# jzhoulab/orca

Hardware: AMD Instinct MI355X
Metric: Mb of sequence encoded+decoded per second (32Mb H1-ESC-shaped model, both strands, 6 levels) (higher is better)
Workload: dtype f16x2 | Encoder Conv1d stages 1-7: f16x2 = fp32 emulated as 2 x fp16 split operands, 3 MFMA products, fp32 accumulate (22 significant operand bits); Decoder / Decoder_1m Conv2d: f16x2 = fp32 emulated as 2 x fp16 split operands, 3 MFMA products, fp32 accumulate (22 significant operand bits); Encoder2; 1 GPU; H1-ESC 32Mb model forward, single random 32Mb sequence, fp32-class (f16x2 split operands on the 16-bit matrix cores, see dtype; parity vs the reference's fp32 in `parity` with --full), both strands (genomepredict-equivalent, 1 model): Encoder+Encoder2+6 Decoder+Decoder_1m per strand; sequence_bp=32000000, strands=2, levels=6, weights=synthetic seed 0, input=1 byte/base packed sequence in HBM, both strands read from it, parallelism=single GPU

## Files before the change

### include/orca_hip.h

```cpp
#ifndef ORCA_HIP_H
#define ORCA_HIP_H

#include <stddef.h>
#include <stdint.h>

#ifdef __cplusplus
extern "C" {
#endif

#define ORCA_OK 0
#define ORCA_EINVAL (-1)
#define ORCA_EHIP (-2)
#define ORCA_ENOMEM (-3)
#define ORCA_ENODEV (-4)

#define ORCA_ABI_VERSION 1

typedef struct orca_ctx orca_ctx;
typedef struct orca_net orca_net;

enum orca_net_kind {
  ORCA_NET_ENCODER = 1,
  ORCA_NET_ENCODER2 = 2,
  ORCA_NET_ENCODER3 = 3,
  ORCA_NET_DECODER = 4,
  ORCA_NET_DECODER_1M = 5,
  ORCA_NET_ENCODER2B = 6
};

#define ORCA_UPSAMPLE_NEAREST 0
#define ORCA_UPSAMPLE_BILINEAR 1

typedef struct orca_conv_desc {
  const float* weight_host;
  const float* bias_host;
  int32_t cout;
  int32_t cin;
  int32_t ksize;
  int32_t dilation;
} orca_conv_desc;


int orca_abi_version(void);
const char* orca_last_error(void);

int orca_device_count(void);

int orca_ctx_create(int device, void* hip_stream, orca_ctx** out);
int orca_ctx_destroy(orca_ctx* ctx);
int orca_ctx_set_stream(orca_ctx* ctx, void* hip_stream);
int orca_ctx_workspace_bytes(orca_ctx* ctx, size_t* out);
int orca_ctx_release_workspace(orca_ctx* ctx);

typedef struct orca_kernel_time {
  int32_t cout, cin, tile, batch;
  int64_t n;
  float ms;
  int32_t ksize;
} orca_kernel_time;
int orca_ctx_set_timing(orca_ctx* ctx, int enable);
int orca_ctx_get_timing(orca_ctx* ctx, orca_kernel_time* out, int max, int* n);

int orca_ctx_launch_counts(orca_ctx* ctx, int64_t* counts4);

int orca_net_create(orca_ctx* ctx, int kind, const orca_conv_desc* convs, int n_convs,
                    int upsample_mode, orca_net** out);
int orca_net_free(orca_net* net);

#define ORCA_PRECISION_F32 0
#define ORCA_PRECISION_BF16 1
#define ORCA_PRECISION_BF16X2 2
#define ORCA_PRECISION_BF16X3 3
#define ORCA_PRECISION_F16X2 4
#define ORCA_PRECISION_F16 5
int orca_net_set_precision(orca_net* net, int precision);
#define ORCA_ENCODER_FORM_DEFAULT 0
#define ORCA_ENCODER_FORM_STORED_RESIDUAL 1
#define ORCA_ENCODER_FORM_LCONV1_ONLY 2
#define ORCA_ENCODER_FORM_TWO_CONV 3
int orca_net_set_encoder_form(orca_net* net, int form);
int orca_net_set_decoder_block_runs(orca_net* net, int on);
int orca_net_set_encoder_two_strands(orca_net* net, int on);
int orca_net_get_encoder_two_strands(orca_net* net, int* on);
int orca_ctx_take_overflow(orca_ctx* ctx, int* flag);


int orca_encoder_forward(orca_ctx* ctx, orca_net* net, const float* x, int64_t sx_b, int64_t sx_c,
                         int64_t sx_l, int B, int64_t L, int64_t bin_lo, int64_t bin_hi, float* out,
                         int64_t so_b, int64_t so_c, int64_t chunk_bp);

int orca_pack_sequence(orca_ctx* ctx, const float* x, int64_t sx_c, int64_t sx_l, int64_t L, uint8_t* codes_out, int* packable);
int orca_encoder_forward_codes(orca_ctx* ctx, orca_net* net, const uint8_t* codes, int64_t sc_b, int reverse, int B, int64_t L,
                               int64_t bin_lo, int64_t bin_hi, float* out, int64_t so_b, int64_t so_c, int64_t chunk_bp);
int orca_encoder_forward_codes_window(orca_ctx* ctx, orca_net* net, const uint8_t* codes, int64_t sc_b, int64_t win_origin,
                                      int64_t win_len, int reverse, int B, int64_t L, int64_t bin_lo, int64_t bin_hi,
                                      float* out, int64_t so_b, int64_t so_c, int64_t chunk_bp);
int orca_encoder_forward_2bit(orca_ctx* ctx, orca_net* net, const uint8_t* two, const uint8_t* nmask, int64_t start, int reverse, int64_t L,
                              int64_t bin_lo, int64_t bin_hi, float* out, int64_t so_c, int64_t chunk_bp);
int orca_encoder_forward_two_strands(orca_ctx* ctx, orca_net* net, const uint8_t* codes, int64_t L, float* out_fwd, float* out_rev, int64_t so_c);

int64_t orca_p16_plane_units(int64_t n);
int orca_encoder_stage3_planes(orca_ctx* ctx, orca_net* net, const uint8_t* codes, int64_t L, int reverse, float* planes, int64_t plane_units);
int orca_p16_pool5_into(orca_ctx* ctx, const float* src, int64_t src_units, int64_t src_pos0, float* dst, int64_t dst_units, int64_t dst_pos0, int64_t count);
int orca_encoder_front_snippet(orca_ctx* ctx, orca_net* net, const uint8_t* codes, int64_t L, int reverse, int64_t base0, int64_t nbases, int64_t skip,
                               int64_t count, float* dst, int64_t dst_units, int64_t dst_pos0);
int orca_encoder_back(orca_ctx* ctx, orca_net* net, const float* s4, int64_t s4_units, int64_t n4, float* out, int64_t so_c);
int orca_encoder_stage4_rows(orca_ctx* ctx, orca_net* net, const float* s4, int64_t s4_units, int64_t n4, float* rows);
int orca_rows_pool5_into(orca_ctx* ctx, const float* src, int64_t src_rows, int64_t src_pos0, float* dst, int64_t dst_rows, int64_t dst_pos0, int64_t count);
int orca_encoder_front4_snippet(orca_ctx* ctx, orca_net* net, const uint8_t* codes, int64_t L, int reverse, int64_t base0, int64_t nbases, int64_t skip,
                                int64_t count, float* dst, int64_t dst_rows, int64_t dst_pos0);
int orca_encoder_front4_ranges(orca_ctx* ctx, orca_net* net, const uint8_t* codes, int64_t L, int reverse, int n_ranges, const int64_t* ranges_host,
                               float* dst, int64_t dst_rows);
int orca_encoder_back5(orca_ctx* ctx, orca_net* net, const float* rows, int64_t n5, float* out, int64_t so_c);

int orca_screen_edit_codes(orca_ctx* ctx, const uint8_t* window, int64_t L, const int64_t* table, int n_snippets, const uint8_t* payload, int64_t n_payload,
                           uint8_t* out, int64_t total);
int orca_screen_splice_rows(orca_ctx* ctx, const float* ref, int64_t n5, const float* fresh, int64_t n_fresh, const int64_t* table, int B, float* out);
int orca_encoder_back5_batch(orca_ctx* ctx, orca_net* net, const float* rows, int B, int64_t n5, float* out, int64_t so_b, int64_t so_c);
int orca_screen_scores(orca_ctx* ctx, const float* alt, int64_t map_bs, const float* ref, int B, int n, float* profile, float* mean, float* amax);

int orca_screen_edit_codes_multi(orca_ctx* ctx, const uint8_t* window, int64_t L, const int64_t* table, const int64_t* table_host, int n_snippets,
                                 const int64_t* spans, const int64_t* spans_host, int64_t n_spans, const uint8_t* payload, int64_t n_payload, uint8_t* out,
                                 int64_t total);
int orca_screen_splice_rows_multi(orca_ctx* ctx, const float* ref, int64_t n5, const float* fresh, int64_t n_fresh, const int64_t* segments,
                                  const int64_t* segments_host, int64_t n_segments, const int64_t* seg_off, const int64_t* seg_off_host, int B, float* out);
int orca_screen_region_scores(orca_ctx* ctx, const float* alt, int64_t map_bs, const float* ref, int B, int n, const int32_t* rects,
                              const int32_t* rects_host, int K, float* mean_signed, float* mean_abs);

int orca_screen_assemble_codes(orca_ctx* ctx, const uint8_t* context, int64_t C, const int64_t* table, const int64_t* table_host, int n_snippets,
                               const int64_t* pieces, const int64_t* pieces_host, int64_t n_pieces, const uint8_t* payload, int64_t n_payload, uint8_t* out,
                               int64_t total);
int orca_screen_gather_rows(orca_ctx* ctx, const float* ref, int64_t n5, const float* fresh, int64_t n_fresh, const float* const* entries,
                            const int64_t* entry_rows, const int64_t* entry_rows_host, int P, const int64_t* segments, const int64_t* segments_host,
                            int64_t n_segments, const int64_t* seg_off, const int64_t* seg_off_host, int B, float* out);

int orca_screen_aligned_scores(orca_ctx* ctx, const float* alt, int64_t map_bs, const float* ref, int B, int n, const int32_t* bin_map,
                               const int32_t* bin_map_host, float* profile, float* mean, float* amax);
int orca_screen_aligned_region_scores(orca_ctx* ctx, const float* alt, int64_t map_bs, const float* ref, int B, int n, const int32_t* bin_map,
                                      const int32_t* bin_map_host, const int32_t* rects, const int32_t* rects_host, int K, float* mean_signed,
                                      float* mean_abs);

int orca_screen_insulation(orca_ctx* ctx, const float* alt, int64_t map_bs, const float* ref, int B, int n, const int32_t* widths, const int32_t* widths_host,
                           int W, const int32_t* bin_map, const int32_t* bin_map_host, float* track, float* delta, float* aligned);
int orca_screen_viewpoints(orca_ctx* ctx, const float* alt, int64_t map_bs, const float* ref, int B, int n, const int32_t* views, const int32_t* views_host,
                           int V, const int32_t* bin_map, const int32_t* bin_map_host, float* delta, float* aligned);

int orca_screen_merge_strands(orca_ctx* ctx, const float* fwd, int64_t fwd_bs, const float* rev, int64_t rev_bs, const float* ref_fwd, const float* ref_rev,
                              int B, int n, float* out, int64_t out_bs, float* gap);

int orca_screen_epistasis_scores(orca_ctx* ctx, const float* alt, int64_t map_bs, const float* bank, int64_t bank_bs, int U, const float* ref, int B, int n,
                                 const int64_t* member_off, const int64_t* member_off_host, const int32_t* members, const int32_t* members_host, int64_t P,
                                 float* profile, float* mean, float* amax, float* add_mean);
int orca_screen_epistasis_region_scores(orca_ctx* ctx, const float* alt, int64_t map_bs, const float* bank, int64_t bank_bs, int U, const float* ref, int B,
                                        int n, const int64_t* member_off, const int64_t* member_off_host, const int32_t* members,
                                        const int32_t* members_host, int64_t P, const int32_t* rects, const int32_t* rects_host, int K, float* mean_signed,
                                        float* mean_abs);

int64_t orca_encoder_num_bins(int64_t L);

int orca_unet_forward(orca_ctx* ctx, orca_net* net, const float* x, int64_t sx_b, int64_t sx_c,
                      int64_t sx_l, int B, int n, float* const* outs_host, int n_outs);

int orca_decoder_forward(orca_ctx* ctx, orca_net* net, const float* x, int64_t sx_b, int64_t sx_c,
                         int64_t sx_l, const float* distenc, int64_t sd_b, int64_t sd_h, int64_t sd_w,
                         const float* y, int64_t sy_b, int64_t sy_h, int64_t sy_w, int B, int n,
                         float* out, int accumulate);

int orca_decoder_forward_mt(orca_ctx* ctx, orca_net* net, const float* x, int64_t sx_b, int64_t sx_c,
                            int64_t sx_l, const float* distenc, int64_t sd_b, int64_t sd_c, int64_t sd_h,
                            int64_t sd_w, const float* y, int64_t sy_b, int64_t sy_c, int64_t sy_h, int64_t sy_w,
                            int B, int n, float* out, int accumulate);

int orca_net_num_targets(orca_net* net, int* num_2d);

int orca_decoder_forward_rows(orca_ctx* ctx, orca_net* net, const float* const* x_rows, int64_t sx_c, int64_t sx_l,
                              const float* const* distenc_rows, int64_t sd_c, int64_t sd_h, int64_t sd_w,
                              const float* const* y_rows, int64_t sy_c, int64_t sy_h, int64_t sy_w, int B, int n,
                              float* out, int accumulate);
int orca_decoder1m_forward_rows(orca_ctx* ctx, orca_net* net, const float* const* x_rows, int64_t sx_c, int64_t sx_l,
                                int B, int n, float* out, int accumulate);

int orca_decoder1m_forward(orca_ctx* ctx, orca_net* net, const float* x, int64_t sx_b, int64_t sx_c,
                           int64_t sx_l, int B, int n, float* out, int accumulate);

int orca_decoder_probe(orca_ctx* ctx, orca_net* net, const float* x, int64_t sx_b, int64_t sx_c, int64_t sx_l,
                       const float* distenc, int64_t sd_b, int64_t sd_c, int64_t sd_h, int64_t sd_w, const float* y,
                       int64_t sy_b, int64_t sy_c, int64_t sy_h, int64_t sy_w, int B, int n, int stage, int channels,
                       float* map_out);

int orca_strand_merge(orca_ctx* ctx, const float* fwd, const float* rev, float* out, int n);

int orca_block_mean_f64(orca_ctx* ctx, const double* mat, int64_t ld, int64_t row0, int64_t col0, int nb, int npix,
                        double* mean_out, float* log_out, int flip);

int orca_adaptive_coarsegrain(orca_ctx* ctx, const float* ar, const float* countar, int64_t ld, int n, float cutoff,
                              int max_levels, int min_shape, float* out, int64_t ld_out);

int orca_genome_unpack_2bit(orca_ctx* ctx, const uint8_t* two_bit, const uint8_t* nmask, int64_t start, int64_t n, uint8_t* codes);

typedef struct orca_comm orca_comm;
#define ORCA_COMM_ID_BYTES 128
int orca_comm_unique_id(void* id128_host);
int orca_comm_init_rank(orca_ctx* ctx, int nranks, int rank, const void* id128_host, orca_comm** out);
int orca_comm_destroy(orca_comm* comm);
int orca_allgather(orca_ctx* ctx, orca_comm* comm, const float* send, float* recv, size_t count);

int orca_pointwise1d_forward(orca_ctx* ctx, const float* w_dev, const float* bias_dev, int cout, int cin, const float* x,
                             int64_t x_bs, int64_t ldx, float* y, int64_t y_bs, int64_t ldy, int B, int64_t n, int act);

int orca_conv1d_forward(orca_ctx* ctx, const orca_conv_desc* conv, const float* x, int64_t x_bs, int64_t ldx,
                        float* y, int64_t y_bs, int64_t ldy, const float* r1, const float* r2, int B, int64_t n,
                        int relu, int tile);
int orca_conv1d_nlc_forward(orca_ctx* ctx, const orca_conv_desc* conv, int precision, const float* x, float* y,
                            const float* r1, int B, int64_t n, int relu);
int orca_conv1d_p16_forward(orca_ctx* ctx, const orca_conv_desc* conv, const float* x, float* y, const float* r1,
                            int64_t n, int relu, int out_mode);
int orca_conv1d_b16_forward(orca_ctx* ctx, const orca_conv_desc* conv, const float* x, float* y, const float* r1,
                            int64_t n, int relu, int out_mode);
int orca_conv2d_forward(orca_ctx* ctx, const orca_conv_desc* conv, const float* x, float* y, const float* r,
                        int B, int n, int relu);
int orca_conv2d_m16_forward(orca_ctx* ctx, const orca_conv_desc* conv, int precision, const float* x, float* y,
                            const float* r, int B, int n, int relu);
int orca_conv2d_dblock_forward(orca_ctx* ctx, const orca_conv_desc* convs, int precision, const float* x, float* y, int B, int n);
int orca_conv2d_dblock_run_forward(orca_ctx* ctx, const orca_conv_desc* convs, int nblk, int precision, const float* x, float* y, int B, int n,
                                   int fused);
int orca_maxpool1d_forward(orca_ctx* ctx, const float* x, int64_t ldx, float* y, int64_t ldy, int64_t rows,
                           int64_t n_out, int k);

#ifdef __cplusplus
}
#endif
#endif
```

### orca_amd/_lib.py

```python
import ctypes
import os
from ctypes import POINTER, c_char_p, c_int, c_int32, c_int64, c_size_t, c_void_p

_HERE = os.path.dirname(os.path.abspath(__file__))
LIB_PATH = os.path.join(_HERE, "csrc", "liborca_hip.so")

ORCA_NET_ENCODER, ORCA_NET_ENCODER2, ORCA_NET_ENCODER3, ORCA_NET_DECODER, ORCA_NET_DECODER_1M, ORCA_NET_ENCODER2B = 1, 2, 3, 4, 5, 6
ORCA_UPSAMPLE_NEAREST, ORCA_UPSAMPLE_BILINEAR = 0, 1
PRECISIONS = {"f32": 0, "bf16": 1, "bf16x2": 2, "bf16x3": 3, "f16x2": 4, "f16": 5}
ENCODER_FORMS = {"default": 0, "stored_residual": 1, "lconv1_only": 2, "two_conv": 3}


class OrcaHipError(RuntimeError):
    pass


class ConvDesc(ctypes.Structure):
    _fields_ = [("weight_host", c_void_p), ("bias_host", c_void_p), ("cout", c_int32), ("cin", c_int32),
                ("ksize", c_int32), ("dilation", c_int32)]


class KernelTime(ctypes.Structure):
    _fields_ = [("cout", c_int32), ("cin", c_int32), ("tile", c_int32), ("batch", c_int32), ("n", c_int64),
                ("ms", ctypes.c_float), ("ksize", c_int32)]


SIGNATURES = {
    "orca_abi_version": (c_int, []),
    "orca_last_error": (c_char_p, []),
    "orca_device_count": (c_int, []),
    "orca_ctx_create": (c_int, [c_int, c_void_p, POINTER(c_void_p)]),
    "orca_ctx_destroy": (c_int, [c_void_p]),
    "orca_ctx_set_stream": (c_int, [c_void_p, c_void_p]),
    "orca_ctx_workspace_bytes": (c_int, [c_void_p, POINTER(c_size_t)]),
    "orca_ctx_release_workspace": (c_int, [c_void_p]),
    "orca_ctx_take_overflow": (c_int, [c_void_p, POINTER(c_int)]),
    "orca_ctx_set_timing": (c_int, [c_void_p, c_int]),
    "orca_ctx_get_timing": (c_int, [c_void_p, POINTER(KernelTime), c_int, POINTER(c_int)]),
    "orca_ctx_launch_counts": (c_int, [c_void_p, POINTER(ctypes.c_int64)]),
    "orca_net_create": (c_int, [c_void_p, c_int, POINTER(ConvDesc), c_int, c_int, POINTER(c_void_p)]),
    "orca_net_free": (c_int, [c_void_p]),
    "orca_net_set_precision": (c_int, [c_void_p, c_int]),
    "orca_net_set_encoder_form": (c_int, [c_void_p, c_int]),
    "orca_net_set_decoder_block_runs": (c_int, [c_void_p, c_int]),
    "orca_net_set_encoder_two_strands": (c_int, [c_void_p, c_int]),
    "orca_net_get_encoder_two_strands": (c_int, [c_void_p, POINTER(c_int)]),
    "orca_encoder_forward_two_strands": (c_int, [c_void_p, c_void_p, c_void_p, c_int64, c_void_p, c_void_p, c_int64]),
    "orca_encoder_forward": (c_int, [c_void_p, c_void_p, c_void_p, c_int64, c_int64, c_int64, c_int, c_int64, c_int64,
                                     c_int64, c_void_p, c_int64, c_int64, c_int64]),
    "orca_p16_plane_units": (c_int64, [c_int64]),
    "orca_encoder_stage3_planes": (c_int, [c_void_p, c_void_p, c_void_p, c_int64, c_int, c_void_p, c_int64]),
    "orca_p16_pool5_into": (c_int, [c_void_p, c_void_p, c_int64, c_int64, c_void_p, c_int64, c_int64, c_int64]),
    "orca_encoder_front_snippet": (c_int, [c_void_p, c_void_p, c_void_p, c_int64, c_int, c_int64, c_int64, c_int64, c_int64, c_void_p, c_int64, c_int64]),
    "orca_encoder_back": (c_int, [c_void_p, c_void_p, c_void_p, c_int64, c_int64, c_void_p, c_int64]),
    "orca_encoder_stage4_rows": (c_int, [c_void_p, c_void_p, c_void_p, c_int64, c_int64, c_void_p]),
    "orca_rows_pool5_into": (c_int, [c_void_p, c_void_p, c_int64, c_int64, c_void_p, c_int64, c_int64, c_int64]),
    "orca_encoder_front4_snippet": (c_int, [c_void_p, c_void_p, c_void_p, c_int64, c_int, c_int64, c_int64, c_int64, c_int64, c_void_p, c_int64, c_int64]),
    "orca_encoder_front4_ranges": (c_int, [c_void_p, c_void_p, c_void_p, c_int64, c_int, c_int, POINTER(ctypes.c_int64), c_void_p, c_int64]),
    "orca_encoder_back5": (c_int, [c_void_p, c_void_p, c_void_p, c_int64, c_void_p, c_int64]),
    "orca_screen_edit_codes": (c_int, [c_void_p, c_void_p, c_int64, c_void_p, c_int, c_void_p, c_int64, c_void_p, c_int64]),
    "orca_screen_splice_rows": (c_int, [c_void_p, c_void_p, c_int64, c_void_p, c_int64, c_void_p, c_int, c_void_p]),
    "orca_encoder_back5_batch": (c_int, [c_void_p, c_void_p, c_void_p, c_int, c_int64, c_void_p, c_int64, c_int64]),
    "orca_screen_scores": (c_int, [c_void_p, c_void_p, c_int64, c_void_p, c_int, c_int, c_void_p, c_void_p, c_void_p]),
    "orca_screen_edit_codes_multi": (c_int, [c_void_p, c_void_p, c_int64, c_void_p, c_void_p, c_int, c_void_p, c_void_p, c_int64, c_void_p, c_int64, c_void_p,
                                             c_int64]),
    "orca_screen_splice_rows_multi": (c_int, [c_void_p, c_void_p, c_int64, c_void_p, c_int64, c_void_p, c_void_p, c_int64, c_void_p, c_void_p, c_int, c_void_p]),
    "orca_screen_region_scores": (c_int, [c_void_p, c_void_p, c_int64, c_void_p, c_int, c_int, c_void_p, c_void_p, c_int, c_void_p, c_void_p]),
    "orca_screen_assemble_codes": (c_int, [c_void_p, c_void_p, c_int64, c_void_p, c_void_p, c_int, c_void_p, c_void_p, c_int64, c_void_p, c_int64, c_void_p,
                                           c_int64]),
    "orca_screen_gather_rows": (c_int, [c_void_p, c_void_p, c_int64, c_void_p, c_int64, c_void_p, c_void_p, c_void_p, c_int, c_void_p, c_void_p, c_int64, c_void_p,
                                        c_void_p, c_int, c_void_p]),
    "orca_screen_aligned_scores": (c_int, [c_void_p, c_void_p, c_int64, c_void_p, c_int, c_int, c_void_p, c_void_p, c_void_p, c_void_p, c_void_p]),
    "orca_screen_aligned_region_scores": (c_int, [c_void_p, c_void_p, c_int64, c_void_p, c_int, c_int, c_void_p, c_void_p, c_void_p, c_void_p, c_int, c_void_p,
                                                  c_void_p]),
    "orca_screen_insulation": (c_int, [c_void_p, c_void_p, c_int64, c_void_p, c_int, c_int, c_void_p, c_void_p, c_int, c_void_p, c_void_p, c_void_p, c_void_p,
                                       c_void_p]),
    "orca_screen_viewpoints": (c_int, [c_void_p, c_void_p, c_int64, c_void_p, c_int, c_int, c_void_p, c_void_p, c_int, c_void_p, c_void_p, c_void_p, c_void_p]),
    "orca_screen_merge_strands":(c_int, [c_void_p, c_void_p, c_int64, c_void_p, c_int64, c_void_p, c_void_p, c_int, c_int, c_void_p, c_int64, c_void_p]),
    "orca_screen_epistasis_scores": (c_int, [c_void_p, c_void_p, c_int64, c_void_p, c_int64, c_int, c_void_p, c_int, c_int, c_void_p, c_void_p, c_void_p, c_void_p,
                                             c_int64, c_void_p, c_void_p, c_void_p, c_void_p]),
    "orca_screen_epistasis_region_scores": (c_int, [c_void_p, c_void_p, c_int64, c_void_p, c_int64, c_int, c_void_p, c_int, c_int, c_void_p, c_void_p, c_void_p,
                                                    c_void_p, c_int64, c_void_p, c_void_p, c_int, c_void_p, c_void_p]),
    "orca_encoder_forward_2bit": (c_int, [c_void_p, c_void_p, c_void_p, c_void_p, c_int64, c_int, c_int64, c_int64, c_int64, c_void_p, c_int64, c_int64]),
    "orca_pack_sequence": (c_int, [c_void_p, c_void_p, c_int64, c_int64, c_int64, c_void_p, POINTER(c_int)]),
    "orca_encoder_forward_codes": (c_int, [c_void_p, c_void_p, c_void_p, c_int64, c_int, c_int, c_int64, c_int64, c_int64,
                                           c_void_p, c_int64, c_int64, c_int64]),
    "orca_encoder_forward_codes_window": (c_int, [c_void_p, c_void_p, c_void_p, c_int64, c_int64, c_int64, c_int, c_int, c_int64, c_int64, c_int64,
                                                  c_void_p, c_int64, c_int64, c_int64]),
    "orca_encoder_num_bins": (c_int64, [c_int64]),
    "orca_unet_forward": (c_int, [c_void_p, c_void_p, c_void_p, c_int64, c_int64, c_int64, c_int, c_int,
                                  POINTER(c_void_p), c_int]),
    "orca_decoder_forward": (c_int, [c_void_p, c_void_p, c_void_p, c_int64, c_int64, c_int64, c_void_p, c_int64,
                                     c_int64, c_int64, c_void_p, c_int64, c_int64, c_int64, c_int, c_int, c_void_p, c_int]),
    "orca_decoder_forward_mt": (c_int, [c_void_p, c_void_p, c_void_p, c_int64, c_int64, c_int64, c_void_p, c_int64, c_int64,
                                        c_int64, c_int64, c_void_p, c_int64, c_int64, c_int64, c_int64, c_int, c_int, c_void_p, c_int]),
    "orca_decoder_forward_rows": (c_int, [c_void_p, c_void_p, POINTER(c_void_p), c_int64, c_int64, POINTER(c_void_p), c_int64, c_int64, c_int64,
                                          POINTER(c_void_p), c_int64, c_int64, c_int64, c_int, c_int, c_void_p, c_int]),
    "orca_decoder1m_forward_rows": (c_int, [c_void_p, c_void_p, POINTER(c_void_p), c_int64, c_int64, c_int, c_int, c_void_p, c_int]),
    "orca_net_num_targets": (c_int, [c_void_p, POINTER(c_int)]),
    "orca_decoder1m_forward": (c_int, [c_void_p, c_void_p, c_void_p, c_int64, c_int64, c_int64, c_int, c_int, c_void_p, c_int]),
    "orca_decoder_probe": (c_int, [c_void_p, c_void_p, c_void_p, c_int64, c_int64, c_int64, c_void_p, c_int64, c_int64, c_int64, c_int64, c_void_p,
                                   c_int64, c_int64, c_int64, c_int64, c_int, c_int, c_int, c_int, c_void_p]),
    "orca_strand_merge": (c_int, [c_void_p, c_void_p, c_void_p, c_void_p, c_int]),
    "orca_block_mean_f64": (c_int, [c_void_p, c_void_p, c_int64, c_int64, c_int64, c_int, c_int, c_void_p, c_void_p, c_int]),
    "orca_adaptive_coarsegrain": (c_int, [c_void_p, c_void_p, c_void_p, c_int64, c_int, ctypes.c_float, c_int, c_int, c_void_p, c_int64]),
    "orca_genome_unpack_2bit": (c_int, [c_void_p, c_void_p, c_void_p, c_int64, c_int64, c_void_p]),
    "orca_comm_unique_id": (c_int, [c_void_p]),
    "orca_comm_init_rank": (c_int, [c_void_p, c_int, c_int, c_void_p, POINTER(c_void_p)]),
    "orca_comm_destroy": (c_int, [c_void_p]),
    "orca_allgather": (c_int, [c_void_p, c_void_p, c_void_p, c_void_p, c_size_t]),
    "orca_conv1d_forward": (c_int, [c_void_p, POINTER(ConvDesc), c_void_p, c_int64, c_int64, c_void_p, c_int64, c_int64,
                                    c_void_p, c_void_p, c_int, c_int64, c_int, c_int]),
    "orca_conv1d_nlc_forward": (c_int, [c_void_p, POINTER(ConvDesc), c_int, c_void_p, c_void_p, c_void_p, c_int, c_int64, c_int]),
    "orca_conv1d_p16_forward": (c_int, [c_void_p, POINTER(ConvDesc), c_void_p, c_void_p, c_void_p, c_int64, c_int, c_int]),
    "orca_conv1d_b16_forward": (c_int, [c_void_p, POINTER(ConvDesc), c_void_p, c_void_p, c_void_p, c_int64, c_int, c_int]),
    "orca_conv2d_forward": (c_int, [c_void_p, POINTER(ConvDesc), c_void_p, c_void_p, c_void_p, c_int, c_int, c_int]),
    "orca_conv2d_m16_forward": (c_int, [c_void_p, POINTER(ConvDesc), c_int, c_void_p, c_void_p, c_void_p, c_int, c_int, c_int]),
    "orca_conv2d_dblock_forward": (c_int, [c_void_p, POINTER(ConvDesc), c_int, c_void_p, c_void_p, c_int, c_int]),
    "orca_conv2d_dblock_run_forward": (c_int, [c_void_p, POINTER(ConvDesc), c_int, c_int, c_void_p, c_void_p, c_int, c_int, c_int]),
    "orca_maxpool1d_forward": (c_int, [c_void_p, c_void_p, c_int64, c_void_p, c_int64, c_int64, c_int64, c_int]),
    "orca_pointwise1d_forward": (c_int, [c_void_p, c_void_p, c_void_p, c_int, c_int, c_void_p, c_int64, c_int64, c_void_p, c_int64,
                                          c_int64, c_int, c_int64, c_int]),
}

_lib = None


def load():
    global _lib
    if _lib is not None:
        return _lib
    if not os.path.exists(LIB_PATH):
        raise OrcaHipError(
            f"{LIB_PATH} not found: the HIP extension is not built. Run `make -C orca_amd/csrc` "
            "(or `python -c 'import __graft_entry__ as g; g.build()'`). There is no CPU fallback.")
    import torch
    lib = ctypes.CDLL(LIB_PATH)
    for name, (res, args) in SIGNATURES.items():
        fn = getattr(lib, name)
        fn.restype = res
        fn.argtypes = args
    if lib.orca_abi_version() != 1:
        raise OrcaHipError("liborca_hip ABI version mismatch")
    _lib = lib
    return lib


def check(rc, what=""):
    if rc != 0:
        msg = load().orca_last_error()
        raise OrcaHipError(f"{what} failed (code {rc}): {msg.decode('utf8', 'replace') if msg else ''}")
```

### orca_amd/csrc/conv2d_dblock.h

```cpp
#pragma once
#include "conv2d_m16.h"

struct DBlockArgs {
  f32x4* cur;
  const void* w[12];
  const float* bias[12];
  long bs;
  int H, W, dil, nblk;
  unsigned* flag;
};

#ifndef DBLOCK_STORE_WT
#define DBLOCK_STORE_WT 0
#endif
__device__ __forceinline__ void db_store_unit(u32x4_t* p, const u32x4_t& v) {
#if DBLOCK_STORE_WT
  m16_store_unit(p, v);
#else
  *p = v;
#endif
}

template <int N>
__device__ __forceinline__ void db_vmwait() { asm volatile("s_waitcnt vmcnt(%0)" ::"n"(N) : "memory"); }

template <int NS, int DT, int MAXBLK, int ABL>
__device__ __forceinline__ void dblock_body(const DBlockArgs& a) {
  static_assert(MAXBLK == 1 || (NS == 2 && DT == 1), "block runs: f16x2 only");
  constexpr int WNS = DT == 1 ? 2 : 1;
  constexpr int NT = 512, PXW = 256 + 16;
  constexpr int AU = NS * 8 * PXW, BU = NS * 4 * PXW;
  constexpr int WP = NS * 9 * 2 * 32;
  constexpr int WIT = (WP + NT - 1) / NT;
  static_assert(NS * 8 * 256 / NT == 4 * NS, "gather: NS DMA instructions per thread and K-chunk of the first layer (the same for every wave)");
  constexpr int EXTRA = (WP - (WIT - 1) * NT + 63) / 64;
  __shared__ f32x4 smem[AU + BU + 3 * WP + 48 * MAXBLK];
  f32x4* const As = smem;
  f32x4* const Bs = smem + AU;
  f32x4* const Ws = smem + AU + BU;
  float* const bias_s = reinterpret_cast<float*>(smem + AU + BU + 3 * WP);

  const int tid = threadIdx.x, lane = tid & 63;
  const int wave = __builtin_amdgcn_readfirstlane(tid >> 6);
  const int l31 = lane & 31, g = lane >> 5;
  const int d = a.dil, H = a.H, W = a.W;
  const int nblk = MAXBLK == 1 ? 1 : a.nblk;
  const int ld = 31 - __builtin_clz(d);
  const int lS = 8 - ld, S = 1 << lS;
  const int lG = 2 * ld - 8, G = 1 << lG;
  f32x4* const cur = a.cur + (long)blockIdx.y * a.bs;

  int bx = (int)blockIdx.x;
  if (!(ABL & 64)) {
    const int xcd = bx & 7, t = bx >> 3;
    if (G == 1) { const int run = xcd * 4 + (t >> 3); bx = (run >> 1) * 16 + (run & 1) * 8 + (t & 7); }
    else if (G == 4) { const int pair = xcd * 16 + (t >> 1); bx = pair * 2 + (t & 1); }
  }
  auto pix = [&](int p, int& row, int& col, int& r, int& c) {
    const int sid = (bx << lG) + (p >> (2 * lS)), q = p & ((1 << (2 * lS)) - 1);
    r = q >> lS; c = q & (S - 1);
    row = (sid >> ld) + (r << ld);
    col = (sid & (d - 1)) + (c << ld);
  };
  {
    const int sid0 = bx << lG;
    if ((sid0 >> ld) >= H || (sid0 & (d - 1)) >= W) return;
  }

  if (tid < NS * 8 * 16) As[(tid >> 4) * PXW + 256 + (tid & 15)] = (f32x4)(0.f);
  if (tid >= 256 && tid < 256 + NS * 4 * 16) Bs[((tid - 256) >> 4) * PXW + 256 + (tid & 15)] = (f32x4)(0.f);
  __syncthreads();
  if (wave == 0 && lane < 48) {
#pragma unroll
    for (int b = 0; b < MAXBLK; ++b)
      if (b < nblk) {
        const float *b0 = a.bias[4 * b], *b1 = a.bias[4 * b + 1], *b2 = a.bias[4 * b + 2], *b3 = a.bias[4 * b + 3];
        const float* src = lane < 8 ? b0 + 4 * lane : (lane < 24 ? b1 + 4 * (lane - 8) : (lane < 32 ? b2 + 4 * (lane - 24) : b3 + 4 * (lane - 32)));
        p16_glds16(reinterpret_cast<const f32x4*>(src), smem + AU + BU + 3 * WP + 48 * b);
      }
  }

  auto issue_piece = [&](const void* wl, int i, int slot) {
    const int L = i >> 2, j = i & 3;
    const bool wide = L & 1;
    const int k = wide ? (j & 1) : j, h = wide ? (j >> 1) : 0, cout = wide ? 64 : 32;
    f32x4* dst = Ws + slot;
#pragma unroll
    for (int it = 0; it < WIT; ++it) {
      const int u = tid + it * NT;
      const int grp = u >> 5, co = u & 31;
      if (u < WP) p16_glds16(reinterpret_cast<const f32x4*>(wl) + ((long)k * (WNS * 9 * 2) + grp) * cout + h * 32 + co, dst + it * NT + wave * 64);
    }
  };
  int ro0 = 0, ro1 = WP, ro2 = 2 * WP;
  {
    int row, col, r_, c_;
    pix(tid & 255, row, col, r_, c_);
    const bool ok = row < H && col < W;
    const long off = ok ? (long)row * M16_PX + col : 255;
#pragma unroll
    for (int k = 0; k < 4; ++k) {
#pragma unroll
      for (int s_ = 0; s_ < NS; ++s_) {
        const int plane = s_ * 8 + 2 * k + (wave >> 2);
        if (!(ABL & 4)) p16_glds16(cur + m16_plane(plane & 7, s_, NS, H) + off, As + plane * PXW + (wave & 3) * 64);
      }
      if (k < 3) issue_piece(a.w[0], k, k * WP);
    }
  }

  const int p = wave * 32 + l31;
  int prow, pcol, pr, pc;
  pix(p, prow, pcol, pr, pc);
  const bool pvalid = prow < H && pcol < W;
  const long poff = (long)prow * M16_PX + pcol;

  f32x16 acc[2];
  const unsigned as_lds = p16_lds_addr(As), bs_lds = p16_lds_addr(Bs), ws_lds = p16_lds_addr(Ws + g * 32 + l31);
  bool overflow = false;
  auto put = [&](f32x4* Xs, int XG, int oct, f32x4 v) {
    if (!pvalid) v = (f32x4)(0.f);
    u32x2 sp[NS];
    split4<NS, DT>(v, sp, overflow);
#pragma unroll
    for (int s = 0; s < NS; ++s) *reinterpret_cast<u32x2*>(reinterpret_cast<char*>(Xs + (s * XG + oct) * PXW + p) + 8 * g) = sp[s];
  };
  auto get_A = [&](int oct) -> f32x4 {
    float f[4] = {0.f, 0.f, 0.f, 0.f};
#pragma unroll
    for (int s = 0; s < NS; ++s) {
      const u32x2 u = *reinterpret_cast<const u32x2*>(reinterpret_cast<const char*>(As + (s * 8 + oct) * PXW + p) + 8 * g);
      float a0, a1, a2, a3;
      m16_pair<DT>(u.x, a0, a1);
      m16_pair<DT>(u.y, a2, a3);
      f[0] += a0; f[1] += a1; f[2] += a2; f[3] += a3;
    }
    f32x4 r;
    r.x = f[0]; r.y = f[1]; r.z = f[2]; r.w = f[3];
    return r;
  };
  auto acc4 = [&](int h, int q, const float* bl, bool relu) -> f32x4 {
    const f32x4 b = *reinterpret_cast<const f32x4*>(bl + 8 * q + 4 * g);
    f32x4 v;
    v.x = acc[h][4 * q + 0] + b.x; v.y = acc[h][4 * q + 1] + b.y; v.z = acc[h][4 * q + 2] + b.z; v.w = acc[h][4 * q + 3] + b.w;
    if (relu) { v.x = p16_vmax(v.x, 0.f); v.y = p16_vmax(v.y, 0.f); v.z = p16_vmax(v.z, 0.f); v.w = p16_vmax(v.w, 0.f); }
    return v;
  };
  auto zero_acc = [&]() {
#pragma unroll
    for (int h = 0; h < 2; ++h)
#pragma unroll
      for (int r = 0; r < 16; ++r) acc[h][r] = 0.f;
  };
#define DB_READ(buf_, t_)                                                                                         \
  _Pragma("unroll") for (int s = 0; s < NS; ++s) {                                                                \
    xv[buf_][s] = p16_lds_read16(xrow + nb16[t_], s * XG * PXW * 16);                                             \
    wv[buf_][s] = p16_lds_read16(wrow, ((s * 9 + (t_)) * 2) * 32 * 16);                                           \
  }
#define DB_WAIT(NG, NW)                            \
  if (wave < EXTRA) db_vmwait<(NG) * NS + (NW) * WIT>(); else db_vmwait<(NG) * NS + (NW) * (WIT - 1)>()
#define DB_LAYER(LY, XLDS, XG_, WIDE)                                                                             \
  {                                                                                                               \
    constexpr int XG = XG_;                                                                                       \
    _Pragma("unroll") for (int j = 0; j < 4; ++j) {                                                               \
      constexpr bool wide_ = WIDE;                                                                                \
      const int piece = 4 * (LY) + j;                                                                             \
      const int k = wide_ ? (j & 1) : j;                                                                          \
      const int h = wide_ ? (j >> 1) : 0;                                                                         \
      if (piece <= 2 && first) {                                                                                  \
        if (piece == 0) { DB_WAIT(3, 2); } else if (piece == 1) { DB_WAIT(2, 1); } else { DB_WAIT(1, 1); }        \
      } else if (piece == 15 && last) db_vmwait<0>();                                                             \
      else { DB_WAIT(0, 1); }                                                                                     \
      if (!(ABL & 16) || j == 0) asm volatile("s_waitcnt lgkmcnt(0)\n\ts_barrier" ::: "memory");                  \
      if (!(ABL & 2)) {                                                                                           \
        const int slot2 = (piece + 2) % 3 == 0 ? ro0 : ((piece + 2) % 3 == 1 ? ro1 : ro2);                        \
        if (piece == 0) { if (!first) issue_piece(wb[0], 2, slot2); }                                             \
        else if (piece >= 14) { if (!last) issue_piece(wb[4], piece - 14, slot2); }                               \
        else issue_piece(wb[(piece + 2) >> 2], piece + 2, slot2);                                                 \
      }                                                                                                           \
      const unsigned wrow = ws_lds + (unsigned)((piece % 3 == 0 ? ro0 : (piece % 3 == 1 ? ro1 : ro2)) * 16);     \
      const unsigned xrow = (XLDS) + (unsigned)((2 * k + g) * PXW * 16);                                          \
      f16x8 xv[2][NS], wv[2][NS];                                                                                 \
      DB_READ(0, 0);                                                                                              \
      _Pragma("unroll") for (int t = 0; t < 9; ++t) {                                                             \
        const int fb = t & 1;                                                                                     \
        if (t + 1 < 9) { if (!(ABL & 8)) { DB_READ(fb ^ 1, t + 1); m16_wait<2 * NS, NS>(xv[fb], wv[fb]); } }      \
        else m16_wait<0, NS>(xv[fb], wv[fb]);                                                                     \
        typedef typename Op16<DT>::vec V_;                                                                        \
        if constexpr ((ABL & 1) != 0) { asm volatile("" ::"v"(xv[fb][0]), "v"(wv[fb][0])); } else                \
        if constexpr (NS == 2) {                                                                                  \
          acc[h] = Op16<DT>::mfma(__builtin_bit_cast(V_, wv[fb][0]), __builtin_bit_cast(V_, xv[fb][NS - 1]), acc[h]); \
          acc[h] = Op16<DT>::mfma(__builtin_bit_cast(V_, wv[fb][NS - 1]), __builtin_bit_cast(V_, xv[fb][0]), acc[h]); \
        }                                                                                                         \
        if constexpr ((ABL & 1) == 0) acc[h] = Op16<DT>::mfma(__builtin_bit_cast(V_, wv[fb][0]), __builtin_bit_cast(V_, xv[fb][0]), acc[h]); \
        __builtin_amdgcn_sched_barrier(0);                                                                        \
      }                                                                                                           \
    }                                                                                                             \
  }

  float vmax = 0.f;
#pragma unroll 1
  for (int bi = 0; bi < nblk; ++bi) {
    const int b = MAXBLK == 1 ? 0 : bi;
    const bool first = b == 0, last = MAXBLK == 1 || b + 1 == nblk;
    const void* wb[5];
#pragma unroll
    for (int q = 0; q < 5; ++q) wb[q] = a.w[4 * b + (q < 4 || !last ? q : 0)];
    const float* const bl = bias_s + 192 * b;
    unsigned nb16[9];
#pragma unroll
    for (int t = 0; t < 9; ++t) {
      const int dy = (t / 3 - 1) * (1 << b), dx = (t % 3 - 1) * (1 << b);
      const bool in = (unsigned)(pr + dy) < (unsigned)S && (unsigned)(pc + dx) < (unsigned)S;
      nb16[t] = (in ? (unsigned)(p + dy * S + dx) : 256u + ((unsigned)(p + dy * S + dx) & 15u)) * 16u;
    }
    zero_acc();
    DB_LAYER(0, as_lds, 8, false);
#pragma unroll
    for (int q = 0; q < 4; ++q) put(Bs, 4, q, acc4(0, q, bl, false));
    zero_acc();
    DB_LAYER(1, bs_lds, 4, true);
#pragma unroll
    for (int h = 0; h < 2; ++h)
#pragma unroll
      for (int q = 0; q < 4; ++q) put(As, 8, h * 4 + q, acc4(h, q, bl + 32 + h * 32, false) + get_A(h * 4 + q));
    zero_acc();
    DB_LAYER(2, as_lds, 8, false);
#pragma unroll
    for (int q = 0; q < 4; ++q) put(Bs, 4, q, acc4(0, q, bl + 96, true));
    zero_acc();
    DB_LAYER(3, bs_lds, 4, true);
    if constexpr (NS == 2) {
#pragma unroll
      for (int h = 0; h < 2; ++h)
#pragma unroll
        for (int q = 0; q < 4; ++q) {
          f32x4 v = acc4(h, q, bl + 128 + h * 32, true) + get_A(h * 4 + q);
          vmax = p16_vmax3_abs(p16_vmax3_abs(vmax, v.x, v.y), v.z, v.w);
          if (!last && !pvalid) v = (f32x4)(0.f);
          unsigned h0_, h1_, l0_, l1_;
          p16_split_hl(v, h0_, h1_, l0_, l1_);
          if (last) {
            p16_swap32(h0_, l0_);
            p16_swap32(h1_, l1_);
            u32x4_t unit_;
            unit_.x = h0_; unit_.y = h1_; unit_.z = l0_; unit_.w = l1_;
            if (pvalid) db_store_unit(reinterpret_cast<u32x4_t*>(cur) + m16_plane(h * 4 + q, g, NS, H) + poff, unit_);
          } else {
            u32x2 hi_, lo_;
            hi_.x = h0_; hi_.y = h1_; lo_.x = l0_; lo_.y = l1_;
            *reinterpret_cast<u32x2*>(reinterpret_cast<char*>(As + (h * 4 + q) * PXW + p) + 8 * g) = hi_;
            *reinterpret_cast<u32x2*>(reinterpret_cast<char*>(As + (8 + h * 4 + q) * PXW + p) + 8 * g) = lo_;
          }
        }
    } else {
#pragma unroll
      for (int h = 0; h < 2; ++h)
#pragma unroll
        for (int qp = 0; qp < 2; ++qp) {
          const f32x4 v0 = acc4(h, 2 * qp, bl + 128 + h * 32, true) + get_A(h * 4 + 2 * qp);
          const f32x4 v1 = acc4(h, 2 * qp + 1, bl + 128 + h * 32, true) + get_A(h * 4 + 2 * qp + 1);
          if (DT == 1) vmax = p16_vmax3_abs(p16_vmax3_abs(p16_vmax3_abs(p16_vmax3_abs(vmax, v0.x, v0.y), v0.z, v0.w), v1.x, v1.y), v1.z, v1.w);
          unsigned a0_ = m16_pk2<DT>(v0.x, v0.y), a1_ = m16_pk2<DT>(v0.z, v0.w), b0_ = m16_pk2<DT>(v1.x, v1.y), b1_ = m16_pk2<DT>(v1.z, v1.w);
          p16_swap32(a0_, b0_);
          p16_swap32(a1_, b1_);
          u32x4_t unit_;
          unit_.x = a0_; unit_.y = a1_; unit_.z = b0_; unit_.w = b1_;
          if (pvalid) db_store_unit(reinterpret_cast<u32x4_t*>(cur) + m16_plane(h * 4 + 2 * qp + g, 0, NS, H) + poff, unit_);
        }
    }
    if constexpr (MAXBLK > 1) { const int t_ = ro0; ro0 = ro1; ro1 = ro2; ro2 = t_; }
  }
#undef DB_LAYER
#undef DB_WAIT
#undef DB_READ
  if (DT == 1 && pvalid && vmax > 65504.f) overflow = true;
  if (DT == 1 && overflow && a.flag) *a.flag = 1u;
}

template <int NS, int DT, int ABL = 0>
__global__ __launch_bounds__(512, NS == 1 ? 4 : 2) void conv2d_dblock_kernel(DBlockArgs a) {
  dblock_body<NS, DT, 1, ABL>(a);
}

template <int NS, int DT, int ABL = 0>
__global__ __launch_bounds__(512, 2) void conv2d_dblock_run_kernel(DBlockArgs a) {
  dblock_body<NS, DT, 3, ABL>(a);
}
```

### orca_amd/csrc/conv2d_m16q.h

```cpp
#pragma once
#include <type_traits>
#include "conv2d_m16.h"

struct ConvM16QArgs {
  ConvM16Args c;
  const f32x4* zero;
  int ngroups;
  int nb;
};

__device__ __forceinline__ float m16_hl_lo(unsigned h, unsigned l) {
  float r;
  asm("v_fma_mix_f32 %0, %1, 1.0, %2 op_sel_hi:[1,0,1]" : "=v"(r) : "v"(h), "v"(l));
  return r;
}
__device__ __forceinline__ float m16_hl_hi(unsigned h, unsigned l) {
  float r;
  asm("v_fma_mix_f32 %0, %1, 1.0, %2 op_sel:[1,0,1] op_sel_hi:[1,0,1]" : "=v"(r) : "v"(h), "v"(l));
  return r;
}


template <int COUT, int NS, int DT, int HB = 0, int NH = COUT / 32>
__device__ __forceinline__ void m16_tile_epilogue(const ConvM16Args& a, f32x16 (&acc)[NH], int b, int yr, int px, int g,
                                                  const u32x4_t* ru, bool res, float& vmax) {
  const int H = a.H, W = a.W;
  const bool pxok = px < W;
  const long rowoff = (long)yr * M16_PX + px;
  f32x4* const yb = a.y + (long)b * a.y_bs;
  const f32x4* const rb = res ? a.r + (long)b * a.r_bs : nullptr;
  const float* tabr = nullptr;
  const float* tabc = nullptr;
  if (a.tab && pxok) {
    const float* tb = a.tab + (long)b * a.tab_bs;
    const int xc = px == 0 ? 0 : (px == W - 1 ? 2 : 1), yc = yr == 0 ? 0 : (yr == H - 1 ? 2 : 1);
    tabr = tb + ((long)xc * H + yr) * 64;
    tabc = tb + ((long)(3 + yc) * H + px) * 64;
  }
  if constexpr (NS == 2) {
#pragma unroll
    for (int h = 0; h < NH; ++h)
#pragma unroll
      for (int q = 0; q < 4; ++q) {
        const int o = (HB + h) * 4 + q;
        f32x4 v;
        v.x = acc[h][4 * q + 0]; v.y = acc[h][4 * q + 1]; v.z = acc[h][4 * q + 2]; v.w = acc[h][4 * q + 3];
        if (tabr) {
          const f32x4 tr = *reinterpret_cast<const f32x4*>(tabr + (HB + h) * 32 + 8 * q + 4 * g), tc = *reinterpret_cast<const f32x4*>(tabc + (HB + h) * 32 + 8 * q + 4 * g);
          v.x += tr.x + tc.x; v.y += tr.y + tc.y; v.z += tr.z + tc.z; v.w += tr.w + tc.w;
        }
        if (a.relu) { v.x = p16_vmax(v.x, 0.f); v.y = p16_vmax(v.y, 0.f); v.z = p16_vmax(v.z, 0.f); v.w = p16_vmax(v.w, 0.f); }
        if (rb) {
          const u32x4_t u_ = ru[h * 4 + q];
          unsigned ux_ = u_.x, uy_ = u_.y, uz_ = u_.z, uw_ = u_.w;
          p16_swap32(ux_, uz_);
          p16_swap32(uy_, uw_);
          v.x += m16_hl_lo(ux_, uz_); v.y += m16_hl_hi(ux_, uz_);
          v.z += m16_hl_lo(uy_, uw_); v.w += m16_hl_hi(uy_, uw_);
        }
        if (!pxok) v = (f32x4)(0.f);
        vmax = p16_vmax3_abs(p16_vmax3_abs(vmax, v.x, v.y), v.z, v.w);
        unsigned h0_, h1_, l0_, l1_;
        p16_split_hl(v, h0_, h1_, l0_, l1_);
        p16_swap32(h0_, l0_);
        p16_swap32(h1_, l1_);
        u32x4_t unit_;
        unit_.x = h0_; unit_.y = h1_; unit_.z = l0_; unit_.w = l1_;
        m16_store_unit(reinterpret_cast<u32x4_t*>(yb) + m16_plane(o, g, NS, H) + rowoff, unit_);
      }
  } else {
#pragma unroll
    for (int h = 0; h < NH; ++h)
#pragma unroll
      for (int qp = 0; qp < 2; ++qp) {
        const int o = (HB + h) * 4 + 2 * qp;
        f32x4 v0, v1;
        v0.x = acc[h][8 * qp + 0]; v0.y = acc[h][8 * qp + 1]; v0.z = acc[h][8 * qp + 2]; v0.w = acc[h][8 * qp + 3];
        v1.x = acc[h][8 * qp + 4]; v1.y = acc[h][8 * qp + 5]; v1.z = acc[h][8 * qp + 6]; v1.w = acc[h][8 * qp + 7];
        if (tabr) {
          const int co_ = (HB + h) * 32 + 16 * qp + 4 * g;
          const f32x4 r0 = *reinterpret_cast<const f32x4*>(tabr + co_), c0 = *reinterpret_cast<const f32x4*>(tabc + co_);
          const f32x4 r1 = *reinterpret_cast<const f32x4*>(tabr + co_ + 8), c1 = *reinterpret_cast<const f32x4*>(tabc + co_ + 8);
          v0.x += r0.x + c0.x; v0.y += r0.y + c0.y; v0.z += r0.z + c0.z; v0.w += r0.w + c0.w;
          v1.x += r1.x + c1.x; v1.y += r1.y + c1.y; v1.z += r1.z + c1.z; v1.w += r1.w + c1.w;
        }
        if (a.relu) {
          v0.x = p16_vmax(v0.x, 0.f); v0.y = p16_vmax(v0.y, 0.f); v0.z = p16_vmax(v0.z, 0.f); v0.w = p16_vmax(v0.w, 0.f);
          v1.x = p16_vmax(v1.x, 0.f); v1.y = p16_vmax(v1.y, 0.f); v1.z = p16_vmax(v1.z, 0.f); v1.w = p16_vmax(v1.w, 0.f);
        }
        if (rb) {
          const u32x4_t u_ = reinterpret_cast<const u32x4_t*>(rb)[m16_plane(o + g, 0, NS, H) + rowoff];
// ... 14 lines not shown
        u32x4_t unit_;
        unit_.x = a0_; unit_.y = a1_; unit_.z = b0_; unit_.w = b1_;
        m16_store_unit(reinterpret_cast<u32x4_t*>(yb) + m16_plane(o + g, 0, NS, H) + rowoff, unit_);
      }
  }
}

template <int N, int NS>
__device__ __forceinline__ void m16q_wait_w(f16x8 (&w)[NS]) {
  if constexpr (NS == 2) asm volatile("s_waitcnt lgkmcnt(%2)" : "+v"(w[0]), "+v"(w[1]) : "n"(N));
  else asm volatile("s_waitcnt lgkmcnt(%1)" : "+v"(w[0]) : "n"(N));
}
template <int N, int NS>
__device__ __forceinline__ void m16q_wait_xw(f16x8 (&x)[4][NS], f16x8 (&w)[NS]) {
  if constexpr (NS == 2)
    asm volatile("s_waitcnt lgkmcnt(%10)"
                 : "+v"(x[0][0]), "+v"(x[0][1]), "+v"(x[1][0]), "+v"(x[1][1]), "+v"(x[2][0]), "+v"(x[2][1]), "+v"(x[3][0]), "+v"(x[3][1]), "+v"(w[0]), "+v"(w[1])
                 : "n"(N));
  else asm volatile("s_waitcnt lgkmcnt(%5)" : "+v"(x[0][0]), "+v"(x[1][0]), "+v"(x[2][0]), "+v"(x[3][0]), "+v"(w[0]) : "n"(N));
}
template <int N>
__device__ __forceinline__ void m16q_vmwait() { asm volatile("s_waitcnt vmcnt(%0)" ::"n"(N) : "memory"); }

#ifndef M16Q_SPREAD
#define M16Q_SPREAD 1
#endif
#ifndef M16Q_ABL
#define M16Q_ABL 0
#endif
#ifdef M16Q_STAMPS
__device__ unsigned long long m16q_stamp_buf[8 * 16];
#define M16Q_STAMP(n_) { if (blockIdx.x == M16Q_STAMPS && blockIdx.y == 0 && lane == 0) { m16q_stamp_buf[wave * 16 + (n_)] = __builtin_readcyclecounter(); if ((n_) == 0 || (n_) == 11) m16q_stamp_buf[wave * 16 + 12 + ((n_) != 0)] = __builtin_amdgcn_s_memrealtime(); } }
#else
#define M16Q_STAMP(n_)
#endif
template <int COUT, int NS, int DT>
__global__ __launch_bounds__(512, 1) void conv2d_3x3_m16q_kernel(ConvM16QArgs aq) {
  static_assert(NS == 1 || DT == 1, "f16x2, plain fp16 or plain bf16");
  const ConvM16Args& a = aq.c;
  constexpr int WNS = DT == 1 ? 2 : 1;
  constexpr int NT = 512, NH = COUT / 32, TW = 128, ROWP = 8 + TW + 8, SR = 6;
  constexpr int XROWS = NS * 2 * SR;
  constexpr int XB = XROWS * ROWP;
  constexpr int WP = NS * 9 * 2 * 32;
  constexpr int XIT = (XB + NT - 1) / NT;
  constexpr int XFULL = (XB - (XIT - 1) * NT) / 64;
  constexpr int WIT = (WP + NT - 1) / NT;
  constexpr int WFULL = (WP - (WIT - 1) * NT) / 64;
  static_assert(XB % 64 == 0 && WP % 64 == 0, "whole-wave DMA rounds");
  __shared__ f32x4 smem[2 * XB + 2 * WP];
  f32x4* const Xs = smem;
  f32x4* const Ws = smem + 2 * XB;

  const int tid = threadIdx.x, lane = tid & 63;
  const int wave = __builtin_amdgcn_readfirstlane(tid >> 6);
  const int l31 = lane & 31, g = lane >> 5;
  const int H = a.H, d = a.dil;
  int b = blockIdx.y;
  const int nb = aq.nb, bstep = gridDim.y;
  const int per_xcd = (int)gridDim.x >> 3, tix = ((int)blockIdx.x & 7) * per_xcd + ((int)blockIdx.x >> 3);
  if (tix >= aq.ngroups * 2) return;
  const int nq = aq.ngroups / d, cls = (tix >> 1) / nq, q4 = (tix >> 1) - cls * nq, px0 = (tix & 1) * TW;
  const int y0 = q4 * 4 * d + cls;
  if (y0 >= H) return;
  const int r0 = (wave >> 2) * 2;
  const int wpx = (wave & 3) * 32;
  M16Q_STAMP(0);

  int xoff[XIT];
#pragma unroll
  for (int it = 0; it < XIT; ++it) {
    const int u = it * NT + tid;
    const int uu = u < XB ? u : 0;
    const int row = uu / ROWP, col = uu - row * ROWP;
    const int s = row / (2 * SR), gg = (row / SR) & 1, rr = row % SR;
    const int ys = y0 + (rr - 1) * d, px = px0 - 8 + col;
    const bool ok = ys >= 0 && ys < H && px >= 0 && px < M16_PX;
    xoff[it] = ok ? (int)(m16_plane(gg, s, NS, H) + (long)ys * M16_PX + px) : -1;
  }
  const f32x4* xb = a.x + (long)b * a.x_bs;
  auto issue_x1 = [&](const f32x4* xm, int k, int buf, int it) {
    if (it + 1 < XIT || wave < XFULL) p16_glds16(xoff[it] >= 0 ? xm + m16_plane(2 * k, 0, NS, H) + xoff[it] : aq.zero, Xs + buf * XB + it * NT + wave * 64);
  };
  auto issue_w1 = [&](int i, int slot, int it) {
    const int k = i / NH, h = i - k * NH;
    const int u = tid + it * NT;
    if (it + 1 < WIT || wave < WFULL)
      p16_glds16(reinterpret_cast<const f32x4*>(a.w) + ((long)k * (WNS * 9 * 2) + (u >> 5)) * COUT + h * 32 + (u & 31), Ws + slot * WP + it * NT + wave * 64);
  };
  auto issue_x = [&](const f32x4* xm, int k, int buf) {
#pragma unroll
    for (int it = 0; it < XIT; ++it) issue_x1(xm, k, buf, it);
  };
  auto issue_w = [&](int i, int slot) {
#pragma unroll
    for (int it = 0; it < WIT; ++it) issue_w1(i, slot, it);
  };

  issue_w(0, 0);
  issue_x(xb, 0, 0);
  M16Q_STAMP(1);
  const unsigned ws_lds = p16_lds_addr(Ws + g * 32 + l31);
  const unsigned xs_lds = p16_lds_addr(Xs + (g * SR + r0) * ROWP + 8 + wpx + l31);
  const int px = px0 + wpx + l31;
  const int yr0 = y0 + r0 * d, yr1 = yr0 + d;
  float vmax = 0.f;

  while (true) {
  const bool has_next = b + bstep < nb;
  const f32x4* const xb_next = xb + (long)bstep * a.x_bs;

  f32x16 acc[2][NH];
  int gb_ = g;
  asm volatile("" : "+v"(gb_));
#pragma unroll
  for (int h = 0; h < NH; ++h)
#pragma unroll
    for (int q = 0; q < 4; ++q) {
      const f32x4 b4 = *reinterpret_cast<const f32x4*>(a.bias + h * 32 + 8 * q + 4 * gb_);
#pragma unroll
      for (int j = 0; j < 2; ++j) { acc[j][h][4 * q + 0] = b4.x; acc[j][h][4 * q + 1] = b4.y; acc[j][h][4 * q + 2] = b4.z; acc[j][h][4 * q + 3] = b4.w; }
    }

  constexpr int NRU = NS == 2 ? NH * 4 : 1;
  u32x4_t ru[NRU], ru1[NRU];
  const f32x4* const rb = a.r ? a.r + (long)b * a.r_bs : nullptr;
  const bool res_late = rb != nullptr;

#define M16Q_READ_X(dst_, kx_)                                            \
  if constexpr (!(M16Q_ABL & 2)) _Pragma("unroll") for (int j_ = 0; j_ < 4; ++j_)                         \
      _Pragma("unroll") for (int s_ = 0; s_ < NS; ++s_) dst_[j_][s_] = p16_lds_read16(xcol[kx_], ((s_ * 2 * SR) + j_) * ROWP * 16);
#define M16Q_READ_W(dst_, t_) if constexpr (!(M16Q_ABL & 2)) _Pragma("unroll") for (int s_ = 0; s_ < NS; ++s_) dst_[s_] = p16_lds_read16(wrow, ((s_ * 9 + (t_)) * 2) * 32 * 16);
#define M16Q_MFMA(w_, x_, j_, h_)                                                                                       \
  if constexpr (!(M16Q_ABL & 1)) {                                                                                      \
    typedef typename Op16<DT>::vec V_;                                                                                  \
    if constexpr (NS == 2) {                                                                                            \
      acc[j_][h_] = Op16<DT>::mfma(__builtin_bit_cast(V_, w_[0]), __builtin_bit_cast(V_, x_[NS - 1]), acc[j_][h_]);     \
      acc[j_][h_] = Op16<DT>::mfma(__builtin_bit_cast(V_, w_[NS - 1]), __builtin_bit_cast(V_, x_[0]), acc[j_][h_]);     \
    }                                                                                                                   \
    acc[j_][h_] = Op16<DT>::mfma(__builtin_bit_cast(V_, w_[0]), __builtin_bit_cast(V_, x_[0]), acc[j_][h_]);           \
  }

  auto piece = [&](const int k, auto hc, auto lastc) __attribute__((always_inline)) {
    constexpr int h = decltype(hc)::value;
    constexpr bool LASTP = decltype(lastc)::value;
    const int i = k * NH + h;
    if (!LASTP && NH == 2 && h == 1) {
      if (wave < XFULL) m16q_vmwait<XIT>();
      else m16q_vmwait<XIT - 1>();
    } else m16q_vmwait<0>();
    M16Q_STAMP(2 + 2 * (i < 4 ? i : 3));
    M16_BARRIER();
    M16Q_STAMP(3 + 2 * (i < 4 ? i : 3));
    if constexpr (NS == 2 && LASTP) {
      if (res_late && yr0 < H) {
        int px_ = px, g_ = g;
        asm volatile("" : "+v"(px_), "+v"(g_));
#pragma unroll
        for (int j = 0; j < NRU; ++j) ru[j] = reinterpret_cast<const u32x4_t*>(rb)[m16_plane(j, g_, NS, H) + (long)yr0 * M16_PX + px_];
      } else {
#pragma unroll
        for (int j = 0; j < NRU; ++j) ru[j] = (u32x4_t)(0u);
      }
    }
    const bool lastk = k + 1 == a.nchunks;
    const bool dow = (LASTP ? has_next : true) && !(M16Q_ABL & 16);
    const bool dox = (LASTP ? (NH == 1 && has_next) : (h == 0 && (lastk ? (NH == 2 && has_next) : true))) && !(M16Q_ABL & 8);
    const int i_nx = LASTP ? 0 : i + 1, k_nx = (LASTP || lastk) ? 0 : k + 1;
    const f32x4* const x_nx = (LASTP || lastk) ? xb_next : xb;
    static_assert(WIT + XIT <= 10, "transfer slots of a piece");
#define M16Q_DMA_SLOT(n_)                                                                              \
  {                                                                                                    \
    const int first_ = (n_) == 0 ? 0 : (n_) + 1, cnt_ = (n_) == 0 ? 2 : 1;                              \
    _Pragma("unroll") for (int q_ = first_; q_ < first_ + cnt_; ++q_) {                                 \
      if (q_ < WIT) { if (dow) issue_w1(i_nx, (i + 1) & 1, q_); }                                       \
      else if (q_ - WIT < XIT) { if (dox) issue_x1(x_nx, k_nx, (k + 1) & 1, q_ - WIT); }                \
    }                                                                                                  \
  }
    if (!M16Q_SPREAD) {
      if (dow) issue_w(i_nx, (i + 1) & 1);
      if (dox) issue_x(x_nx, k_nx, (k + 1) & 1);
    }
    const unsigned wrow = ws_lds + (unsigned)((i & 1) * WP * 16);
    unsigned xcol[3];
#pragma unroll
    for (int kx = 0; kx < 3; ++kx) xcol[kx] = xs_lds + (unsigned)(((k & 1) * XB + (kx - 1) * d) * 16);
    f16x8 xr[2][4][NS], wv[2][NS];
    if constexpr (M16Q_ABL & 2) { _Pragma("unroll") for (int q_ = 0; q_ < 2; ++q_) _Pragma("unroll") for (int s_ = 0; s_ < NS; ++s_) { wv[q_][s_] = (f16x8)(0); _Pragma("unroll") for (int j_ = 0; j_ < 4; ++j_) xr[q_][j_][s_] = (f16x8)(0); } }
    M16Q_READ_X(xr[0], 0);
    M16Q_READ_W(wv[0], 0);
#pragma unroll
    for (int kx = 0; kx < 3; ++kx) {
#pragma unroll
      for (int ky = 0; ky < 3; ++ky) {
        const int n = kx * 3 + ky, fb = n & 1, xq = kx & 1;
        if (M16Q_SPREAD) M16Q_DMA_SLOT(n);
        if constexpr (NS == 2 && LASTP) {
          if (kx == 2 && ky == 0 && res_late && yr1 < H) {
            int px_ = px, g_ = g;
            asm volatile("" : "+v"(px_), "+v"(g_));
#pragma unroll
            for (int j = 0; j < NRU; ++j) ru1[j] = reinterpret_cast<const u32x4_t*>(rb)[m16_plane(j, g_, NS, H) + (long)yr1 * M16_PX + px_];
          } else if (kx == 2 && ky == 0) {
#pragma unroll
            for (int j = 0; j < NRU; ++j) ru1[j] = (u32x4_t)(0u);
          }
        }
        if (n < 8) { const int n1 = n + 1, t1 = (n1 % 3) * 3 + n1 / 3; M16Q_READ_W(wv[fb ^ 1], t1); }
        if (ky == 0 && kx < 2) M16Q_READ_X(xr[xq ^ 1], kx + 1);
        if (ky == 0) {
          if (kx == 0 && (M16Q_ABL & 32)) m16q_wait_xw<15, NS>(xr[xq], wv[fb]);
          else if (kx < 2) m16q_wait_xw<5 * NS, NS>(xr[xq], wv[fb]);
          else m16q_wait_xw<NS, NS>(xr[xq], wv[fb]);
        } else {
          if (n < 8) m16q_wait_w<NS, NS>(wv[fb]);
          else m16q_wait_w<0, NS>(wv[fb]);
        }
        M16Q_MFMA(wv[fb], xr[xq][ky], 0, h);
        M16Q_MFMA(wv[fb], xr[xq][ky + 1], 1, h);
        __builtin_amdgcn_sched_barrier(0);
      }
    }
  };
  typedef std::integral_constant<int, 0> H0_;
  typedef std::integral_constant<int, 1> H1_;
  for (int k = 0; k + 1 < a.nchunks; ++k) {
    piece(k, H0_(), std::false_type());
    if constexpr (NH == 2) piece(k, H1_(), std::false_type());
  }
  if constexpr (NH == 2) {
    piece(a.nchunks - 1, H0_(), std::false_type());
    piece(a.nchunks - 1, H1_(), std::true_type());
  } else piece(a.nchunks - 1, H0_(), std::true_type());

  M16Q_STAMP(10);
  if constexpr (M16Q_ABL & 4) { if (acc[0][0][0] != 0.12345f) return; }
  {
    int px_ = px, g_ = g;
    asm volatile("" : "+v"(px_), "+v"(g_));
    if (yr0 < H) m16_tile_epilogue<COUT, NS, DT>(a, acc[0], b, yr0, px_, g_, ru, res_late, vmax);
    if (yr1 < H) m16_tile_epilogue<COUT, NS, DT>(a, acc[1], b, yr1, px_, g_, ru1, res_late, vmax);
  }
  M16Q_STAMP(11);
  if (!has_next) break;
  b += bstep;
  xb = xb_next;
  }
#undef M16Q_READ_X
#undef M16Q_READ_W
#undef M16Q_MFMA
#undef M16Q_DMA_SLOT
  if (DT == 1 && vmax > 65504.f && a.flag) *a.flag = 1u;
}
```

### orca_amd/csrc/orca_core.hip

```cpp
#include "orca_internal.h"

static thread_local std::string g_err;

int fail(int code, const char* fmt, ...) {
  char buf[1024];
  va_list ap;
  va_start(ap, fmt);
  vsnprintf(buf, sizeof buf, fmt, ap);
  va_end(ap);
  g_err = buf;
  return code;
}

int ws_ensure(orca_ctx* ctx, size_t bytes) {
  ctx->ws_off = 0;
  if (ctx->ws_used && ctx->ws_stream != ctx->stream) HIPCHECK(hipStreamSynchronize(ctx->ws_stream));
  ctx->ws_stream = ctx->stream;
  ctx->ws_used = true;
  if (bytes <= ctx->ws_bytes) return ORCA_OK;
  const size_t step = bytes >= (size_t(1) << 30) ? (size_t(1) << 30) : (size_t(64) << 20);
  bytes = (bytes + step - 1) / step * step;
  if (ctx->ws) {
    HIPCHECK(hipStreamSynchronize(ctx->stream));
    HIPCHECK(hipFree(ctx->ws));
// ... 257 lines not shown
  HIPCHECK(hipSetDevice(device));
  hipDeviceProp_t prop;
  HIPCHECK(hipGetDeviceProperties(&prop, device));
  if (strncmp(prop.gcnArchName, "gfx950", 6) != 0)
    return fail(ORCA_ENODEV, "device %d is %s; liborca_hip is built for gfx950 only", device, prop.gcnArchName);
  orca_ctx* c = new orca_ctx();
  c->device = device;
  c->stream = static_cast<hipStream_t>(hip_stream);
  if (hipMalloc(reinterpret_cast<void**>(&c->d_flag), 4 * sizeof(unsigned)) != hipSuccess || hipMemset(c->d_flag, 0, 4 * sizeof(unsigned)) != hipSuccess ||
      hipMalloc(reinterpret_cast<void**>(&c->d_edge), 4 * 40 * 128 * sizeof(float)) != hipSuccess ||
      hipMalloc(reinterpret_cast<void**>(&c->d_zero), 256) != hipSuccess || hipMemset(c->d_zero, 0, 256) != hipSuccess) {
    delete c;
    return fail(ORCA_ENOMEM, "could not allocate the context flag word");
  }
  *out = c;
  return ORCA_OK;
}

extern "C" int orca_ctx_destroy(orca_ctx* ctx) {
  if (!ctx) return ORCA_OK;
  (void)hipSetDevice(ctx->device);
  if (ctx->ws) {
    if (ctx->ws_used && ctx->ws_stream != ctx->stream) (void)hipStreamSynchronize(ctx->ws_stream);
    (void)hipStreamSynchronize(ctx->stream);
    (void)hipFree(ctx->ws);
  }
  if (ctx->d_flag) (void)hipFree(ctx->d_flag);
  if (ctx->d_edge) (void)hipFree(ctx->d_edge);
  if (ctx->d_zero) (void)hipFree(ctx->d_zero);
  delete ctx;
  return ORCA_OK;
}

extern "C" int orca_ctx_set_stream(orca_ctx* ctx, void* hip_stream) {
  if (!ctx) return fail(ORCA_EINVAL, "ctx is NULL");
  ctx->stream = static_cast<hipStream_t>(hip_stream);
  return ORCA_OK;
}

extern "C" int orca_ctx_set_timing(orca_ctx* ctx, int enable) {
  if (!ctx) return fail(ORCA_EINVAL, "ctx is NULL");
  ctx->timing = enable != 0;
  return ORCA_OK;
}

extern "C" int orca_ctx_launch_counts(orca_ctx* ctx, int64_t* counts4) {
  if (!ctx || !counts4) return fail(ORCA_EINVAL, "NULL argument");
  for (int i = 0; i < 4; ++i) counts4[i] = ctx->counts[i];
  return ORCA_OK;
}

extern "C" int orca_ctx_get_timing(orca_ctx* ctx, orca_kernel_time* out, int max, int* n) {
  if (!ctx || !n) return fail(ORCA_EINVAL, "NULL argument");
  HIPCHECK(hipSetDevice(ctx->device));
  HIPCHECK(hipStreamSynchronize(ctx->stream));
  *n = (int)ctx->timed.size();
  for (size_t i = 0; i < ctx->timed.size(); ++i) {
    TimedLaunch& t = ctx->timed[i];
    float ms = 0.f;
    (void)hipEventElapsedTime(&ms, t.e0, t.e1);
    t.rec.ms = ms;
    if (out && (int)i < max) out[i] = t.rec;
    (void)hipEventDestroy(t.e0);
    (void)hipEventDestroy(t.e1);
  }
  ctx->timed.clear();
  return ORCA_OK;
}

extern "C" int orca_ctx_take_overflow(orca_ctx* ctx, int* flag) {
  if (!ctx || !flag) return fail(ORCA_EINVAL, "NULL argument");
  HIPCHECK(hipSetDevice(ctx->device));
  unsigned h = 0;
  HIPCHECK(hipMemcpyAsync(&h, ctx->d_flag, sizeof h, hipMemcpyDeviceToHost, ctx->stream));
  HIPCHECK(hipMemsetAsync(ctx->d_flag, 0, sizeof h, ctx->stream));
  HIPCHECK(hipStreamSynchronize(ctx->stream));
  *flag = (int)h;
  return ORCA_OK;
}

extern "C" int orca_ctx_workspace_bytes(orca_ctx* ctx, size_t* out) {
  if (!ctx || !out) return fail(ORCA_EINVAL, "NULL argument");
  *out = ctx->ws_bytes;
  return ORCA_OK;
}

extern "C" int orca_ctx_release_workspace(orca_ctx* ctx) {
  if (!ctx) return fail(ORCA_EINVAL, "ctx is NULL");
  HIPCHECK(hipSetDevice(ctx->device));
  if (ctx->ws) {
    if (ctx->ws_used && ctx->ws_stream != ctx->stream) HIPCHECK(hipStreamSynchronize(ctx->ws_stream));
    HIPCHECK(hipStreamSynchronize(ctx->stream));
    HIPCHECK(hipFree(ctx->ws));
  }
  ctx->ws = nullptr; ctx->ws_bytes = 0; ctx->ws_off = 0; ctx->ws_used = false;
  return ORCA_OK;
}

struct Shape { int cout, cin, k; };

static void expected_shapes(int kind, std::vector<Shape>* s, int T = 1) {
  const int F = T > 5 ? T : 5;
  s->clear();
  auto c1 = [&](int co, int ci) { s->push_back({co, ci, 9}); };
  auto c2 = [&](int co, int ci) { s->push_back({co, ci, 3}); };
  if (kind == ORCA_NET_ENCODER) {
    const int ch[7] = {64, 96, 128, 128, 128, 128, 128};
    int prev = 4;
    for (int i = 0; i < 7; ++i) { c1(ch[i], prev); c1(ch[i], ch[i]); c1(ch[i], ch[i]); c1(ch[i], ch[i]); prev = ch[i]; }
  } else if (kind == ORCA_NET_ENCODER2 || kind == ORCA_NET_ENCODER3) {
    const int nlev = kind == ORCA_NET_ENCODER2 ? 5 : 3;
    for (int i = 0; i < 8 * nlev; ++i) c1(128, 128);
  } else if (kind == ORCA_NET_ENCODER2B) {
    for (int i = 0; i < 4 * 5; ++i) c1(128, 128);
  } else if (kind == ORCA_NET_DECODER) {
    c2(64, 128 + T); c2(64, 64); c2(64, 64); c2(64, 64);
    c2(64, 64 + T); c2(64, 64); c2(64, 64); c2(64, 64);
    for (int i = 0; i < 28; ++i) { c2(32, 64); c2(64, 32); c2(32, 64); c2(64, 32); }
    s->push_back({F, 64, 1}); s->push_back({T, F, 1});
  } else if (kind == ORCA_NET_DECODER_1M) {
    for (int i = 0; i < 19; ++i) { c2(32, i == 0 ? 128 : 64); c2(64, 32); c2(32, 64); c2(64, 32); }
    s->push_back({F, 64, 1}); s->push_back({T, F, 1});
  }
}

extern "C" int orca_net_create(orca_ctx* ctx, int kind, const orca_conv_desc* convs, int n_convs, int upsample_mode, orca_net** out) {
  if (!ctx || !convs || !out) return fail(ORCA_EINVAL, "orca_net_create: NULL argument");
  HIPCHECK(hipSetDevice(ctx->device));
  std::vector<Shape> exp;
  int T = 1;
  if ((kind == ORCA_NET_DECODER || kind == ORCA_NET_DECODER_1M) && n_convs > 0) {
    T = convs[n_convs - 1].cout;
    if (T < 1 || T > ORCA_MAX_TARGETS) return fail(ORCA_EINVAL, "decoder with %d target maps (supported: 1..%d)", T, ORCA_MAX_TARGETS);
  }
  expected_shapes(kind, &exp, T);
  if (exp.empty()) return fail(ORCA_EINVAL, "unknown net kind %d", kind);
  if ((int)exp.size() != n_convs) return fail(ORCA_EINVAL, "net kind %d expects %zu convs, got %d", kind, exp.size(), n_convs);
  for (int i = 0; i < n_convs; ++i)
    if (convs[i].cout != exp[i].cout || convs[i].cin != exp[i].cin || convs[i].ksize != exp[i].k)
      return fail(ORCA_EINVAL, "net kind %d conv %d: expected cout=%d cin=%d k=%d, got cout=%d cin=%d k=%d", kind, i,
                  exp[i].cout, exp[i].cin, exp[i].k, convs[i].cout, convs[i].cin, convs[i].ksize);
  orca_net* net = new orca_net();
  net->ctx = ctx; net->kind = kind; net->upsample_mode = upsample_mode; net->num_2d = T;
  net->convs.resize(n_convs);
  for (int i = 0; i < n_convs; ++i) {
    int rc = make_layer(convs[i], &net->convs[i]);
    if (rc != ORCA_OK) { orca_net_free(net); return rc; }
  }
  if (kind == ORCA_NET_DECODER) {
    const orca_conv_desc& d0 = convs[0];
    std::vector<float> ws((size_t)2 * 3 * 3 * 128 * 64);
    for (int which = 0; which < 2; ++which)
      for (int cls = 0; cls < 3; ++cls)
        for (int k = 0; k < 3; ++k)
          for (int c = 0; c < 128; ++c)
            for (int co = 0; co < 64; ++co) {
              double acc = 0.0;
              for (int o = (cls == 0 ? 1 : 0); o <= (cls == 2 ? 1 : 2); ++o) {
                const int ky = which == 0 ? k : o, kx = which == 0 ? o : k;
                acc += d0.weight_host[(((size_t)co * d0.cin + c) * 3 + ky) * 3 + kx];
              }
              ws[((((size_t)which * 3 + cls) * 3 + k) * 128 + c) * 64 + co] = (float)acc;
            }
    int rc = upload(ws, &net->d_sep);
    if (rc != ORCA_OK) { orca_net_free(net); return rc; }
  }
// ... 40 lines not shown
      auto pack_first = [&](const std::vector<double>& w, const std::vector<double>& b, int ntap, void** d_w, float** d_b) -> int {
        const int KS = (4 * ntap + 15) / 16;
        std::vector<uint16_t> pk((size_t)2 * KS * 2 * 64 * 8, 0);
        for (int co = 0; co < 64; ++co)
          for (int k = 0; k < 4 * ntap; ++k) {
            float v = (float)w[((size_t)co * 4 + (k & 3)) * ntap + (k >> 2)];
            const int kk = k / 16, gg = (k % 16) / 8, e = k % 8;
            for (int sp = 0; sp < 2; ++sp) {
              const _Float16 hh = (_Float16)v;
              v -= (float)hh;
              uint16_t bits;
              memcpy(&bits, &hh, 2);
              pk[((((size_t)sp * KS + kk) * 2 + gg) * 64 + co) * 8 + e] = bits;
            }
          }
        std::vector<float> bf(64);
        for (int i = 0; i < 64; ++i) bf[i] = (float)b[i];
        if (hipMalloc(d_w, pk.size() * 2) != hipSuccess || hipMemcpy(*d_w, pk.data(), pk.size() * 2, hipMemcpyHostToDevice) != hipSuccess) return ORCA_EHIP;
        return upload(bf, d_b);
      };
      auto in_f16 = [](const std::vector<double>& w) {
        for (double v : w) if (!(v > -65504.0 && v < 65504.0)) return false;
        return true;
      };
      {
        auto tab32 = [&](const std::vector<double>& w, const std::vector<double>& b, int ntap, float** d_w, float** d_b) -> int {
          std::vector<float> t((size_t)ntap * 4 * 64), bf(64);
          for (int co = 0; co < 64; ++co) {
            bf[co] = (float)b[co];
            for (int ci = 0; ci < 4; ++ci)
              for (int tt = 0; tt < ntap; ++tt) t[((size_t)tt * 4 + ci) * 64 + co] = (float)w[((size_t)co * 4 + ci) * ntap + tt];
          }
          return upload(t, d_w) != ORCA_OK ? ORCA_EHIP : upload(bf, d_b);
        };
        if (tab32(w17, b17, 17, &net->d_l1_f32, &net->d_l1_bias32) != ORCA_OK || tab32(w25, b25, 25, &net->d_c1a_f32, &net->d_c1a_bias32) != ORCA_OK) {
          orca_net_free(net);
          return fail(ORCA_EHIP, "composed first-layer upload failed");
        }
      }
      if (in_f16(w17) && in_f16(b17)) {
        if (pack_first(w17, b17, 17, &net->d_l1_w16, &net->d_l1_bias) != ORCA_OK) { orca_net_free(net); return fail(ORCA_EHIP, "composed first-layer upload failed"); }
        if (in_f16(w25) && in_f16(b25) && pack_first(w25, b25, 25, &net->d_c1a_w16, &net->d_c1a_bias) != ORCA_OK) {
          orca_net_free(net);
          return fail(ORCA_EHIP, "composed first-layer upload failed");
        }
      }
      for (int st = 1; st <= 2; ++st) {
        compose_pair(convs[4 * st], convs[4 * st + 1], &w17, &b17);
        if (!in_f16(w17)) continue;
        rc = make_layer17(convs[4 * st].cin, convs[4 * st + 1].cout, w17, b17, &net->comp[st]);
        if (rc != ORCA_OK) { orca_net_free(net); return rc; }
      }
    }
  }
  *out = net;
  return ORCA_OK;
}

extern "C" int orca_net_set_precision(orca_net* net, int precision) {
  if (!net) return fail(ORCA_EINVAL, "net is NULL");
  if (precision < ORCA_PRECISION_F32 || precision > ORCA_PRECISION_F16) return fail(ORCA_EINVAL, "unknown precision %d", precision);
  const bool dec = net->kind == ORCA_NET_DECODER || net->kind == ORCA_NET_DECODER_1M;
  const bool unet = net->kind == ORCA_NET_ENCODER2 || net->kind == ORCA_NET_ENCODER3 || net->kind == ORCA_NET_ENCODER2B;
  if (precision != ORCA_PRECISION_F32 && !(((net->kind == ORCA_NET_ENCODER || unet) && precision != ORCA_PRECISION_F16) ||
                                           (dec && (precision == ORCA_PRECISION_F16X2 || precision == ORCA_PRECISION_BF16 || precision == ORCA_PRECISION_F16))))
    return fail(ORCA_EINVAL, "precision %d is not implemented for net kind %d", precision, net->kind);
  net->precision = precision;
  return ORCA_OK;
}

extern "C" int orca_net_set_encoder_form(orca_net* net, int form) {
  if (!net || net->kind != ORCA_NET_ENCODER) return fail(ORCA_EINVAL, "orca_net_set_encoder_form: not an Encoder net");
  if (form < ORCA_ENCODER_FORM_DEFAULT || form > ORCA_ENCODER_FORM_TWO_CONV) return fail(ORCA_EINVAL, "orca_net_set_encoder_form: form %d unknown", form);
  net->enc_form = form;
  return ORCA_OK;
}

extern "C" int orca_net_set_decoder_block_runs(orca_net* net, int on) {
  if (!net || (net->kind != ORCA_NET_DECODER && net->kind != ORCA_NET_DECODER_1M)) return fail(ORCA_EINVAL, "orca_net_set_decoder_block_runs: not a Decoder net");
  net->dec_block_runs = on ? 1 : 0;
  return ORCA_OK;
}

extern "C" int orca_net_free(orca_net* net) {
  if (!net) return ORCA_OK;
  if (net->ctx) (void)hipSetDevice(net->ctx->device);
  for (auto& L : net->convs) free_layer(L);
  if (net->d_first_w) (void)hipFree(net->d_first_w);
  if (net->d_first_w16) (void)hipFree(net->d_first_w16);
  if (net->d_first_tab) (void)hipFree(net->d_first_tab);
  if (net->d_sep) (void)hipFree(net->d_sep);
  if (net->d_l1_w16) (void)hipFree(net->d_l1_w16);
  if (net->d_l1_bias) (void)hipFree(net->d_l1_bias);
  if (net->d_c1a_w16) (void)hipFree(net->d_c1a_w16);
  if (net->d_c1a_bias) (void)hipFree(net->d_c1a_bias);
  if (net->d_l1_f32) (void)hipFree(net->d_l1_f32);
  if (net->d_c1a_f32) (void)hipFree(net->d_c1a_f32);
  if (net->d_l1_bias32) (void)hipFree(net->d_l1_bias32);
  if (net->d_c1a_bias32) (void)hipFree(net->d_c1a_bias32);
  for (auto& L : net->comp) free_layer(L);
  delete net;
  return ORCA_OK;
}


extern "C" int orca_net_num_targets(orca_net* net, int* num_2d) {
  if (!net || !num_2d) return fail(ORCA_EINVAL, "orca_net_num_targets: NULL argument");
  *num_2d = net->num_2d;
  return ORCA_OK;
}
```

### orca_amd/csrc/orca_decoder.hip

```cpp
#include "orca_internal.h"

#include <type_traits>

#include "conv2d_m16.h"
#include "conv2d_m16q.h"
#include "conv2d_dblock.h"
#include "misc_kernels.h"
#include "coarsegrain.h"

int launch_conv2d(orca_ctx* ctx, const ConvLayer& L, const float* x, long x_bs, float* y, long y_bs,
                         const float* r, long r_bs, int B, int n, int relu) {
  if (L.ksize != 3) return fail(ORCA_EINVAL, "launch_conv2d on a non-3x3 layer");
  Conv2dArgs a;
  a.x = x; a.w = L.d_w; a.bias = L.d_bias; a.y = y; a.r = r;
  a.x_bs = x_bs; a.y_bs = y_bs; a.r_bs = r_bs; a.H = n; a.W = n; a.dil = L.dil; a.nchunks = L.nchunks; a.relu = relu;
  dim3 grid((unsigned)n, (unsigned)B);
  if (L.cout == 64) hipLaunchKernelGGL((conv2d_3x3_kernel<64>), grid, dim3(512), 0, ctx->stream, a);
  else hipLaunchKernelGGL((conv2d_3x3_kernel<32>), grid, dim3(512), 0, ctx->stream, a);
  LAUNCHCHECK("conv2d_3x3_kernel");
  return ORCA_OK;
}

template <class F>
static void m16_variant(int mode, int cout, F f) {
  auto by_cout = [&](auto ns, auto dt) {
    if (cout == 64) f(std::integral_constant<int, 64>(), ns, dt);
    else f(std::integral_constant<int, 32>(), ns, dt);
  };
  if (mode == 1) by_cout(std::integral_constant<int, 1>(), std::integral_constant<int, 0>());
  else if (mode == 2) by_cout(std::integral_constant<int, 1>(), std::integral_constant<int, 1>());
  else by_cout(std::integral_constant<int, 2>(), std::integral_constant<int, 1>());
}

int launch_conv2d_m16(orca_ctx* ctx, const ConvLayer& L, const f32x4* x, long x_bs, int x_oct, f32x4* y, long y_bs, int y_oct,
                             const f32x4* r, long r_bs, int B, int n, int relu, int mode, int chunk0, int nchunks_,
                             const float* tab, long tab_bs) {
  const bool bf16 = mode == 1;
  if (L.ksize != 3 || !L.d_wf16 || !L.d_wb16p) return fail(ORCA_EINVAL, "launch_conv2d_m16 on a layer without a 16-bit pack");
  if (!bf16 && !L.f16_ok) return fail(ORCA_EINVAL, "layer weights exceed the fp16 range");
  if (L.dil > 8) return fail(ORCA_EINVAL, "conv2d_3x3_m16_kernel handles dilations 1-8 (got %d); larger ones run as fused blocks", L.dil);
  ConvM16Args a;
  a.x = x; a.w = bf16 ? L.d_wb16p : L.d_wf16; a.bias = L.d_bias; a.y = y; a.r = r; a.x_bs = x_bs; a.y_bs = y_bs; a.r_bs = r_bs;
  a.H = n; a.W = n; a.dil = L.dil; a.nchunks = nchunks_ > 0 ? nchunks_ : (L.cin + 15) / 16; a.relu = relu; a.flag = ctx->d_flag;
  a.tab = tab; a.tab_bs = tab_bs;
  if (chunk0 > 0) a.w = static_cast<const char*>(a.w) + (size_t)chunk0 * (bf16 ? 1 : 2) * 9 * 2 * L.cout * 8 * 2;
  if (a.nchunks * 2 > x_oct) return fail(ORCA_EINVAL, "conv2d_m16: input map has %d channel octets, layer needs %d", x_oct, a.nchunks * 2);
  if (L.cout / 8 > y_oct) return fail(ORCA_EINVAL, "conv2d_m16: output map narrower than the layer");
  if (B >= 2) {
    ConvM16QArgs aq;
    aq.c = a; aq.c.banded = 0; aq.zero = reinterpret_cast<const f32x4*>(ctx->d_zero);
    aq.ngroups = ((n + 4 * L.dil - 1) / (4 * L.dil)) * L.dil;
    aq.nb = B;
    const int ncu = device_cus();
    const int gx = (aq.ngroups * 2 + 7) / 8 * 8;
    int gy = B;
    const int res = (mode != 0 && L.cout == 32) ? 2 * ncu : ncu;
    if (a.nchunks % 2 == 0 && gx * B > res) gy = res / gx > 1 ? res / gx : 1;
    if (gy > B) gy = B;
    dim3 gridq((unsigned)gx, (unsigned)gy);
    m16_variant(mode, L.cout, [&](auto co, auto ns, auto dt) {
      hipLaunchKernelGGL((conv2d_3x3_m16q_kernel<decltype(co)::value, decltype(ns)::value, decltype(dt)::value>), gridq, dim3(512), 0, ctx->stream, aq);
    });
    LAUNCHCHECK("conv2d_3x3_m16q_kernel");
    return ORCA_OK;
  }
  a.banded = n >= 64 ? 1 : 0;
  dim3 grid((unsigned)(a.banded ? 8 * ((n + 7) / 8) : n), (unsigned)B);
  m16_variant(mode, L.cout, [&](auto co, auto ns, auto dt) {
    hipLaunchKernelGGL((conv2d_3x3_m16_kernel<decltype(co)::value, decltype(ns)::value, decltype(dt)::value>), grid, dim3(512), 0, ctx->stream, a);
  });
  LAUNCHCHECK("conv2d_3x3_m16_kernel");
  return ORCA_OK;
}

template <int NS, int DT>
int launch_dblocks(orca_ctx* ctx, f32x4* cur, long bs, int B, int n, const ConvLayer* p, int nblk) {
  if (nblk < 1 || nblk > (NS == 2 && DT == 1 ? 3 : 1)) return fail(ORCA_EINVAL, "launch_dblocks: %d blocks in one launch", nblk);
  DBlockArgs a{};
  a.cur = cur; a.bs = bs; a.H = n; a.W = n; a.dil = p[0].dil; a.nblk = nblk; a.flag = ctx->d_flag;
  for (int k = 0; k < 4 * nblk; ++k) {
    const int dil = a.dil << (k >> 2);
    if (!(dil == 16 || dil == 32 || dil == 64) || p[k].dil != dil) return fail(ORCA_EINVAL, "decoder block: dilation %d unsupported", p[k].dil);
    if (DT == 1 && !p[k].f16_ok) return fail(ORCA_EINVAL, "layer weights exceed the fp16 range");
    a.w[k] = DT == 0 ? p[k].d_wb16p : p[k].d_wf16;
    a.bias[k] = p[k].d_bias;
  }
  if (nblk == 1) {
    hipLaunchKernelGGL((conv2d_dblock_kernel<NS, DT>), dim3(256, (unsigned)B), dim3(512), 0, ctx->stream, a);
    LAUNCHCHECK("conv2d_dblock_kernel");
  } else if constexpr (NS == 2 && DT == 1) {
    hipLaunchKernelGGL((conv2d_dblock_run_kernel<2, 1>), dim3(256, (unsigned)B), dim3(512), 0, ctx->stream, a);
    LAUNCHCHECK("conv2d_dblock_run_kernel");
  }
  return ORCA_OK;
}
template int launch_dblocks<2, 1>(orca_ctx*, f32x4*, long, int, int, const ConvLayer*, int);
template int launch_dblocks<1, 0>(orca_ctx*, f32x4*, long, int, int, const ConvLayer*, int);
template int launch_dblocks<1, 1>(orca_ctx*, f32x4*, long, int, int, const ConvLayer*, int);

struct RowSrc {
  const float* base = nullptr;
  long bs = 0;
  const float* const* rows = nullptr;
  const float* at(int b) const { return rows ? rows[b] : (base ? base + (long)b * bs : nullptr); }
  explicit operator bool() const { return rows || base; }
};

static FinalArgs final_args(const orca_net* net, const float* cur, long cur_bs, float* out, int n, int accumulate) {
  const ConvLayer& fa = net->convs[net->convs.size() - 2];
  const ConvLayer& fb = net->convs[net->convs.size() - 1];
  FinalArgs a;
  a.cur = cur; a.w1 = fa.d_w; a.b1 = fa.d_bias; a.w2 = fb.d_w; a.b2 = fb.d_bias; a.out = out;
  a.cur_bs = cur_bs; a.out_bs = (long)net->num_2d * n * n; a.n = n; a.accumulate = accumulate;
  a.T = net->num_2d; a.F = fa.cout;
  return a;
}

struct DecoderProbe {
  int stage, channels;
  float* out;
};

template <class P>
struct DecMaps {
  P* p;
  long bs;
  int oct;
};
constexpr int DEC_STOP = 1;

template <class M, class Conv>
static int residual_block(Conv& conv, const ConvLayer* p, const M& cur, const M& oth, const M& T) {
  ORCA_TRY(conv(p[0], cur, T, nullptr, 0));
  ORCA_TRY(conv(p[1], T, oth, &cur, 0));
  ORCA_TRY(conv(p[2], oth, T, nullptr, 1));
  return conv(p[3], T, cur, &oth, 1);
}

template <class M, class Conv, class Block>
static int decoder_chain(const orca_net* net, bool with_y, const M& IN, const M& A, const M& Bf, const M& Cf, const M& Df, const M& T, Conv conv,
                         Block block, M* last) {
  const bool is1m = net->kind == ORCA_NET_DECODER_1M;
  const ConvLayer* L = net->convs.data();
  const ConvLayer* pairs = is1m ? L : L + 8;
  const int npairs = is1m ? 19 : 28;
  if (!is1m) {
    ORCA_TRY(conv(L[0], IN, Bf, nullptr, 0));
    ORCA_TRY(conv(L[1], Bf, Cf, nullptr, 0));
    ORCA_TRY(conv(L[2], Cf, Bf, nullptr, 1));
    ORCA_TRY(conv(L[3], Bf, A, &Cf, 1));
  }
  if (!is1m && with_y) {
    ORCA_TRY(conv(L[4], A, Bf, nullptr, 0));
    ORCA_TRY(conv(L[5], Bf, Cf, nullptr, 0));
    ORCA_TRY(conv(L[6], Cf, Bf, nullptr, 1));
    ORCA_TRY(conv(L[7], Bf, Df, &Cf, 1));
  } else {
    ORCA_TRY(conv(pairs[0], is1m ? IN : A, T, nullptr, 0));
    ORCA_TRY(conv(pairs[1], T, Cf, nullptr, 0));
    ORCA_TRY(conv(pairs[2], Cf, T, nullptr, 1));
    ORCA_TRY(conv(pairs[3], T, Df, &Cf, 1));
  }
  for (int i = 1; i < npairs; ++i) ORCA_TRY(block(i, Df, Cf));
  *last = Df;
  return ORCA_OK;
}

template <int NS, int DT>
static int decoder_m16(orca_ctx* ctx, orca_net* net, const RowSrc& x, long sx_c, long sx_l, const RowSrc& de,
                       long sd_c, long sd_h, long sd_w, const RowSrc& y, long sy_c, long sy_h, long sy_w, int B, int n,
                       float* out, int accumulate, const DecoderProbe* probe = nullptr) {
  typedef DecMaps<f32x4> M;
  const int nt2 = net->num_2d;
  const bool is1m = net->kind == ORCA_NET_DECODER_1M;
  const int mode = DT == 0 ? 1 : (NS == 1 ? 2 : 0);
  const int oIN = is1m ? 16 : 2, oA = 10;
  const size_t tabsz = (size_t)2 * 3 * n * 64;
  const size_t upo = (size_t)NS * n * ORCA_LDW;
  const size_t szIN = upo * oIN, szA = upo * oA, sz64 = upo * 8, sz32 = upo * 4;
  const size_t need = ru256(B * szIN * 16) + ru256(B * szA * 16) + 3 * ru256(B * sz64 * 16) + ru256(B * sz32 * 16) + ru256(B * tabsz * 4);
  ORCA_TRY(ws_ensure(ctx, need));
  auto take = [&](size_t units, int oct) { return M{reinterpret_cast<f32x4*>(ws_take(ctx, B * units * 4)), (long)units, oct}; };
  float* const TAB = is1m ? nullptr : ws_take(ctx, B * tabsz);
  const M IN = take(szIN, oIN), A = take(szA, oA), Bf = take(sz64, 8), Cf = take(sz64, 8), Df = take(sz64, 8), T = take(sz32, 4);
  hipStream_t s = ctx->stream;
  auto emit = [&](const M& m) -> int {
    for (int b = 0; b < B; ++b)
      hipLaunchKernelGGL((m16_to_nchw_kernel<NS, DT>), dim3((unsigned)n), dim3(ORCA_LDW), 0, s, m.p + b * m.bs, probe->channels, n,
                         probe->out + (size_t)b * probe->channels * n * n);
    LAUNCHCHECK("m16_to_nchw_kernel");
    return DEC_STOP;
  };
#define PROBE(k, m) \
  if (probe && probe->stage == (k)) return emit(m)
  for (int c0 = 0; c0 < B; c0 += 8) {
    const int nc = B - c0 < 8 ? B - c0 : 8;
    M16HeadArgs ha{};
    for (int b = 0; b < nc; ++b) { ha.x[b] = x.at(c0 + b); ha.de[b] = de.at(c0 + b); ha.y[b] = (!is1m && y) ? y.at(c0 + b) : nullptr; }
    ha.sx_c = sx_c; ha.sx_l = sx_l; ha.sd_c = sd_c; ha.sd_h = sd_h; ha.sd_w = sd_w; ha.sy_c = sy_c; ha.sy_h = sy_h; ha.sy_w = sy_w;
    ha.in = IN.p + c0 * szIN; ha.in_bs = (long)szIN;
    ha.tab = is1m ? nullptr : TAB + c0 * tabsz; ha.tab_bs = (long)tabsz;
    ha.a = A.p + c0 * szA; ha.a_bs = (long)szA;
    ha.wsep = net->d_sep; ha.nt = nt2; ha.n = n; ha.o0 = is1m ? 0 : 16; ha.noct = oIN; ha.nsep = is1m ? 0 : 6;
    ha.bilinear = net->upsample_mode == ORCA_UPSAMPLE_BILINEAR ? 1 : 0; ha.flag = ctx->d_flag;
    const unsigned roles = (unsigned)(oIN + ha.nsep + ((!is1m && y) ? 1 : 0));
    hipLaunchKernelGGL((decoder_head_m16_kernel<NS, DT>), dim3((unsigned)n, roles, (unsigned)nc), dim3(256), 0, s, ha);
    LAUNCHCHECK("decoder_head_m16_kernel");
  }
  const auto stop = [](int rc) { return rc == DEC_STOP ? ORCA_OK : rc; };
  if (probe && probe->stage == 0) return stop(emit(IN));
  const ConvLayer* L = net->convs.data();
  const ConvLayer* pairs = is1m ? L : L + 8;
  const int npairs = is1m ? 19 : 28;
  auto conv = [&](const ConvLayer& l, const M& src, const M& dst, const M* res, int relu) -> int {
    const bool sep = !is1m && &l == L;
    ORCA_TRY(launch_conv2d_m16(ctx, l, src.p, src.bs, src.oct, dst.p, dst.bs, dst.oct, res ? res->p : nullptr, res ? res->bs : 0, B, n, relu, mode,
                               sep ? 8 : 0, sep ? 1 : 0, sep ? TAB : nullptr, sep ? (long)tabsz : 0));
    if (sep) PROBE(1, dst);
    if (!is1m && &l == L + 3) PROBE(2, dst);
    return ORCA_OK;
  };
  int run_end = 0;
  auto block = [&](int i, const M& cur, const M& oth) -> int {
    if (i < run_end) return ORCA_OK;
    PROBE(3 + i - 1, cur);
    const ConvLayer* p = pairs + 4 * i;
    if (p[0].dil < 16) return residual_block(conv, p, cur, oth, T);
    int nblk = 1;
    if constexpr (NS == 2 && DT == 1) {
      bool is_run = net->dec_block_runs && p[0].dil == 16 && i + 2 < npairs && !(probe && (probe->stage == 3 + i || probe->stage == 3 + i + 1));
      for (int k = 0; is_run && k < 12; ++k) is_run = p[k].dil == 16 << (k >> 2);
      if (is_run) nblk = 3;
    }
    run_end = i + nblk;
    return launch_dblocks<NS, DT>(ctx, cur.p, cur.bs, B, n, p, nblk);
  };
  M cur;
  int rc = decoder_chain(net, (bool)y, IN, A, Bf, Cf, Df, T, conv, block, &cur);
  if (rc == ORCA_OK && probe && probe->stage == 3 + npairs - 1) rc = emit(cur);
#undef PROBE
  if (rc != ORCA_OK) return stop(rc);
  const FinalArgs fa = final_args(net, reinterpret_cast<const float*>(cur.p), cur.bs, out, n, accumulate);
  hipLaunchKernelGGL((final_sym_m16_kernel<NS, DT>), dim3(136u, (unsigned)B), dim3(256), 0, s, fa);
  LAUNCHCHECK("final_sym_m16_kernel");
  return ORCA_OK;
}

static int decoder_common(orca_ctx* ctx, orca_net* net, const RowSrc& x, long sx_c, long sx_l, const RowSrc& de,
                          long sd_c, long sd_h, long sd_w, const RowSrc& y, long sy_c, long sy_h, long sy_w,
                          int B, int n, float* out, int accumulate, const DecoderProbe* probe = nullptr) {
  const int nt2 = net->num_2d;
  if (n <= 0 || n > ORCA_LDW || (n & 1)) return fail(ORCA_EINVAL, "map size %d unsupported (even, <=256)", n);
  if (B <= 0) return ORCA_OK;
  HIPCHECK(hipSetDevice(ctx->device));
  if (net->precision == ORCA_PRECISION_F16X2)
    return decoder_m16<2, 1>(ctx, net, x, sx_c, sx_l, de, sd_c, sd_h, sd_w, y, sy_c, sy_h, sy_w, B, n, out, accumulate, probe);
  if (net->precision == ORCA_PRECISION_BF16)
    return decoder_m16<1, 0>(ctx, net, x, sx_c, sx_l, de, sd_c, sd_h, sd_w, y, sy_c, sy_h, sy_w, B, n, out, accumulate, probe);
  if (net->precision == ORCA_PRECISION_F16)
    return decoder_m16<1, 1>(ctx, net, x, sx_c, sx_l, de, sd_c, sd_h, sd_w, y, sy_c, sy_h, sy_w, B, n, out, accumulate, probe);
  if (probe) return fail(ORCA_EINVAL, "orca_decoder_probe: an f32 net has no M16 stages (its convs are conv2d_3x3_kernel)");
  typedef DecMaps<float> M;
  const bool is1m = net->kind == ORCA_NET_DECODER_1M;
  const size_t plane = (size_t)n * ORCA_LDW;
  const int cin0 = is1m ? 128 : 136;
  const size_t szIN = plane * cin0, szA = plane * 72, sz64 = plane * 64, sz32 = plane * 32;
  const size_t need = ru256(B * szIN * 4) + ru256(B * szA * 4) + 3 * ru256(B * sz64 * 4) + ru256(B * sz32 * 4);
  ORCA_TRY(ws_ensure(ctx, need));
  auto take = [&](size_t floats) { return M{ws_take(ctx, B * floats), (long)floats, 0}; };
  const M IN = take(szIN), A = take(szA), Bf = take(sz64), Cf = take(sz64), Df = take(sz64), T = take(sz32);
  hipStream_t s = ctx->stream;
  for (int b = 0; b < B; ++b) {
    hipLaunchKernelGGL(outer_sum_kernel, dim3((unsigned)n, (unsigned)cin0), dim3(64), 0, s, x.at(b), sx_c, sx_l,
                       de.at(b), sd_c, sd_h, sd_w, nt2, IN.p + b * szIN, n, cin0);
    LAUNCHCHECK("outer_sum_kernel");
  }
  const ConvLayer* L = net->convs.data();
  auto conv = [&](const ConvLayer& l, const M& src, const M& dst, const M* res, int relu) -> int {
    ORCA_TRY(launch_conv2d(ctx, l, src.p, src.bs, dst.p, dst.bs, res ? res->p : nullptr, res ? res->bs : 0, B, n, relu));
    if (is1m || !y || &l != L + 3) return ORCA_OK;
    for (int b = 0; b < B; ++b) {
      hipLaunchKernelGGL(upsample2d_x2_kernel, dim3((unsigned)n, 8), dim3(ORCA_LDW), 0, s, y.at(b), sy_c, sy_h, sy_w, nt2,
                         A.p + b * szA + 64 * plane, n, net->upsample_mode == ORCA_UPSAMPLE_BILINEAR ? 1 : 0, 8);
      LAUNCHCHECK("upsample2d_x2_kernel");
    }
    return ORCA_OK;
  };
  const ConvLayer* pairs = is1m ? L : L + 8;
  auto block = [&](int i, const M& cur, const M& oth) -> int { return residual_block(conv, pairs + 4 * i, cur, oth, T); };
  M cur;
  ORCA_TRY(decoder_chain(net, (bool)y, IN, A, Bf, Cf, Df, T, conv, block, &cur));
  const FinalArgs fa = final_args(net, cur.p, cur.bs, out, n, accumulate);
  hipLaunchKernelGGL(final_sym_kernel, dim3((unsigned)n, (unsigned)B), dim3(256), 0, s, fa);
  LAUNCHCHECK("final_sym_kernel");
  return ORCA_OK;
}

extern "C" int orca_decoder_forward(orca_ctx* ctx, orca_net* net, const float* x, int64_t sx_b, int64_t sx_c, int64_t sx_l,
                                    const float* distenc, int64_t sd_b, int64_t sd_h, int64_t sd_w, const float* y,
                                    int64_t sy_b, int64_t sy_h, int64_t sy_w, int B, int n, float* out, int accumulate) {
  if (!ctx || !net || !x || !distenc || !out) return fail(ORCA_EINVAL, "orca_decoder_forward: NULL argument");
  if (net->kind != ORCA_NET_DECODER) return fail(ORCA_EINVAL, "orca_decoder_forward: net is not a Decoder");
  if (net->num_2d != 1) return fail(ORCA_EINVAL, "orca_decoder_forward: net predicts %d maps, use orca_decoder_forward_mt", net->num_2d);
  RowSrc xs, ds, ys;
  xs.base = x; xs.bs = sx_b; ds.base = distenc; ds.bs = sd_b; ys.base = y; ys.bs = sy_b;
  return decoder_common(ctx, net, xs, sx_c, sx_l, ds, 0, sd_h, sd_w, ys, 0, sy_h, sy_w, B, n, out, accumulate);
}

extern "C" int orca_decoder_forward_mt(orca_ctx* ctx, orca_net* net, const float* x, int64_t sx_b, int64_t sx_c, int64_t sx_l,
                                       const float* distenc, int64_t sd_b, int64_t sd_c, int64_t sd_h, int64_t sd_w, const float* y,
                                       int64_t sy_b, int64_t sy_c, int64_t sy_h, int64_t sy_w, int B, int n, float* out,
                                       int accumulate) {
  if (!ctx || !net || !x || !distenc || !out) return fail(ORCA_EINVAL, "orca_decoder_forward_mt: NULL argument");
  if (net->kind != ORCA_NET_DECODER) return fail(ORCA_EINVAL, "orca_decoder_forward_mt: net is not a Decoder");
  RowSrc xs, ds, ys;
  xs.base = x; xs.bs = sx_b; ds.base = distenc; ds.bs = sd_b; ys.base = y; ys.bs = sy_b;
  return decoder_common(ctx, net, xs, sx_c, sx_l, ds, sd_c, sd_h, sd_w, ys, sy_c, sy_h, sy_w, B, n, out, accumulate);
}

extern "C" int orca_decoder_forward_rows(orca_ctx* ctx, orca_net* net, const float* const* x_rows, int64_t sx_c, int64_t sx_l,
                                         const float* const* distenc_rows, int64_t sd_c, int64_t sd_h, int64_t sd_w,
                                         const float* const* y_rows, int64_t sy_c, int64_t sy_h, int64_t sy_w, int B, int n, float* out,
                                         int accumulate) {
  if (!ctx || !net || !x_rows || !distenc_rows || !out) return fail(ORCA_EINVAL, "orca_decoder_forward_rows: NULL argument");
  if (net->kind != ORCA_NET_DECODER) return fail(ORCA_EINVAL, "orca_decoder_forward_rows: net is not a Decoder");
  for (int b = 0; b < B; ++b)
    if (!x_rows[b] || !distenc_rows[b] || (y_rows && !y_rows[b])) return fail(ORCA_EINVAL, "orca_decoder_forward_rows: NULL row pointer %d", b);
  RowSrc xs, ds, ys;
  xs.rows = x_rows; ds.rows = distenc_rows; ys.rows = y_rows;
  return decoder_common(ctx, net, xs, sx_c, sx_l, ds, sd_c, sd_h, sd_w, ys, sy_c, sy_h, sy_w, B, n, out, accumulate);
}

extern "C" int orca_decoder1m_forward_rows(orca_ctx* ctx, orca_net* net, const float* const* x_rows, int64_t sx_c, int64_t sx_l, int B, int n,
                                           float* out, int accumulate) {
  if (!ctx || !net || !x_rows || !out) return fail(ORCA_EINVAL, "orca_decoder1m_forward_rows: NULL argument");
  if (net->kind != ORCA_NET_DECODER_1M) return fail(ORCA_EINVAL, "orca_decoder1m_forward_rows: net is not a Decoder_1m");
  for (int b = 0; b < B; ++b)
    if (!x_rows[b]) return fail(ORCA_EINVAL, "orca_decoder1m_forward_rows: NULL row pointer %d", b);
  RowSrc xs, none;
  xs.rows = x_rows;
  return decoder_common(ctx, net, xs, sx_c, sx_l, none, 0, 0, 0, none, 0, 0, 0, B, n, out, accumulate);
}

extern "C" int orca_decoder1m_forward(orca_ctx* ctx, orca_net* net, const float* x, int64_t sx_b, int64_t sx_c, int64_t sx_l,
                                      int B, int n, float* out, int accumulate) {
  if (!ctx || !net || !x || !out) return fail(ORCA_EINVAL, "orca_decoder1m_forward: NULL argument");
  if (net->kind != ORCA_NET_DECODER_1M) return fail(ORCA_EINVAL, "orca_decoder1m_forward: net is not a Decoder_1m");
  RowSrc xs, none;
  xs.base = x; xs.bs = sx_b;
  return decoder_common(ctx, net, xs, sx_c, sx_l, none, 0, 0, 0, none, 0, 0, 0, B, n, out, accumulate);
}

extern "C" int orca_decoder_probe(orca_ctx* ctx, orca_net* net, const float* x, int64_t sx_b, int64_t sx_c, int64_t sx_l, const float* distenc,
                                  int64_t sd_b, int64_t sd_c, int64_t sd_h, int64_t sd_w, const float* y, int64_t sy_b, int64_t sy_c, int64_t sy_h,
                                  int64_t sy_w, int B, int n, int stage, int channels, float* map_out) {
  if (!ctx || !net || !x || !map_out) return fail(ORCA_EINVAL, "orca_decoder_probe: NULL argument");
  const bool is1m = net->kind == ORCA_NET_DECODER_1M;
  if (!is1m && net->kind != ORCA_NET_DECODER) return fail(ORCA_EINVAL, "orca_decoder_probe: net is neither a Decoder nor a Decoder_1m");
  if (is1m ? (distenc || y) : !distenc) return fail(ORCA_EINVAL, "orca_decoder_probe: a Decoder needs distenc, a Decoder_1m takes neither distenc nor y");
  const int last = 3 + (is1m ? 19 : 28) - 1;
  if (stage < 0 || stage > last || (is1m && (stage == 1 || stage == 2)))
    return fail(ORCA_EINVAL, "orca_decoder_probe: this net has no stage %d", stage);
  const int want = stage == 0 ? (is1m ? 128 : 16) : (stage == 2 && y ? 80 : 64);
  if (channels != want) return fail(ORCA_EINVAL, "orca_decoder_probe: stage %d has %d channels, got %d", stage, want, channels);
  const DecoderProbe probe{stage, channels, map_out};
  RowSrc xs, ds, ys;
  xs.base = x; xs.bs = sx_b; ds.base = distenc; ds.bs = sd_b; ys.base = y; ys.bs = sy_b;
  return decoder_common(ctx, net, xs, sx_c, sx_l, ds, sd_c, sd_h, sd_w, ys, sy_c, sy_h, sy_w, B, n, nullptr, 0, &probe);
}

extern "C" int orca_strand_merge(orca_ctx* ctx, const float* fwd, const float* rev, float* out, int n) {
  if (!ctx || !fwd || !rev || !out || n <= 0) return fail(ORCA_EINVAL, "orca_strand_merge: bad argument");
  HIPCHECK(hipSetDevice(ctx->device));
  hipLaunchKernelGGL(strand_merge_kernel, dim3((unsigned)((n * n + 255) / 256)), dim3(256), 0, ctx->stream, fwd, rev, out, n);
  LAUNCHCHECK("strand_merge_kernel");
  return ORCA_OK;
}

extern "C" int orca_block_mean_f64(orca_ctx* ctx, const double* mat, int64_t ld, int64_t row0, int64_t col0, int nb, int npix, double* mean_out,
                                   float* log_out, int flip) {
// ... 51 lines not shown
```

### orca_amd/csrc/orca_internal.h

```cpp
#pragma once
#include <hip/hip_runtime.h>

#include <cstdarg>
#include <cstdint>
#include <cstdio>
#include <cstdlib>
#include <cstring>
#include <string>
#include <vector>

#include "conv_kernels.h"
#include "orca_hip.h"

int fail(int code, const char* fmt, ...) __attribute__((format(printf, 2, 3)));

#define HIPCHECK(expr)                                                                          \
  do {                                                                                          \
    hipError_t _e = (expr);                                                                     \
    if (_e != hipSuccess) return fail(ORCA_EHIP, "%s failed: %s (%s:%d)", #expr, hipGetErrorString(_e), __FILE__, __LINE__); \
  } while (0)

#define LAUNCHCHECK(name)                                                                        \
  do {                                                                                          \
    hipError_t _e = hipGetLastError();                                                          \
    if (_e != hipSuccess) return fail(ORCA_EHIP, "launch of %s failed: %s", name, hipGetErrorString(_e)); \
  } while (0)

#define ORCA_TRY(expr)        \
  do {                        \
    int _rc = (expr);         \
    if (_rc != ORCA_OK) return _rc; \
  } while (0)

static inline long ru4(long v) { return (v + 3) & ~3L; }
static inline size_t ru256(size_t v) { return (v + 255) & ~size_t(255); }

struct TimedLaunch {
  orca_kernel_time rec;
  hipEvent_t e0, e1;
};

struct orca_ctx {
  int device = 0;
  hipStream_t stream = nullptr;
  char* ws = nullptr;
  size_t ws_bytes = 0;
  size_t ws_off = 0;
  hipStream_t ws_stream = nullptr;
  bool ws_used = false;
  bool timing = false;
  std::vector<TimedLaunch> timed;
  long long counts[4] = {0, 0, 0, 0};
  unsigned* d_flag = nullptr;
  float* d_edge = nullptr;
  float* d_zero = nullptr;
};

int ws_ensure(orca_ctx* ctx, size_t bytes);
float* ws_take(orca_ctx* ctx, size_t nfloats);
static inline int ws_three(orca_ctx* ctx, size_t nfloats, float* buf[3]) {
  const int rc = ws_ensure(ctx, 3 * ru256(nfloats * sizeof(float)));
  for (int i = 0; rc == ORCA_OK && i < 3; ++i) buf[i] = ws_take(ctx, nfloats);
  return rc;
}

#ifndef ORCA_MAX_TARGETS
#define ORCA_MAX_TARGETS 8
#endif
#define ORCA_EDGE_SLAB (40 * 128)

struct ConvLayer {
  int cin = 0, cout = 0, ksize = 0, dil = 1;
  int kc = 8, nchunks = 0;
  float* d_w = nullptr;
  float* d_bias = nullptr;
  void* d_wb16 = nullptr;
  void* d_wf16 = nullptr;
  void* d_wb16p = nullptr;
  bool f16_ok = true;
};

struct orca_net {
  orca_ctx* ctx = nullptr;
  int kind = 0;
  int precision = ORCA_PRECISION_F32;
  int dec_block_runs = 1;
  int enc_two_strands = 1;
  int enc_form = ORCA_ENCODER_FORM_DEFAULT;
  float* d_first_w = nullptr;
  void* d_first_w16 = nullptr;
  float* d_first_tab = nullptr;
  int upsample_mode = ORCA_UPSAMPLE_BILINEAR;
  int num_2d = 1;
  float* d_sep = nullptr;
  void* d_l1_w16 = nullptr;
  float* d_l1_bias = nullptr;
  void* d_c1a_w16 = nullptr;
  float* d_c1a_bias = nullptr;
  float* d_l1_f32 = nullptr;
  float* d_c1a_f32 = nullptr;
  float* d_l1_bias32 = nullptr;
  float* d_c1a_bias32 = nullptr;
  ConvLayer comp[3];
  std::vector<ConvLayer> convs;
};

int make_layer(const orca_conv_desc& d, ConvLayer* out);
int make_layer17(int cin, int cout, const std::vector<double>& w17, const std::vector<double>& b17, ConvLayer* out);
void compose_pair(const orca_conv_desc& c1, const orca_conv_desc& c2, std::vector<double>* w17, std::vector<double>* b17);
void free_layer(ConvLayer& L);

static inline int device_cus() {
  static int ncu = [] { int dev = 0, v = 256; (void)hipGetDevice(&dev); (void)hipDeviceGetAttribute(&v, hipDeviceAttributeMultiprocessorCount, dev); return v; }();
  return ncu;
}
template <auto KERNEL, int THREADS>
static int resident_workgroups() {
  static int resident = [] {
    int per_cu = 1;
    if (hipOccupancyMaxActiveBlocksPerMultiprocessor(&per_cu, KERNEL, THREADS, 0) != hipSuccess || per_cu < 1) { (void)hipGetLastError(); per_cu = 1; }
    return device_cus() * per_cu;
  }();
  return resident;
}
struct LaunchTimer {
  orca_ctx* ctx;
  bool on;
  TimedLaunch tl;
  LaunchTimer(orca_ctx* c, long n, bool wanted = true) : ctx(c), on(c->timing && n >= 65536 && wanted) {}
  int open() {
    if (!on) return ORCA_OK;
    HIPCHECK(hipEventCreate(&tl.e0));
    HIPCHECK(hipEventCreate(&tl.e1));
    HIPCHECK(hipEventRecord(tl.e0, ctx->stream));
    return ORCA_OK;
  }
  int close(int cout, int cin, int tile, int batch, long n, int ksize) {
    if (!on) return ORCA_OK;
    HIPCHECK(hipEventRecord(tl.e1, ctx->stream));
    tl.rec.cout = cout; tl.rec.cin = cin; tl.rec.tile = tile; tl.rec.batch = batch; tl.rec.n = n; tl.rec.ms = 0.f; tl.rec.ksize = ksize;
    ctx->timed.push_back(tl);
    return ORCA_OK;
  }
};

static inline bool al16(const void* p) { return (reinterpret_cast<uintptr_t>(p) & 15) == 0; }
static inline long p16_plen(long n) { return ((n + 512) / 512) * 512 + 32; }
struct FusedFirst;
struct P16Layout { long x_plen = 0, y_plen = 0, y_off = 0, n_valid = 0; };
int launch_conv1d(orca_ctx* ctx, const ConvLayer& L, const float* x, long x_bs, long ldx, float* y, long y_bs, long ldy, const float* r1, const float* r2,
                  int B, long n, int relu, int tile, int y_nlc = 0);
int launch_conv1d_b16(orca_ctx* ctx, const ConvLayer& L, int precision, const float* x, long x_bs, float* y, long y_bs, const float* r1, int B, long n, int relu,
                      int pool4 = 0, const float* r2 = nullptr, int fixed_tile = 0);
int launch_conv1d_p16(orca_ctx* ctx, const ConvLayer& L, const float* x, void* y, const float* r1, long n, int relu, int out_mode, const FusedFirst* f1 = nullptr,
                      int fmt = 0, const P16Layout* lay = nullptr);
int launch_p16_zero_pads(orca_ctx* ctx, float* base, int C, long n_valid, int fmt = 0, long plen = 0, long gap0 = 0, long gap1 = 0);
int launch_pool(orca_ctx* ctx, const float* x, long ldx, float* y, long ldy, long rows, long n_out, int k);
int launch_conv2d(orca_ctx* ctx, const ConvLayer& L, const float* x, long x_bs, float* y, long y_bs, const float* r, long r_bs, int B, int n, int relu);
int launch_conv2d_m16(orca_ctx* ctx, const ConvLayer& L, const f32x4* x, long x_bs, int x_oct, f32x4* y, long y_bs, int y_oct, const f32x4* r, long r_bs, int B,
                      int n, int relu, int mode, int chunk0 = 0, int nchunks_ = 0, const float* tab = nullptr, long tab_bs = 0);
template <int NS, int DT>
int launch_dblocks(orca_ctx* ctx, f32x4* cur, long bs, int B, int n, const ConvLayer* p, int nblk);
```

### orca_amd/engine.py

```python
import ctypes
import threading
import weakref

import numpy as np
import torch

from . import _lib
from ._lib import ConvDesc, OrcaHipError, check

BN_EPS = 1e-5


_tls = threading.local()


class Context:
    def __init__(self, device_index):
        lib = _lib.load()
        self.device_index = device_index
        self.handle = ctypes.c_void_p()
        stream = torch.cuda.current_stream(device_index).cuda_stream
        check(lib.orca_ctx_create(device_index, ctypes.c_void_p(stream), ctypes.byref(self.handle)), "orca_ctx_create")
        self._finalizer = weakref.finalize(self, lib.orca_ctx_destroy, self.handle)

    def sync_stream(self):
        stream = torch.cuda.current_stream(self.device_index).cuda_stream
        check(_lib.load().orca_ctx_set_stream(self.handle, ctypes.c_void_p(stream)), "orca_ctx_set_stream")

    def workspace_bytes(self):
        n = ctypes.c_size_t()
        check(_lib.load().orca_ctx_workspace_bytes(self.handle, ctypes.byref(n)))
        return n.value

    def take_overflow(self):
        f = ctypes.c_int()
        check(_lib.load().orca_ctx_take_overflow(self.handle, ctypes.byref(f)), "orca_ctx_take_overflow")
        return bool(f.value)

    def set_timing(self, enable):
        check(_lib.load().orca_ctx_set_timing(self.handle, 1 if enable else 0))

    def get_timing(self, max_records=4096):
        buf = (_lib.KernelTime * max_records)()
        n = ctypes.c_int()
        check(_lib.load().orca_ctx_get_timing(self.handle, buf, max_records, ctypes.byref(n)))
        return [(r.cout, r.cin, r.tile, r.batch, r.n, r.ms, r.ksize) for r in buf[: min(n.value, max_records)]]

    def launch_counts(self):
        c = (ctypes.c_int64 * 4)()
        check(_lib.load().orca_ctx_launch_counts(self.handle, c), "orca_ctx_launch_counts")
        return dict(zip(("conv_small", "conv_bf16s", "planar", "decoder_pairs"), [int(x) for x in c]))

    def release_workspace(self):
        check(_lib.load().orca_ctx_release_workspace(self.handle))


def get_context(device):
    if isinstance(device, torch.device):
        if device.type != "cuda":
            raise OrcaHipError(f"orca_amd runs on MI355X only; got a tensor on '{device}'. There is no CPU path.")
        idx = device.index if device.index is not None else torch.cuda.current_device()
    else:
        idx = int(device)
    ctx = getattr(_tls, "override", None)
    if ctx is None or ctx.device_index != idx:
        ctxs = getattr(_tls, "ctxs", None)
        if ctxs is None:
            ctxs = _tls.ctxs = {}
        if idx not in ctxs:
            ctxs[idx] = Context(idx)
        ctx = ctxs[idx]
    ctx.sync_stream()
    return ctx


import contextlib


class _GuardState(threading.local):
    defer = False
    force_safe = False

    def __getitem__(self, key):
        return getattr(self, key)

    def __setitem__(self, key, value):
        setattr(self, key, value)


_guard = _GuardState()


@contextlib.contextmanager
def _guard_scope(key, value):
    old = _guard[key]
    _guard[key] = value
    try:
        yield
    finally:
        _guard[key] = old


def defer_overflow_guard():
    return _guard_scope("defer", True)


def immediate_overflow_guard():
    return _guard_scope("defer", False)


def force_safe_precision():
    return _guard_scope("force_safe", True)


class ContextPool:

    def __init__(self, device, k):
        self.index = device.index if isinstance(device, torch.device) and device.index is not None else torch.cuda.current_device()
        self.streams = [torch.cuda.Stream(device=self.index) for _ in range(k)]
        self.ctxs = []
        for s in self.streams:
            with torch.cuda.stream(s):
                self.ctxs.append(Context(self.index))
        self._fork = torch.cuda.Event()
        self._join = [torch.cuda.Event() for _ in range(k)]
        self.side = torch.cuda.Stream(device=self.index)
        self._dirty = set()

    def __len__(self):
        return len(self.ctxs)

    def fork(self, stream=None):
        self._fork.record(stream or torch.cuda.current_stream(self.index))
        for s in self.streams:
            s.wait_event(self._fork)

    def run(self, i, fn):
# ... 63 lines not shown
    if lst is not None and _guard.defer and not _guard.force_safe:
        lst.append(undo)


def run_with_overflow_retry(fn, device, pool=None):
    if not (isinstance(device, torch.device) and device.type == "cuda"):
        return fn()
    ctx = get_context(device)
    outer, _tls.tentative = getattr(_tls, "tentative", None), []
    try:
        with defer_overflow_guard():
            out = fn()
        over = ctx.take_overflow()
        for p in ([pool] if pool is not None else []) + [q for q in _thread_pools().values() if q is not pool and q.index == ctx.device_index]:
            over = p.take_overflow() or over
        if over:
            import warnings
            warnings.warn("orca_amd: an activation left the fp16 range; recomputing with range-safe arithmetic (bf16x3 / f32)")
            for undo in _tls.tentative:
                undo()
            _tls.tentative = []
            with force_safe_precision():
                out = fn()
    finally:
        _tls.tentative = outer
    return out


def _np64(v):
    if isinstance(v, torch.Tensor):
        return v.detach().cpu().double().numpy()
    return np.asarray(v, dtype=np.float64)


def fold_conv(sd, conv, bn=None, dilation=1):
    w = _np64(sd[conv + ".weight"])
    b = _np64(sd[conv + ".bias"])
    if bn is not None:
        s = _np64(sd[bn + ".weight"]) / np.sqrt(_np64(sd[bn + ".running_var"]) + BN_EPS)
        w = w * s.reshape((-1,) + (1,) * (w.ndim - 1))
        b = (b - _np64(sd[bn + ".running_mean"])) * s + _np64(sd[bn + ".bias"])
    return {"w": np.ascontiguousarray(w, dtype=np.float32), "b": np.ascontiguousarray(b, dtype=np.float32),
            "cout": w.shape[0], "cin": w.shape[1], "k": w.shape[2], "dil": int(dilation)}


def make_descs(convs):
    arr = (ConvDesc * len(convs))()
    for i, c in enumerate(convs):
        arr[i].weight_host = c["w"].ctypes.data
        arr[i].bias_host = c["b"].ctypes.data
        arr[i].cout, arr[i].cin, arr[i].ksize, arr[i].dilation = c["cout"], c["cin"], c["k"], c["dil"]
    return arr


class Net:

    def __init__(self, ctx, kind, convs, upsample_mode=_lib.ORCA_UPSAMPLE_BILINEAR):
        lib = _lib.load()
        self.ctx, self.kind = ctx, kind
        self.handle = ctypes.c_void_p()
        descs = make_descs(convs)
        check(lib.orca_net_create(ctx.handle, kind, descs, len(convs), upsample_mode, ctypes.byref(self.handle)), "orca_net_create")
        self._finalizer = weakref.finalize(self, lib.orca_net_free, self.handle)

    def num_targets(self):
        if getattr(self, "_num_targets", None) is None:
            t = ctypes.c_int(0)
            check(_lib.load().orca_net_num_targets(self.handle, ctypes.byref(t)), "orca_net_num_targets")
            self._num_targets = int(t.value)
        return self._num_targets

    def set_precision(self, name):
        if name not in _lib.PRECISIONS:
            raise ValueError(f"precision must be one of {sorted(_lib.PRECISIONS)}, got {name!r}")
        check(_lib.load().orca_net_set_precision(self.handle, _lib.PRECISIONS[name]), "orca_net_set_precision")

    def set_encoder_form(self, name):
        if name not in _lib.ENCODER_FORMS:
            raise ValueError(f"form must be one of {sorted(_lib.ENCODER_FORMS)}, got {name!r}")
        check(_lib.load().orca_net_set_encoder_form(self.handle, _lib.ENCODER_FORMS[name]), "orca_net_set_encoder_form")

    def set_decoder_block_runs(self, on):
        check(_lib.load().orca_net_set_decoder_block_runs(self.handle, 1 if on else 0), "orca_net_set_decoder_block_runs")

    def set_encoder_two_strands(self, on):
        check(_lib.load().orca_net_set_encoder_two_strands(self.handle, 1 if on else 0), "orca_net_set_encoder_two_strands")

    def encoder_two_strands(self):
        on = ctypes.c_int(0)
        check(_lib.load().orca_net_get_encoder_two_strands(self.handle, ctypes.byref(on)), "orca_net_get_encoder_two_strands")
        return bool(on.value)


def _f32_cuda(t, name):
    if not isinstance(t, torch.Tensor):
        raise TypeError(f"{name} must be a torch.Tensor")
    if not t.is_cuda:
        raise OrcaHipError(f"{name} is on '{t.device}': orca_amd has no CPU path (move it to the MI355X with .cuda())")
    if t.dtype != torch.float32:
        t = t.float()
    return t


def _p(t):
    return ctypes.c_void_p(t.data_ptr())


def encoder_num_bins(L):
    return int(_lib.load().orca_encoder_num_bins(int(L)))


def encoder_forward(net, x, bin_lo=0, bin_hi=0, chunk_bp=0, out=None):
    x = _f32_cuda(x, "x")
    if x.dim() != 3 or x.shape[1] != 4:
        raise ValueError(f"Encoder input must be [B,4,L], got {tuple(x.shape)}")
    B, _, L = x.shape
    total = encoder_num_bins(L)
    hi = total if bin_hi <= 0 else bin_hi
    if out is None:
        out = torch.empty((B, 128, hi - bin_lo), dtype=torch.float32, device=x.device)
    net.ctx.sync_stream()
    check(_lib.load().orca_encoder_forward(net.ctx.handle, net.handle, _p(x), x.stride(0), x.stride(1), x.stride(2), B, L,
                                           bin_lo, hi, _p(out), out.stride(0), out.stride(1), chunk_bp), "orca_encoder_forward")
    return out


def pack_sequence(x):
    x = _f32_cuda(x, "x")
    B, C, L = x.shape
    if C != 4:
        raise ValueError(f"sequence must be [B,4,L], got {tuple(x.shape)}")
    codes = torch.empty((B, L), dtype=torch.uint8, device=x.device)
    ctx = get_context(x.device)
    ok = True
    for b in range(B):
        flag = ctypes.c_int()
        check(_lib.load().orca_pack_sequence(ctx.handle, ctypes.c_void_p(x[b].data_ptr()), x.stride(1), x.stride(2), L,
                                             ctypes.c_void_p(codes[b].data_ptr()), ctypes.byref(flag)), "orca_pack_sequence")
        ok = ok and bool(flag.value)
    return codes, ok


class CodeWindow:

    def __init__(self, codes, origin, L):
        self.codes, self.origin, self.L = codes, int(origin), int(L)

    @property
    def shape(self):
        return (self.codes.shape[0], self.L)

    device = property(lambda self: self.codes.device)
    dtype = property(lambda self: self.codes.dtype)


def code_window_range(L, bin_lo, bin_hi, reverse=False, halo=112000, binsize=4000):
    total = encoder_num_bins(L)
    lo = max(0, bin_lo * binsize - halo)
    hi = L if bin_hi >= total else min(L, bin_hi * binsize + halo)
    return (L - hi, L - lo) if reverse else (lo, hi)


def encoder_forward_codes(net, codes, reverse=False, bin_lo=0, bin_hi=0, chunk_bp=0, out=None):
    win = codes if isinstance(codes, CodeWindow) else None
    if win is not None:
        codes = win.codes
# ... 485 lines not shown
def unet_forward(net, x, nlev):
    x = _f32_cuda(x, "x")
    if x.dim() != 3 or x.shape[1] != 128:
        raise ValueError(f"Encoder2/3 input must be [B,128,n], got {tuple(x.shape)}")
    B, _, n = x.shape
    outs = [torch.empty((B, 128, n >> i), dtype=torch.float32, device=x.device) for i in range(nlev + 1)]
    ptrs = (ctypes.c_void_p * (nlev + 1))(*[o.data_ptr() for o in outs])
    net.ctx.sync_stream()
    check(_lib.load().orca_unet_forward(net.ctx.handle, net.handle, _p(x), x.stride(0), x.stride(1), x.stride(2), B, n, ptrs,
                                        nlev + 1), "orca_unet_forward")
    return outs


def decoder_forward(net, x, distenc, y=None, out=None, accumulate=False):
    x = _f32_cuda(x, "x")
    distenc = _f32_cuda(distenc, "distenc")
    B, C, n = x.shape
    T = net.num_targets()
    if C != 128:
        raise ValueError(f"Decoder input must be [B,128,n], got {tuple(x.shape)}")
    if distenc.dim() != 4 or distenc.shape[1] != T or distenc.shape[2] != n or distenc.shape[3] != n:
        raise ValueError(f"distenc must be [B,{T},{n},{n}], got {tuple(distenc.shape)}")
    if distenc.shape[0] not in (1, B):
        raise ValueError("distenc batch mismatch")
    sd_b = distenc.stride(0) if distenc.shape[0] == B else 0
    yp, sy = ctypes.c_void_p(0), (0, 0, 0, 0)
    if y is not None:
        y = _f32_cuda(y, "y")
        if tuple(y.shape) != (B, T, n // 2, n // 2):
            raise ValueError(f"coarse prediction must be [{B},{T},{n // 2},{n // 2}], got {tuple(y.shape)}")
        yp, sy = _p(y), (y.stride(0), y.stride(1), y.stride(2), y.stride(3))
    if out is None:
        out = torch.empty((B, T, n, n), dtype=torch.float32, device=x.device)
        accumulate = False
    elif tuple(out.shape) != (B, T, n, n) or not out.is_contiguous():
        raise ValueError(f"out must be a contiguous [{B},{T},{n},{n}] tensor")
    net.ctx.sync_stream()
    if T == 1:
        check(_lib.load().orca_decoder_forward(net.ctx.handle, net.handle, _p(x), x.stride(0), x.stride(1), x.stride(2), _p(distenc),
                                               sd_b, distenc.stride(2), distenc.stride(3), yp, sy[0], sy[2], sy[3], B, n, _p(out),
                                               1 if accumulate else 0), "orca_decoder_forward")
    else:
        check(_lib.load().orca_decoder_forward_mt(net.ctx.handle, net.handle, _p(x), x.stride(0), x.stride(1), x.stride(2),
                                                  _p(distenc), sd_b, distenc.stride(1), distenc.stride(2), distenc.stride(3), yp,
                                                  sy[0], sy[1], sy[2], sy[3], B, n, _p(out), 1 if accumulate else 0),
              "orca_decoder_forward_mt")
    return out


def _row_ptrs(rows):
    return (ctypes.c_void_p * len(rows))(*[r.data_ptr() for r in rows])


def _same_strides(rows, name):
    st = rows[0].stride()
    if any(r.stride() != st or r.shape != rows[0].shape for r in rows):
        raise ValueError(f"{name}: the rows of a batch must share one shape and one set of strides")
    return st


def decoder_forward_rows(net, xs, des, ys=None, out=None, accumulate=False):
    xs = [_f32_cuda(t, "x") for t in xs]
    des = [_f32_cuda(t, "distenc") for t in des]
    B, T = len(xs), net.num_targets()
    C, n = xs[0].shape
    if C != 128 or tuple(des[0].shape) != (T, n, n) or len(des) != B:
        raise ValueError(f"decoder rows: x [128,n] and distenc [{T},n,n] per row, got {tuple(xs[0].shape)} / {tuple(des[0].shape)}")
    sx, sd = _same_strides(xs, "x"), _same_strides(des, "distenc")
    yp, sy = None, (0, 0, 0)
    if ys is not None:
        ys = [_f32_cuda(t, "y") for t in ys]
        if len(ys) != B or tuple(ys[0].shape) != (T, n // 2, n // 2):
            raise ValueError(f"coarse prediction rows must be [{T},{n // 2},{n // 2}]")
        yp, sy = _row_ptrs(ys), _same_strides(ys, "y")
    if out is None:
        out = torch.empty((B, T, n, n), dtype=torch.float32, device=xs[0].device)
        accumulate = False
    net.ctx.sync_stream()
    check(_lib.load().orca_decoder_forward_rows(net.ctx.handle, net.handle, _row_ptrs(xs), sx[0], sx[1], _row_ptrs(des), sd[0], sd[1], sd[2],
                                                yp, sy[0], sy[1], sy[2], B, n, _p(out), 1 if accumulate else 0), "orca_decoder_forward_rows")
    return out


def decoder1m_forward_rows(net, xs, out=None, accumulate=False):
    xs = [_f32_cuda(t, "x") for t in xs]
    B, T = len(xs), net.num_targets()
    C, n = xs[0].shape
    sx = _same_strides(xs, "x")
    if out is None:
        out = torch.empty((B, T, n, n), dtype=torch.float32, device=xs[0].device)
        accumulate = False
    net.ctx.sync_stream()
    check(_lib.load().orca_decoder1m_forward_rows(net.ctx.handle, net.handle, _row_ptrs(xs), sx[0], sx[1], B, n, _p(out), 1 if accumulate else 0),
          "orca_decoder1m_forward_rows")
    return out


def decoder1m_forward(net, x, out=None, accumulate=False):
    x = _f32_cuda(x, "x")
    B, C, n = x.shape
    T = net.num_targets()
    if C != 128:
        raise ValueError(f"Decoder_1m input must be [B,128,n], got {tuple(x.shape)}")
    if out is None:
        out = torch.empty((B, T, n, n), dtype=torch.float32, device=x.device)
        accumulate = False
    elif tuple(out.shape) != (B, T, n, n) or not out.is_contiguous():
        raise ValueError(f"out must be a contiguous [{B},{T},{n},{n}] tensor")
    net.ctx.sync_stream()
    check(_lib.load().orca_decoder1m_forward(net.ctx.handle, net.handle, _p(x), x.stride(0), x.stride(1), x.stride(2), B, n,
                                             _p(out), 1 if accumulate else 0), "orca_decoder1m_forward")
    return out


def decoder_probe(net, x, distenc, y, stage):
    x = _f32_cuda(x, "x")
    B, C, n = x.shape
    if C != 128:
        raise ValueError(f"Decoder input must be [B,128,n], got {tuple(x.shape)}")
    is1m = net.kind == _lib.ORCA_NET_DECODER_1M
    T = net.num_targets()
    dp, sd, yp, sy = ctypes.c_void_p(0), (0, 0, 0, 0), ctypes.c_void_p(0), (0, 0, 0, 0)
    if distenc is not None:
        distenc = _f32_cuda(distenc, "distenc")
        if distenc.dim() != 4 or tuple(distenc.shape[1:]) != (T, n, n) or distenc.shape[0] not in (1, B):
            raise ValueError(f"distenc must be [B or 1,{T},{n},{n}], got {tuple(distenc.shape)}")
        dp, sd = _p(distenc), (distenc.stride(0) if distenc.shape[0] == B else 0, distenc.stride(1), distenc.stride(2), distenc.stride(3))
    if y is not None:
        y = _f32_cuda(y, "y")
        if tuple(y.shape) != (B, T, n // 2, n // 2):
            raise ValueError(f"coarse prediction must be [{B},{T},{n // 2},{n // 2}], got {tuple(y.shape)}")
        yp, sy = _p(y), (y.stride(0), y.stride(1), y.stride(2), y.stride(3))
    channels = (128 if is1m else 16) if stage == 0 else (80 if stage == 2 and y is not None else 64)
    out = torch.empty((B, channels, n, n), dtype=torch.float32, device=x.device)
    net.ctx.sync_stream()
    check(_lib.load().orca_decoder_probe(net.ctx.handle, net.handle, _p(x), x.stride(0), x.stride(1), x.stride(2), dp, *sd, yp, *sy, B, n,
                                         int(stage), channels, _p(out)), "orca_decoder_probe")
    return out


def strand_merge(fwd, rev):
    fwd, rev = _f32_cuda(fwd, "fwd").contiguous(), _f32_cuda(rev, "rev").contiguous()
    n = fwd.shape[-1]
    out = torch.empty_like(fwd)
    ctx = get_context(fwd.device)
    check(_lib.load().orca_strand_merge(ctx.handle, _p(fwd), _p(rev), _p(out), n), "orca_strand_merge")
    return out


def block_mean(normmat, start, nb, npix=250, flip=False, want_mean=True):
    if not (normmat.is_cuda and normmat.dtype == torch.float64 and normmat.dim() == 2 and normmat.stride(1) == 1):
        raise OrcaHipError("block_mean: a float64 [n,n] ROCm tensor with unit column stride is required")
    if start < 0 or start + npix * nb > min(normmat.shape):
        raise ValueError(f"block_mean: window [{start}, {start + npix * nb}) outside the {tuple(normmat.shape)} background")
    ctx = get_context(normmat.device)
    ctx.sync_stream()
    mean = torch.empty((npix, npix), dtype=torch.float64, device=normmat.device) if want_mean else None
    logt = torch.empty((1, 1, npix, npix), dtype=torch.float32, device=normmat.device)
    check(_lib.load().orca_block_mean_f64(ctx.handle, _p(normmat), normmat.stride(0), int(start), int(start), int(nb), int(npix),
                                          _p(mean) if mean is not None else None, _p(logt), 1 if flip else 0), "orca_block_mean_f64")
    return mean, logt


def conv1d(x, w, b, relu=False, r1=None, r2=None, tile=0):
    x = _f32_cuda(x, "x").contiguous()
    B, cin, n = x.shape
# ... 132 lines not shown
```

### orca_amd/orca_modules.py

```python
import os

import numpy as np
import torch
from torch import nn

from . import _lib, engine

ENCODER_CHANNELS = (64, 96, 128, 128, 128, 128, 128)
ENCODER_POOLS = (1, 4, 4, 5, 5, 5, 2)
DECODER_DILATIONS = tuple([1, 2, 4, 8, 16, 32, 64] * 4)
DECODER1M_DILATIONS = tuple([1, 2, 4, 8, 16, 32, 64] + [2, 4, 8, 16, 32, 64] * 2)


def _linear_pair(conv, bn, cin, cmid, cout, lead=None, **kw):
    mods = [] if lead is None else [lead]
    mods += [conv(cin, cmid, **kw), bn(cmid), conv(cmid, cout, **kw), bn(cout)]
    return nn.Sequential(*mods)


def _relu_pair(conv, bn, cin, cmid, cout, second_bn=True, **kw):
    mods = [conv(cin, cmid, **kw), bn(cmid), nn.ReLU(inplace=True), conv(cmid, cout, **kw)]
    if second_bn:
        mods.append(bn(cout))
    mods.append(nn.ReLU(inplace=True))
# ... 249 lines not shown

    def _conv_items(self):
        items = []
        for i in range(5):
            items += [(f"lblocks.{i}", self.lblocks[i], 1), (f"blocks.{i}", self.blocks[i], 1)]
        return items

    def forward(self, x):
        net = self._net(x.device)
        return self._run_guarded(net, lambda: engine.unet_forward(net, x, 5), "bf16x3")


class Encoder3(_UNetEncoder):
    _kind = _lib.ORCA_NET_ENCODER3
    _nlev = 3


def _c2(d):
    return dict(kernel_size=(3, 3), padding=d, dilation=d)


MAX_TARGETS = 8


def _final_head(num_2d=1):
    hidden = num_2d if num_2d > 5 else 5
    return nn.Sequential(nn.Conv2d(64, hidden, kernel_size=(1, 1), padding=0), nn.BatchNorm2d(hidden), nn.ReLU(inplace=True),
                         nn.Conv2d(hidden, num_2d, kernel_size=(1, 1), padding=0))


def _check_num_2d(num_2d):
    if not (isinstance(num_2d, int) and 1 <= num_2d <= MAX_TARGETS):
        raise ValueError(f"num_2d must be an int in 1..{MAX_TARGETS}, got {num_2d!r}")
    return num_2d


class Decoder(_HipModule):

    _kind = _lib.ORCA_NET_DECODER

    def __init__(self, upsample_mode="nearest", precision=None, num_2d=1):
        super().__init__()
        self.num_2d = _check_num_2d(num_2d)
        self.precision = precision or os.environ.get("ORCA_DECODER_PRECISION", "f16x2")
        if self.precision not in ("f16x2", "f32", "bf16", "f16"):
            raise ValueError("Decoder precision must be 'f16x2', 'f32', 'bf16' or 'f16'")
        if upsample_mode not in ("nearest", "bilinear"):
            raise ValueError("upsample_mode must be 'nearest' or 'bilinear'")
        self._upsample = _lib.ORCA_UPSAMPLE_BILINEAR if upsample_mode == "bilinear" else _lib.ORCA_UPSAMPLE_NEAREST
        self.lconvtwos = nn.ModuleList([
            _linear_pair(nn.Conv2d, nn.BatchNorm2d, 64, 32, 64, nn.Dropout(p=0.1) if i == 0 else None, **_c2(d))
            for i, d in enumerate(DECODER_DILATIONS)])
        self.convtwos = nn.ModuleList([_relu_pair(nn.Conv2d, nn.BatchNorm2d, 64, 32, 64, **_c2(d)) for d in DECODER_DILATIONS])
        self.final = _final_head(num_2d)
        self.upsample = nn.Upsample(scale_factor=(2, 2), mode=upsample_mode)
        self.lcombiner = _linear_pair(nn.Conv2d, nn.BatchNorm2d, 64 + num_2d, 64, 64, nn.Dropout(p=0.1), **_c2(1))
        self.combiner = _relu_pair(nn.Conv2d, nn.BatchNorm2d, 64, 64, 64, **_c2(1))
        self.lcombinerD = _linear_pair(nn.Conv2d, nn.BatchNorm2d, 128 + num_2d, 64, 64, **_c2(1))
        self.combinerD = _relu_pair(nn.Conv2d, nn.BatchNorm2d, 64, 64, 64, **_c2(1))

    def _conv_items(self):
        items = [("lcombinerD", self.lcombinerD, 1), ("combinerD", self.combinerD, 1),
                 ("lcombiner", self.lcombiner, 1), ("combiner", self.combiner, 1)]
        for i, d in enumerate(DECODER_DILATIONS):
            items += [(f"lconvtwos.{i}", self.lconvtwos[i], d), (f"convtwos.{i}", self.convtwos[i], d)]
        items.append(("final", self.final, 1))
        return items

    def forward(self, x, distenc, y=None):
        net = self._net(x.device)
        return self._run_guarded(net, lambda: engine.decoder_forward(net, x, distenc, y), "f32")

    def forward_into(self, out, x, distenc, y=None, accumulate=False):
        net = self._net(x.device)
        if accumulate and self.precision in ("f16x2", "f16"):
            base = out.clone()
            return self._run_guarded(net, lambda: engine.decoder_forward(net, x, distenc, y, out=out.copy_(base), accumulate=True), "f32")
        return self._run_guarded(net, lambda: engine.decoder_forward(net, x, distenc, y, out=out, accumulate=accumulate), "f32")

    def forward_rows(self, xs, distencs, ys=None):
        net = self._net(xs[0].device)
        return self._run_guarded(net, lambda: engine.decoder_forward_rows(net, xs, distencs, ys), "f32")


class Decoder_1m(_HipModule):

    _kind = _lib.ORCA_NET_DECODER_1M

    def __init__(self, precision=None, num_2d=1):
        super().__init__()
        self.num_2d = _check_num_2d(num_2d)
        self.precision = precision or os.environ.get("ORCA_DECODER_PRECISION", "f16x2")
        if self.precision not in ("f16x2", "f32", "bf16", "f16"):
            raise ValueError("Decoder_1m precision must be 'f16x2', 'f32', 'bf16' or 'f16'")
        self.lconvtwos = nn.ModuleList([
            _linear_pair(nn.Conv2d, nn.BatchNorm2d, 128 if i == 0 else 64, 32, 64, nn.Dropout(p=0.1) if i == 0 else None, **_c2(d))
            for i, d in enumerate(DECODER1M_DILATIONS)])
        self.convtwos = nn.ModuleList([_relu_pair(nn.Conv2d, nn.BatchNorm2d, 64, 32, 64, **_c2(d)) for d in DECODER1M_DILATIONS])
        self.final = _final_head(num_2d)

    def _conv_items(self):
        items = []
        for i, d in enumerate(DECODER1M_DILATIONS):
            items += [(f"lconvtwos.{i}", self.lconvtwos[i], d), (f"convtwos.{i}", self.convtwos[i], d)]
        items.append(("final", self.final, 1))
        return items

    def forward(self, x):
        net = self._net(x.device)
        return self._run_guarded(net, lambda: engine.decoder1m_forward(net, x), "f32")

    def forward_into(self, out, x, accumulate=False):
        net = self._net(x.device)
        if accumulate and self.precision in ("f16x2", "f16"):
            base = out.clone()
            return self._run_guarded(net, lambda: engine.decoder1m_forward(net, x, out=out.copy_(base), accumulate=True), "f32")
        return self._run_guarded(net, lambda: engine.decoder1m_forward(net, x, out=out, accumulate=accumulate), "f32")

    def forward_rows_into(self, out, xs, accumulate=False):
        net = self._net(xs[0].device)
        if accumulate and self.precision in ("f16x2", "f16"):
            base = out.clone()
            return self._run_guarded(net, lambda: engine.decoder1m_forward_rows(net, xs, out=out.copy_(base), accumulate=True), "f32")
        return self._run_guarded(net, lambda: engine.decoder1m_forward_rows(net, xs, out=out, accumulate=accumulate), "f32")


class Net(nn.Module):

    def __init__(self, num_1d=None, precision=None, num_2d=1):
        super().__init__()
        enc, dec = Encoder(precision), Decoder_1m(num_2d=num_2d)
        self.num_2d = num_2d
        for name, child in list(enc.named_children()) + list(dec.named_children()):
            self.add_module(name, child)
        if num_1d is not None:
            self.final_1d = nn.Sequential(nn.Conv1d(128, 128, kernel_size=1, padding=0), nn.BatchNorm1d(128), nn.ReLU(inplace=True),
                                          nn.Conv1d(128, num_1d, kernel_size=1, padding=0), nn.Sigmoid())
        self.num_1d = num_1d
        object.__setattr__(self, "_enc", enc)
        object.__setattr__(self, "_dec", dec)
        self._head1d = {}

    @property
    def precision(self):
        return self._enc.precision

    @precision.setter
    def precision(self, name):
        self._enc.precision = name

    def _invalidate(self):
        self._enc.invalidate()
        self._dec.invalidate()
        self._head1d = {}

    def _apply(self, fn, *a, **k):
        self._invalidate()
        return super()._apply(fn, *a, **k)

    def load_state_dict(self, state_dict, *a, **k):
        self._invalidate()
        own = set(self.state_dict().keys())
        fixed = {}
        for key, v in state_dict.items():
            kk = key
            while kk not in own and kk.startswith("module."):
# ... 23 lines not shown
```

### orca_amd/orca_predict.py

```python
import os

import numpy as np
import torch

from . import engine

model_dict_global = {}


def load_resources(models=("32M",), use_cuda=True, model_dir=None):
    from . import orca_models
    if "32M" in models:
        for key, cls in (("h1esc", orca_models.H1esc), ("hff", orca_models.Hff)):
            if key not in model_dict_global:
                model_dict_global[key] = cls(model_dir=model_dir)
    if "256M" in models:
        for key, cls in (("h1esc_256m", orca_models.H1esc_256M), ("hff_256m", orca_models.Hff_256M)):
            if key not in model_dict_global:
                model_dict_global[key] = cls(model_dir=model_dir)
    if "1M" in models or "1m" in models:
        for key, cls in (("h1esc_1m", orca_models.H1esc_1M), ("hff_1m", orca_models.Hff_1M)):
            if key not in model_dict_global:
                model_dict_global[key] = cls(model_dir=model_dir)
    if use_cuda:
# ... 232 lines not shown
            if hit is not None and flip in hit[2]:
                return hit[2][flip]
            mean, logt = engine.block_mean(self.normmat, start, nb, 250, flip, want_mean=hit is None)
            if hit is None:
                self.ns[k][level] = hit = (start, mean, {})
            hit[2][flip] = logt
            return logt
        if hit is None:
            w = 250 * nb
            self.ns[k][level] = hit = (start, _coarse_grain(self.normmat[None, start: start + w, start: start + w], nb, 1))
        return _log_background(hit[1], 1, self.use_cuda, flip=flip)


def _scale_annotation(annotation, newstart, newend):
    span = newend - newstart
    out = []
    for r in annotation:
        if len(r) == 3:
            if not (r[0] >= newend or r[1] <= newstart):
                out.append((np.fmax((r[0] - newstart) / span, 0), np.fmin((r[1] - newstart) / span, 1), r[2]))
        elif newstart <= r[0] < newend:
            out.append(((r[0] - newstart) / span, r[1]))
    return out


def zoom_index_32m(level, start, mpos, wpos, reverse):
    half = level * 1000000 / 4
    if not reverse:
        v = np.floor(((mpos - half) - (wpos - 16000000 + start * 4000)) / (4000 * level))
    else:
        v = np.ceil(((wpos + 16000000 - start * 4000) - (mpos + half)) / (4000 * level))
    return int(np.clip(v, 0, 125))


def zoom_index_256m(level, start, mpos, wpos, chrlen, reverse):
    half = level * 1000000 / 4
    if not reverse:
        proposed = (mpos - half) - (wpos - 128000000 + start * 32000)
    else:
        proposed = (mpos - half) - (wpos + 128000000 - start * 32000 - level * 1000000)
    if chrlen is not None:
        lo = 0 - (wpos - 128000000)
        hi = chrlen - level * 1000000 / 2 - (wpos - 128000000)
        proposed = np.clip(proposed, lo, hi) if lo < hi else lo
    i = int(np.clip(np.floor(proposed / (4000 * level)), 0, 125))
    return 250 - (i + 125) if reverse else i


def _rows(t, B, idx, width, dims):
    out = []
    for k, i in enumerate(idx):
        for b in range(B):
            sl = t[k * B + b]
            for d in dims:
                sl = sl.narrow(d - 1, i, width)
            out.append(sl)
    return out


def _gather(t, B, idx, width, dims):
    parts = []
    for k, i in enumerate(idx):
        sl = t[k * B:(k + 1) * B]
        for d in dims:
            sl = sl.narrow(d, i, width)
        parts.append(sl)
    return parts[0] if len(parts) == 1 else torch.cat(parts, dim=0)


def run_cascade(model, encodings, levels, unit, B, reverse_flags, background, zoom, add_1m_level=None, on_level=None):
    S = len(reverse_flags)
    starts = [[0] for _ in range(S)]
    zoom_idx = [0] * S
    preds = []
    for j, level in enumerate(levels):
        u = unit(level)
        sl = [int(starts[k][j] / u) for k in range(S)]
        bgs = [background(level, k, starts[k][j]) for k in range(S)]
        dec = model.denets[level]
        if hasattr(dec, "forward_rows") and encodings[level].is_cuda:
            xs = _rows(encodings[level], B, sl, 250, (2,))
            des = [bgs[k][b if bgs[k].shape[0] > 1 else 0] for k in range(S) for b in range(B)]
            ys = _rows(preds[j - 1], B, zoom_idx, 125, (2, 3)) if j > 0 else None
            pred = dec.forward_rows(xs, des, ys)
            if level == add_1m_level:
                model.denet_1_pt.forward_rows_into(pred, xs, accumulate=True)
            preds.append(pred)
        else:
            enc = _gather(encodings[level], B, sl, 250, (2,))
            if all(b is bgs[0] for b in bgs):
                distenc = bgs[0].expand(S * B, -1, -1, -1)
            else:
                distenc = torch.cat([b.expand(B, -1, -1, -1) for b in bgs], dim=0)
            coarse = _gather(preds[j - 1], B, zoom_idx, 125, (2, 3)) if j > 0 else None
            preds.append(_decode(model, level, enc, distenc, coarse, level == add_1m_level))
        if on_level is not None:
            on_level(j, level, [starts[k][j] for k in range(S)])
        for k in range(S):
            zoom_idx[k] = (zoom[k] if isinstance(zoom, (list, tuple)) else zoom)(level, starts[k][j], reverse_flags[k])
            starts[k].append(starts[k][j] + zoom_idx[k] * u)
    return preds, [st[:-1] for st in starts]


def cascade_32m(model, xs, mpos, wpos, reverse_flags, distencs=None, merge=False):
    B = xs[0].shape[0]
    cache = {}

    def background(level, k, start):
        if distencs is not None:
            return distencs[level]
        if level not in cache:
            cache[level] = _cached_log_background(model, level, xs[0].is_cuda)
        return cache[level]

    def forward():
        def encode(x, rev, out=None):
            return model.net0.forward_codes(x, reverse=rev, out=out) if x.dtype == torch.uint8 else model.net0(x)
        if len(xs) > 1 and all(x.dtype == torch.uint8 for x in xs) and hasattr(model.net0, "_net"):
            enc0 = torch.empty((len(xs) * B, 128, engine.encoder_num_bins(xs[0].shape[1])), dtype=torch.float32, device=xs[0].device)
            if len(xs) == 2 and xs[0] is xs[1] and list(reverse_flags) == [False, True]:
                _encode_two_strands(lambda rev, out: encode(xs[0], rev, out), enc0, B, _joint_encode(model.net0, xs[0]))
            else:
                for k, (x, r) in enumerate(zip(xs, reverse_flags)):
                    encode(x, r, enc0[k * B:(k + 1) * B])
        else:
            enc0 = torch.cat([encode(x, r) for x, r in zip(xs, reverse_flags)], dim=0) if len(xs) > 1 else encode(xs[0], reverse_flags[0])
        encodings = dict(zip([1, 2, 4, 8, 16, 32], model.net(enc0)))
        preds, starts = run_cascade(model, encodings, [32, 16, 8, 4, 2, 1], lambda lv: lv, B, list(reverse_flags), background,
                                    lambda lv, st, rev: zoom_index_32m(lv, st, mpos, wpos, rev), add_1m_level=1)
        return (preds, starts, _merge_device(preds, B)) if merge else (preds, starts)

    return engine.run_with_overflow_retry(forward, xs[0].device)


def starts_32m(mpos, wpos, reverse):
    st = [0]
    for level in [32, 16, 8, 4, 2, 1]:
        st.append(st[-1] + zoom_index_32m(level, st[-1], mpos, wpos, reverse) * level)
    return st[:-1]


def denet1m_32m_from_enc(model, enc0, mpos, wpos, reverse_flags):
    S = len(reverse_flags)
    B = enc0.shape[0] // S

    def forward():
        enc1 = model.net(enc0)[0]
        xs = []
        for k in range(S):
            s = int(starts_32m(mpos, wpos, bool(reverse_flags[k]))[5])
            xs.append(enc1[k * B: (k + 1) * B, :, s: s + 250])
        return model.denet_1_pt(torch.cat(xs, dim=0).contiguous())

    return engine.run_with_overflow_retry(forward, enc0.device)


def cascade_32m_from_enc(model, enc0, mpos, wpos, reverse_flags, distencs=None, with_1m=True):
    S = len(reverse_flags)
    B = enc0.shape[0] // S
    cache = {}

    def background(level, k, start):
        if distencs is not None:
            return distencs[level]
        if level not in cache:
            cache[level] = _cached_log_background(model, level, enc0.is_cuda)
        return cache[level]

    def forward():
# ... 171 lines not shown
```

Before: 1014 Mb/s.

## Run the 1M decoder alongside the level decoder in shared batched launches

Adds a combined decoder path where the level decoder and the Decoder_1m run in the same conv and dilated-block kernel launches. Batch entries past a split index select a second weight and bias set. The goal is to fill the grid better and halve the number of launches for the residual trunk at the level that adds the 1M prediction, instead of running the two nets one after the other. The cost is a larger kernel argument struct, per-batch weight selection inside the kernels, and a fallback to the old sequential path if fp16 overflows.

```diff
diff --git a/include/orca_hip.h b/include/orca_hip.h
--- a/include/orca_hip.h
+++ b/include/orca_hip.h
@@ -51,6 +51,7 @@
 int orca_ctx_set_stream(orca_ctx* ctx, void* hip_stream);
 int orca_ctx_workspace_bytes(orca_ctx* ctx, size_t* out);
 int orca_ctx_release_workspace(orca_ctx* ctx);
+int orca_ctx_fill_workspace(orca_ctx* ctx, size_t bytes, int value);
 
 typedef struct orca_kernel_time {
   int32_t cout, cin, tile, batch;
@@ -80,6 +81,7 @@
 #define ORCA_ENCODER_FORM_TWO_CONV 3
 int orca_net_set_encoder_form(orca_net* net, int form);
 int orca_net_set_decoder_block_runs(orca_net* net, int on);
+int orca_net_set_decoder_with_1m(orca_net* net, int on);
 int orca_net_set_encoder_two_strands(orca_net* net, int on);
 int orca_net_get_encoder_two_strands(orca_net* net, int* on);
 int orca_ctx_take_overflow(orca_ctx* ctx, int* flag);
@@ -179,6 +181,9 @@
                               float* out, int accumulate);
 int orca_decoder1m_forward_rows(orca_ctx* ctx, orca_net* net, const float* const* x_rows, int64_t sx_c, int64_t sx_l,
                                 int B, int n, float* out, int accumulate);
+int orca_decoder_forward_rows_with_1m(orca_ctx* ctx, orca_net* net, orca_net* net_1m, const float* const* x_rows, int64_t sx_c, int64_t sx_l,
+                                      const float* const* distenc_rows, int64_t sd_c, int64_t sd_h, int64_t sd_w,
+                                      const float* const* y_rows, int64_t sy_c, int64_t sy_h, int64_t sy_w, int B, int n, float* out);
 
 int orca_decoder1m_forward(orca_ctx* ctx, orca_net* net, const float* x, int64_t sx_b, int64_t sx_c,
                            int64_t sx_l, int B, int n, float* out, int accumulate);
diff --git a/orca_amd/_lib.py b/orca_amd/_lib.py
--- a/orca_amd/_lib.py
+++ b/orca_amd/_lib.py
@@ -34,6 +34,7 @@
     "orca_ctx_set_stream": (c_int, [c_void_p, c_void_p]),
     "orca_ctx_workspace_bytes": (c_int, [c_void_p, POINTER(c_size_t)]),
     "orca_ctx_release_workspace": (c_int, [c_void_p]),
+    "orca_ctx_fill_workspace": (c_int, [c_void_p, c_size_t, c_int]),
     "orca_ctx_take_overflow": (c_int, [c_void_p, POINTER(c_int)]),
     "orca_ctx_set_timing": (c_int, [c_void_p, c_int]),
     "orca_ctx_get_timing": (c_int, [c_void_p, POINTER(KernelTime), c_int, POINTER(c_int)]),
@@ -43,6 +44,7 @@
     "orca_net_set_precision": (c_int, [c_void_p, c_int]),
     "orca_net_set_encoder_form": (c_int, [c_void_p, c_int]),
     "orca_net_set_decoder_block_runs": (c_int, [c_void_p, c_int]),
+    "orca_net_set_decoder_with_1m": (c_int, [c_void_p, c_int]),
     "orca_net_set_encoder_two_strands": (c_int, [c_void_p, c_int]),
     "orca_net_get_encoder_two_strands": (c_int, [c_void_p, POINTER(c_int)]),
     "orca_encoder_forward_two_strands": (c_int, [c_void_p, c_void_p, c_void_p, c_int64, c_void_p, c_void_p, c_int64]),
@@ -97,6 +99,8 @@
     "orca_decoder_forward_rows": (c_int, [c_void_p, c_void_p, POINTER(c_void_p), c_int64, c_int64, POINTER(c_void_p), c_int64, c_int64, c_int64,
                                           POINTER(c_void_p), c_int64, c_int64, c_int64, c_int, c_int, c_void_p, c_int]),
     "orca_decoder1m_forward_rows": (c_int, [c_void_p, c_void_p, POINTER(c_void_p), c_int64, c_int64, c_int, c_int, c_void_p, c_int]),
+    "orca_decoder_forward_rows_with_1m": (c_int, [c_void_p, c_void_p, c_void_p, POINTER(c_void_p), c_int64, c_int64, POINTER(c_void_p), c_int64, c_int64,
+                                                  c_int64, POINTER(c_void_p), c_int64, c_int64, c_int64, c_int, c_int, c_void_p]),
     "orca_net_num_targets": (c_int, [c_void_p, POINTER(c_int)]),
     "orca_decoder1m_forward": (c_int, [c_void_p, c_void_p, c_void_p, c_int64, c_int64, c_int64, c_int, c_int, c_void_p, c_int]),
     "orca_decoder_probe": (c_int, [c_void_p, c_void_p, c_void_p, c_int64, c_int64, c_int64, c_void_p, c_int64, c_int64, c_int64, c_int64, c_void_p,
diff --git a/orca_amd/csrc/conv2d_dblock.h b/orca_amd/csrc/conv2d_dblock.h
--- a/orca_amd/csrc/conv2d_dblock.h
+++ b/orca_amd/csrc/conv2d_dblock.h
@@ -3,11 +3,12 @@
 
 struct DBlockArgs {
   f32x4* cur;
-  const void* w[12];
-  const float* bias[12];
+  const void* w[24];
+  const float* bias[24];
   long bs;
   int H, W, dil, nblk;
   unsigned* flag;
+  int split;
 };
 
 #ifndef DBLOCK_STORE_WT
@@ -49,6 +50,7 @@
   const int lS = 8 - ld, S = 1 << lS;
   const int lG = 2 * ld - 8, G = 1 << lG;
   f32x4* const cur = a.cur + (long)blockIdx.y * a.bs;
+  const int set = (a.split > 0 && (int)blockIdx.y >= a.split) ? 12 : 0;
 
   int bx = (int)blockIdx.x;
   if (!(ABL & 64)) {
@@ -74,7 +76,7 @@
 #pragma unroll
     for (int b = 0; b < MAXBLK; ++b)
       if (b < nblk) {
-        const float *b0 = a.bias[4 * b], *b1 = a.bias[4 * b + 1], *b2 = a.bias[4 * b + 2], *b3 = a.bias[4 * b + 3];
+        const float *b0 = a.bias[set + 4 * b], *b1 = a.bias[set + 4 * b + 1], *b2 = a.bias[set + 4 * b + 2], *b3 = a.bias[set + 4 * b + 3];
         const float* src = lane < 8 ? b0 + 4 * lane : (lane < 24 ? b1 + 4 * (lane - 8) : (lane < 32 ? b2 + 4 * (lane - 24) : b3 + 4 * (lane - 32)));
         p16_glds16(reinterpret_cast<const f32x4*>(src), smem + AU + BU + 3 * WP + 48 * b);
       }
@@ -105,7 +107,7 @@
         const int plane = s_ * 8 + 2 * k + (wave >> 2);
         if (!(ABL & 4)) p16_glds16(cur + m16_plane(plane & 7, s_, NS, H) + off, As + plane * PXW + (wave & 3) * 64);
       }
-      if (k < 3) issue_piece(a.w[0], k, k * WP);
+      if (k < 3) issue_piece(a.w[set], k, k * WP);
     }
   }
 
@@ -205,7 +207,7 @@
     const bool first = b == 0, last = MAXBLK == 1 || b + 1 == nblk;
     const void* wb[5];
 #pragma unroll
-    for (int q = 0; q < 5; ++q) wb[q] = a.w[4 * b + (q < 4 || !last ? q : 0)];
+    for (int q = 0; q < 5; ++q) wb[q] = a.w[set + 4 * b + (q < 4 || !last ? q : 0)];
     const float* const bl = bias_s + 192 * b;
     unsigned nb16[9];
 #pragma unroll
diff --git a/orca_amd/csrc/conv2d_m16q.h b/orca_amd/csrc/conv2d_m16q.h
--- a/orca_amd/csrc/conv2d_m16q.h
+++ b/orca_amd/csrc/conv2d_m16q.h
@@ -7,6 +7,9 @@
   const f32x4* zero;
   int ngroups;
   int nb;
+  const void* w2;
+  const float* bias2;
+  int split;
 };
 
 __device__ __forceinline__ float m16_hl_lo(unsigned h, unsigned l) {
@@ -187,22 +190,23 @@
   auto issue_x1 = [&](const f32x4* xm, int k, int buf, int it) {
     if (it + 1 < XIT || wave < XFULL) p16_glds16(xoff[it] >= 0 ? xm + m16_plane(2 * k, 0, NS, H) + xoff[it] : aq.zero, Xs + buf * XB + it * NT + wave * 64);
   };
-  auto issue_w1 = [&](int i, int slot, int it) {
+  auto issue_w1 = [&](const void* wm, int i, int slot, int it) {
     const int k = i / NH, h = i - k * NH;
     const int u = tid + it * NT;
     if (it + 1 < WIT || wave < WFULL)
-      p16_glds16(reinterpret_cast<const f32x4*>(a.w) + ((long)k * (WNS * 9 * 2) + (u >> 5)) * COUT + h * 32 + (u & 31), Ws + slot * WP + it * NT + wave * 64);
+      p16_glds16(reinterpret_cast<const f32x4*>(wm) + ((long)k * (WNS * 9 * 2) + (u >> 5)) * COUT + h * 32 + (u & 31), Ws + slot * WP + it * NT + wave * 64);
   };
   auto issue_x = [&](const f32x4* xm, int k, int buf) {
 #pragma unroll
     for (int it = 0; it < XIT; ++it) issue_x1(xm, k, buf, it);
   };
-  auto issue_w = [&](int i, int slot) {
-#pragma unroll
-    for (int it = 0; it < WIT; ++it) issue_w1(i, slot, it);
-  };
-
-  issue_w(0, 0);
+  auto issue_w = [&](const void* wm, int i, int slot) {
+#pragma unroll
+    for (int it = 0; it < WIT; ++it) issue_w1(wm, i, slot, it);
+  };
+  auto second = [&](int m) { return aq.split > 0 && m >= aq.split; };
+
+  issue_w(second(b) ? aq.w2 : a.w, 0, 0);
   issue_x(xb, 0, 0);
   M16Q_STAMP(1);
   const unsigned ws_lds = p16_lds_addr(Ws + g * 32 + l31);
@@ -214,6 +218,9 @@
   while (true) {
   const bool has_next = b + bstep < nb;
   const f32x4* const xb_next = xb + (long)bstep * a.x_bs;
+  const void* const w_cur = second(b) ? aq.w2 : a.w;
+  const void* const w_next = second(b + bstep) ? aq.w2 : a.w;
+  const float* const bias_cur = second(b) ? aq.bias2 : a.bias;
 
   f32x16 acc[2][NH];
   int gb_ = g;
@@ -222,7 +229,7 @@
   for (int h = 0; h < NH; ++h)
 #pragma unroll
     for (int q = 0; q < 4; ++q) {
-      const f32x4 b4 = *reinterpret_cast<const f32x4*>(a.bias + h * 32 + 8 * q + 4 * gb_);
+      const f32x4 b4 = *reinterpret_cast<const f32x4*>(bias_cur + h * 32 + 8 * q + 4 * gb_);
 #pragma unroll
       for (int j = 0; j < 2; ++j) { acc[j][h][4 * q + 0] = b4.x; acc[j][h][4 * q + 1] = b4.y; acc[j][h][4 * q + 2] = b4.z; acc[j][h][4 * q + 3] = b4.w; }
     }
@@ -273,17 +280,18 @@
     const bool dox = (LASTP ? (NH == 1 && has_next) : (h == 0 && (lastk ? (NH == 2 && has_next) : true))) && !(M16Q_ABL & 8);
     const int i_nx = LASTP ? 0 : i + 1, k_nx = (LASTP || lastk) ? 0 : k + 1;
     const f32x4* const x_nx = (LASTP || lastk) ? xb_next : xb;
+    const void* const w_nx = LASTP ? w_next : w_cur;
     static_assert(WIT + XIT <= 10, "transfer slots of a piece");
 #define M16Q_DMA_SLOT(n_)                                                                              \
   {                                                                                                    \
     const int first_ = (n_) == 0 ? 0 : (n_) + 1, cnt_ = (n_) == 0 ? 2 : 1;                              \
     _Pragma("unroll") for (int q_ = first_; q_ < first_ + cnt_; ++q_) {                                 \
-      if (q_ < WIT) { if (dow) issue_w1(i_nx, (i + 1) & 1, q_); }                                       \
+      if (q_ < WIT) { if (dow) issue_w1(w_nx, i_nx, (i + 1) & 1, q_); }                                  \
       else if (q_ - WIT < XIT) { if (dox) issue_x1(x_nx, k_nx, (k + 1) & 1, q_ - WIT); }                \
     }                                                                                                  \
   }
     if (!M16Q_SPREAD) {
-      if (dow) issue_w(i_nx, (i + 1) & 1);
+      if (dow) issue_w(w_nx, i_nx, (i + 1) & 1);
       if (dox) issue_x(x_nx, k_nx, (k + 1) & 1);
     }
     const unsigned wrow = ws_lds + (unsigned)((i & 1) * WP * 16);
diff --git a/orca_amd/csrc/orca_core.hip b/orca_amd/csrc/orca_core.hip
--- a/orca_amd/csrc/orca_core.hip
+++ b/orca_amd/csrc/orca_core.hip
@@ -363,6 +363,14 @@
 extern "C" int orca_ctx_workspace_bytes(orca_ctx* ctx, size_t* out) {
   if (!ctx || !out) return fail(ORCA_EINVAL, "NULL argument");
   *out = ctx->ws_bytes;
+  return ORCA_OK;
+}
+
+extern "C" int orca_ctx_fill_workspace(orca_ctx* ctx, size_t bytes, int value) {
+  if (!ctx) return fail(ORCA_EINVAL, "ctx is NULL");
+  HIPCHECK(hipSetDevice(ctx->device));
+  ORCA_TRY(ws_ensure(ctx, bytes));
+  if (ctx->ws) HIPCHECK(hipMemsetAsync(ctx->ws, value, ctx->ws_bytes, ctx->stream));
   return ORCA_OK;
 }
 
@@ -569,6 +577,12 @@
   return ORCA_OK;
 }
 
+extern "C" int orca_net_set_decoder_with_1m(orca_net* net, int on) {
+  if (!net || net->kind != ORCA_NET_DECODER) return fail(ORCA_EINVAL, "orca_net_set_decoder_with_1m: not a Decoder net");
+  net->dec_with_1m = on ? 1 : 0;
+  return ORCA_OK;
+}
+
 extern "C" int orca_net_free(orca_net* net) {
   if (!net) return ORCA_OK;
   if (net->ctx) (void)hipSetDevice(net->ctx->device);
diff --git a/orca_amd/csrc/orca_decoder.hip b/orca_amd/csrc/orca_decoder.hip
--- a/orca_amd/csrc/orca_decoder.hip
+++ b/orca_amd/csrc/orca_decoder.hip
@@ -34,8 +34,11 @@
 
 int launch_conv2d_m16(orca_ctx* ctx, const ConvLayer& L, const f32x4* x, long x_bs, int x_oct, f32x4* y, long y_bs, int y_oct,
                              const f32x4* r, long r_bs, int B, int n, int relu, int mode, int chunk0, int nchunks_,
-                             const float* tab, long tab_bs) {
+                             const float* tab, long tab_bs, const ConvLayer* L2, int split) {
   const bool bf16 = mode == 1;
+  if (L2 && (mode != 0 || split < 1 || split >= B || chunk0 || nchunks_ || tab || L2->ksize != 3 || L2->dil != L.dil || L2->cin != L.cin || L2->cout != L.cout ||
+             !L2->d_wf16 || !L2->f16_ok))
+    return fail(ORCA_EINVAL, "launch_conv2d_m16: the second layer does not ride in this launch");
   if (L.ksize != 3 || !L.d_wf16 || !L.d_wb16p) return fail(ORCA_EINVAL, "launch_conv2d_m16 on a layer without a 16-bit pack");
   if (!bf16 && !L.f16_ok) return fail(ORCA_EINVAL, "layer weights exceed the fp16 range");
   if (L.dil > 8) return fail(ORCA_EINVAL, "conv2d_3x3_m16_kernel handles dilations 1-8 (got %d); larger ones run as fused blocks", L.dil);
@@ -51,6 +54,7 @@
     aq.c = a; aq.c.banded = 0; aq.zero = reinterpret_cast<const f32x4*>(ctx->d_zero);
     aq.ngroups = ((n + 4 * L.dil - 1) / (4 * L.dil)) * L.dil;
     aq.nb = B;
+    aq.w2 = L2 ? L2->d_wf16 : nullptr; aq.bias2 = L2 ? L2->d_bias : nullptr; aq.split = L2 ? split : 0;
     const int ncu = device_cus();
     const int gx = (aq.ngroups * 2 + 7) / 8 * 8;
     int gy = B;
@@ -62,6 +66,7 @@
       hipLaunchKernelGGL((conv2d_3x3_m16q_kernel<decltype(co)::value, decltype(ns)::value, decltype(dt)::value>), gridq, dim3(512), 0, ctx->stream, aq);
     });
     LAUNCHCHECK("conv2d_3x3_m16q_kernel");
+    if (L2) ctx->counts[3]++;
     return ORCA_OK;
   }
   a.banded = n >= 64 ? 1 : 0;
@@ -74,7 +79,8 @@
 }
 
 template <int NS, int DT>
-int launch_dblocks(orca_ctx* ctx, f32x4* cur, long bs, int B, int n, const ConvLayer* p, int nblk) {
+int launch_dblocks(orca_ctx* ctx, f32x4* cur, long bs, int B, int n, const ConvLayer* p, int nblk, const ConvLayer* p2, int split) {
+  if (p2 && (split < 1 || split >= B)) return fail(ORCA_EINVAL, "launch_dblocks: second weight set from map %d of %d", split, B);
   if (nblk < 1 || nblk > (NS == 2 && DT == 1 ? 3 : 1)) return fail(ORCA_EINVAL, "launch_dblocks: %d blocks in one launch", nblk);
   DBlockArgs a{};
   a.cur = cur; a.bs = bs; a.H = n; a.W = n; a.dil = p[0].dil; a.nblk = nblk; a.flag = ctx->d_flag;
@@ -84,7 +90,14 @@
     if (DT == 1 && !p[k].f16_ok) return fail(ORCA_EINVAL, "layer weights exceed the fp16 range");
     a.w[k] = DT == 0 ? p[k].d_wb16p : p[k].d_wf16;
     a.bias[k] = p[k].d_bias;
-  }
+    if (p2) {
+      if (p2[k].dil != dil || p2[k].cin != p[k].cin || p2[k].cout != p[k].cout) return fail(ORCA_EINVAL, "decoder block: the second net's layer %d differs", k);
+      if (DT == 1 && !p2[k].f16_ok) return fail(ORCA_EINVAL, "layer weights exceed the fp16 range");
+      a.w[12 + k] = DT == 0 ? p2[k].d_wb16p : p2[k].d_wf16;
+      a.bias[12 + k] = p2[k].d_bias;
+    }
+  }
+  a.split = p2 ? split : 0;
   if (nblk == 1) {
     hipLaunchKernelGGL((conv2d_dblock_kernel<NS, DT>), dim3(256, (unsigned)B), dim3(512), 0, ctx->stream, a);
     LAUNCHCHECK("conv2d_dblock_kernel");
@@ -92,11 +105,12 @@
     hipLaunchKernelGGL((conv2d_dblock_run_kernel<2, 1>), dim3(256, (unsigned)B), dim3(512), 0, ctx->stream, a);
     LAUNCHCHECK("conv2d_dblock_run_kernel");
   }
-  return ORCA_OK;
-}
-template int launch_dblocks<2, 1>(orca_ctx*, f32x4*, long, int, int, const ConvLayer*, int);
-template int launch_dblocks<1, 0>(orca_ctx*, f32x4*, long, int, int, const ConvLayer*, int);
-template int launch_dblocks<1, 1>(orca_ctx*, f32x4*, long, int, int, const ConvLayer*, int);
+  if (p2) ctx->counts[3]++;
+  return ORCA_OK;
+}
+template int launch_dblocks<2, 1>(orca_ctx*, f32x4*, long, int, int, const ConvLayer*, int, const ConvLayer*, int);
+template int launch_dblocks<1, 0>(orca_ctx*, f32x4*, long, int, int, const ConvLayer*, int, const ConvLayer*, int);
+template int launch_dblocks<1, 1>(orca_ctx*, f32x4*, long, int, int, const ConvLayer*, int, const ConvLayer*, int);
 
 struct RowSrc {
   const float* base = nullptr;
@@ -137,13 +151,11 @@
   return conv(p[3], T, cur, &oth, 1);
 }
 
-template <class M, class Conv, class Block>
-static int decoder_chain(const orca_net* net, bool with_y, const M& IN, const M& A, const M& Bf, const M& Cf, const M& Df, const M& T, Conv conv,
-                         Block block, M* last) {
+template <class M, class Conv>
+static int decoder_chain_head(const orca_net* net, bool with_y, const M& IN, const M& A, const M& Bf, const M& Cf, const M& Df, const M& T, Conv& conv) {
   const bool is1m = net->kind == ORCA_NET_DECODER_1M;
   const ConvLayer* L = net->convs.data();
   const ConvLayer* pairs = is1m ? L : L + 8;
-  const int npairs = is1m ? 19 : 28;
   if (!is1m) {
     ORCA_TRY(conv(L[0], IN, Bf, nullptr, 0));
     ORCA_TRY(conv(L[1], Bf, Cf, nullptr, 0));
@@ -161,8 +173,39 @@
     ORCA_TRY(conv(pairs[2], Cf, T, nullptr, 1));
     ORCA_TRY(conv(pairs[3], T, Df, &Cf, 1));
   }
+  return ORCA_OK;
+}
+
+template <class M, class Conv, class Block>
+static int decoder_chain(const orca_net* net, bool with_y, const M& IN, const M& A, const M& Bf, const M& Cf, const M& Df, const M& T, Conv conv,
+                         Block block, M* last) {
+  const int npairs = net->kind == ORCA_NET_DECODER_1M ? 19 : 28;
+  ORCA_TRY(decoder_chain_head(net, with_y, IN, A, Bf, Cf, Df, T, conv));
   for (int i = 1; i < npairs; ++i) ORCA_TRY(block(i, Df, Cf));
   *last = Df;
+  return ORCA_OK;
+}
+
+static size_t dec_tab_floats(int n) { return (size_t)2 * 3 * n * 64; }
+template <int NS, int DT>
+static int decoder_head_m16(orca_ctx* ctx, const orca_net* net, const RowSrc& x, long sx_c, long sx_l, const RowSrc& de, long sd_c, long sd_h, long sd_w,
+                            const RowSrc& y, long sy_c, long sy_h, long sy_w, int B, int n, const DecMaps<f32x4>& IN, const DecMaps<f32x4>& A, float* TAB) {
+  const bool is1m = net->kind == ORCA_NET_DECODER_1M;
+  const size_t tabsz = dec_tab_floats(n);
+  for (int c0 = 0; c0 < B; c0 += 8) {
+    const int nc = B - c0 < 8 ? B - c0 : 8;
+    M16HeadArgs ha{};
+    for (int b = 0; b < nc; ++b) { ha.x[b] = x.at(c0 + b); ha.de[b] = de.at(c0 + b); ha.y[b] = (!is1m && y) ? y.at(c0 + b) : nullptr; }
+    ha.sx_c = sx_c; ha.sx_l = sx_l; ha.sd_c = sd_c; ha.sd_h = sd_h; ha.sd_w = sd_w; ha.sy_c = sy_c; ha.sy_h = sy_h; ha.sy_w = sy_w;
+    ha.in = IN.p + c0 * IN.bs; ha.in_bs = IN.bs;
+    ha.tab = is1m ? nullptr : TAB + c0 * tabsz; ha.tab_bs = (long)tabsz;
+    ha.a = A.p ? A.p + c0 * A.bs : nullptr; ha.a_bs = A.bs;
+    ha.wsep = net->d_sep; ha.nt = net->num_2d; ha.n = n; ha.o0 = is1m ? 0 : 16; ha.noct = IN.oct; ha.nsep = is1m ? 0 : 6;
+    ha.bilinear = net->upsample_mode == ORCA_UPSAMPLE_BILINEAR ? 1 : 0; ha.flag = ctx->d_flag;
+    const unsigned roles = (unsigned)(IN.oct + ha.nsep + ((!is1m && y) ? 1 : 0));
+    hipLaunchKernelGGL((decoder_head_m16_kernel<NS, DT>), dim3((unsigned)n, roles, (unsigned)nc), dim3(256), 0, ctx->stream, ha);
+    LAUNCHCHECK("decoder_head_m16_kernel");
+  }
   return ORCA_OK;
 }
 
@@ -171,11 +214,10 @@
                        long sd_c, long sd_h, long sd_w, const RowSrc& y, long sy_c, long sy_h, long sy_w, int B, int n,
                        float* out, int accumulate, const DecoderProbe* probe = nullptr) {
   typedef DecMaps<f32x4> M;
-  const int nt2 = net->num_2d;
   const bool is1m = net->kind == ORCA_NET_DECODER_1M;
   const int mode = DT == 0 ? 1 : (NS == 1 ? 2 : 0);
   const int oIN = is1m ? 16 : 2, oA = 10;
-  const size_t tabsz = (size_t)2 * 3 * n * 64;
+  const size_t tabsz = dec_tab_floats(n);
   const size_t upo = (size_t)NS * n * ORCA_LDW;
   const size_t szIN = upo * oIN, szA = upo * oA, sz64 = upo * 8, sz32 = upo * 4;
   const size_t need = ru256(B * szIN * 16) + ru256(B * szA * 16) + 3 * ru256(B * sz64 * 16) + ru256(B * sz32 * 16) + ru256(B * tabsz * 4);
@@ -193,20 +235,7 @@
   };
 #define PROBE(k, m) \
   if (probe && probe->stage == (k)) return emit(m)
-  for (int c0 = 0; c0 < B; c0 += 8) {
-    const int nc = B - c0 < 8 ? B - c0 : 8;
-    M16HeadArgs ha{};
-    for (int b = 0; b < nc; ++b) { ha.x[b] = x.at(c0 + b); ha.de[b] = de.at(c0 + b); ha.y[b] = (!is1m && y) ? y.at(c0 + b) : nullptr; }
-    ha.sx_c = sx_c; ha.sx_l = sx_l; ha.sd_c = sd_c; ha.sd_h = sd_h; ha.sd_w = sd_w; ha.sy_c = sy_c; ha.sy_h = sy_h; ha.sy_w = sy_w;
-    ha.in = IN.p + c0 * szIN; ha.in_bs = (long)szIN;
-    ha.tab = is1m ? nullptr : TAB + c0 * tabsz; ha.tab_bs = (long)tabsz;
-    ha.a = A.p + c0 * szA; ha.a_bs = (long)szA;
-    ha.wsep = net->d_sep; ha.nt = nt2; ha.n = n; ha.o0 = is1m ? 0 : 16; ha.noct = oIN; ha.nsep = is1m ? 0 : 6;
-    ha.bilinear = net->upsample_mode == ORCA_UPSAMPLE_BILINEAR ? 1 : 0; ha.flag = ctx->d_flag;
-    const unsigned roles = (unsigned)(oIN + ha.nsep + ((!is1m && y) ? 1 : 0));
-    hipLaunchKernelGGL((decoder_head_m16_kernel<NS, DT>), dim3((unsigned)n, roles, (unsigned)nc), dim3(256), 0, s, ha);
-    LAUNCHCHECK("decoder_head_m16_kernel");
-  }
+  ORCA_TRY((decoder_head_m16<NS, DT>(ctx, net, x, sx_c, sx_l, de, sd_c, sd_h, sd_w, y, sy_c, sy_h, sy_w, B, n, IN, A, TAB)));
   const auto stop = [](int rc) { return rc == DEC_STOP ? ORCA_OK : rc; };
   if (probe && probe->stage == 0) return stop(emit(IN));
   const ConvLayer* L = net->convs.data();
@@ -296,6 +325,112 @@
   return ORCA_OK;
 }
 
+static bool same_block(const ConvLayer* p, const ConvLayer* q) {
+  for (int k = 0; k < 4; ++k)
+    if (p[k].ksize != 3 || q[k].ksize != 3 || p[k].dil != q[k].dil || p[k].cin != q[k].cin || p[k].cout != q[k].cout || p[k].cin != ((k & 1) ? 32 : 64) ||
+        p[k].cout != ((k & 1) ? 64 : 32) || !p[k].d_wf16 || !q[k].d_wf16 || !p[k].f16_ok || !q[k].f16_ok)
+      return false;
+  return true;
+}
+static int block_launch_len(const orca_net* net, const ConvLayer* pairs, int npairs, int i) {
+  const ConvLayer* p = pairs + 4 * i;
+  if (p[0].dil < 16) return 0;
+  bool is_run = net->dec_block_runs && p[0].dil == 16 && i + 2 < npairs;
+  for (int k = 0; is_run && k < 12; ++k) is_run = p[k].dil == 16 << (k >> 2);
+  return is_run ? 3 : 1;
+}
+
+static int decoder_with_1m_m16(orca_ctx* ctx, orca_net* net, orca_net* net1, const RowSrc& x, long sx_c, long sx_l, const RowSrc& de, long sd_c, long sd_h,
+                               long sd_w, const RowSrc& y, long sy_c, long sy_h, long sy_w, int B, int n, float* out) {
+  typedef DecMaps<f32x4> M;
+  constexpr int NS = 2, DT = 1;
+  const size_t tabsz = dec_tab_floats(n), upo = (size_t)NS * n * ORCA_LDW;
+  const size_t szIN = upo * 2, szIN1 = upo * 16, szA = upo * 10, sz64 = upo * 8, sz32 = upo * 4;
+  const size_t need = ru256(B * szIN * 16) + ru256(B * szIN1 * 16) + ru256(B * szA * 16) + ru256(B * sz64 * 16) + 2 * ru256(2 * B * sz64 * 16) +
+                      ru256(2 * B * sz32 * 16) + ru256(B * tabsz * 4);
+  ORCA_TRY(ws_ensure(ctx, need));
+  auto take = [&](size_t units, int oct, int maps) { return M{reinterpret_cast<f32x4*>(ws_take(ctx, maps * units * 4)), (long)units, oct}; };
+  float* const TAB = ws_take(ctx, B * tabsz);
+  const M IN = take(szIN, 2, B), IN1 = take(szIN1, 16, B), A = take(szA, 10, B), Bf = take(sz64, 8, B);
+  const M Cf = take(sz64, 8, 2 * B), Df = take(sz64, 8, 2 * B), T = take(sz32, 4, 2 * B);
+  auto rows1 = [&](const M& m) { return M{m.p + (size_t)B * m.bs, m.bs, m.oct}; };
+  const M Cf1 = rows1(Cf), Df1 = rows1(Df), T1 = rows1(T);
+  const ConvLayer* const LD = net->convs.data();
+  const ConvLayer *const pD = LD + 8, *const pM = net1->convs.data();
+  const int nD = 28, nM = 19;
+  const ConvLayer *jd = nullptr, *jm = nullptr;
+  auto convD = [&](const ConvLayer& l, const M& src, const M& dst, const M* res, int relu) -> int {
+    const bool sep = &l == LD;
+    return launch_conv2d_m16(ctx, l, src.p, src.bs, src.oct, dst.p, dst.bs, dst.oct, res ? res->p : nullptr, res ? res->bs : 0, B, n, relu, 0, sep ? 8 : 0,
+                             sep ? 1 : 0, sep ? TAB : nullptr, sep ? (long)tabsz : 0);
+  };
+  auto convM = [&](const ConvLayer& l, const M& src, const M& dst, const M* res, int relu) -> int {
+    return launch_conv2d_m16(ctx, l, src.p, src.bs, src.oct, dst.p, dst.bs, dst.oct, res ? res->p : nullptr, res ? res->bs : 0, B, n, relu, 0);
+  };
+  auto convJ = [&](const ConvLayer& l, const M& src, const M& dst, const M* res, int relu) -> int {
+    return launch_conv2d_m16(ctx, l, src.p, src.bs, src.oct, dst.p, dst.bs, dst.oct, res ? res->p : nullptr, res ? res->bs : 0, 2 * B, n, relu, 0, 0, 0, nullptr,
+                             0, jm + (&l - jd), B);
+  };
+  RowSrc none;
+  ORCA_TRY((decoder_head_m16<NS, DT>(ctx, net, x, sx_c, sx_l, de, sd_c, sd_h, sd_w, y, sy_c, sy_h, sy_w, B, n, IN, A, TAB)));
+  ORCA_TRY(decoder_chain_head(net, (bool)y, IN, A, Bf, Cf, Df, T, convD));
+  ORCA_TRY((decoder_head_m16<NS, DT>(ctx, net1, x, sx_c, sx_l, none, 0, 0, 0, none, 0, 0, 0, B, n, IN1, M{nullptr, 0, 0}, nullptr)));
+  ORCA_TRY(decoder_chain_head(net1, false, IN1, A, Bf, Cf1, Df1, T1, convM));
+  int iD = 1, iM = 1;
+  while (iD < nD || iM < nM) {
+    const ConvLayer* const bd = iD < nD ? pD + 4 * iD : nullptr;
+    const ConvLayer* const bm = iM < nM ? pM + 4 * iM : nullptr;
+    if (bd && bm && same_block(bd, bm)) {
+      const int lenD = block_launch_len(net, pD, nD, iD), lenM = block_launch_len(net1, pM, nM, iM);
+      if (lenD == 0) {
+        jd = bd; jm = bm;
+        ORCA_TRY(residual_block(convJ, bd, Df, Cf, T));
+        ++iD; ++iM;
+      } else {
+        const int nblk = (lenD == 3 && lenM == 3 && same_block(bd + 4, bm + 4) && same_block(bd + 8, bm + 8)) ? 3 : 1;
+        ORCA_TRY((launch_dblocks<NS, DT>(ctx, Df.p, Df.bs, 2 * B, n, bd, nblk, bm, B)));
+        iD += nblk; iM += nblk;
+      }
+    } else if (bd) {
+      const int len = block_launch_len(net, pD, nD, iD);
+      if (len == 0) ORCA_TRY(residual_block(convD, bd, Df, Cf, T));
+      else ORCA_TRY((launch_dblocks<NS, DT>(ctx, Df.p, Df.bs, B, n, bd, len)));
+      iD += len ? len : 1;
+    } else {
+      const int len = block_launch_len(net1, pM, nM, iM);
+      if (len == 0) ORCA_TRY(residual_block(convM, bm, Df1, Cf1, T1));
+      else ORCA_TRY((launch_dblocks<NS, DT>(ctx, Df1.p, Df1.bs, B, n, bm, len)));
+      iM += len ? len : 1;
+    }
+  }
+  const FinalArgs fa = final_args(net, reinterpret_cast<const float*>(Df.p), Df.bs, out, n, 0);
+  hipLaunchKernelGGL((final_sym_m16_kernel<NS, DT>), dim3(136u, (unsigned)B), dim3(256), 0, ctx->stream, fa);
+  const FinalArgs f1 = final_args(net1, reinterpret_cast<const float*>(Df1.p), Df1.bs, out, n, 1);
+  hipLaunchKernelGGL((final_sym_m16_kernel<NS, DT>), dim3(136u, (unsigned)B), dim3(256), 0, ctx->stream, f1);
+  LAUNCHCHECK("final_sym_m16_kernel");
+  return ORCA_OK;
+}
+
+extern "C" int orca_decoder_forward_rows_with_1m(orca_ctx* ctx, orca_net* net, orca_net* net_1m, const float* const* x_rows, int64_t sx_c, int64_t sx_l,
+                                                 const float* const* distenc_rows, int64_t sd_c, int64_t sd_h, int64_t sd_w, const float* const* y_rows,
+                                                 int64_t sy_c, int64_t sy_h, int64_t sy_w, int B, int n, float* out) {
+  if (!ctx || !net || !net_1m || !x_rows || !distenc_rows || !out) return fail(ORCA_EINVAL, "orca_decoder_forward_rows_with_1m: NULL argument");
+  if (net->kind != ORCA_NET_DECODER || net_1m->kind != ORCA_NET_DECODER_1M)
+    return fail(ORCA_EINVAL, "orca_decoder_forward_rows_with_1m: takes a Decoder and a Decoder_1m");
+  if (net->num_2d != net_1m->num_2d) return fail(ORCA_EINVAL, "orca_decoder_forward_rows_with_1m: the nets predict %d and %d maps", net->num_2d, net_1m->num_2d);
+  for (int b = 0; b < B; ++b)
+    if (!x_rows[b] || !distenc_rows[b] || (y_rows && !y_rows[b])) return fail(ORCA_EINVAL, "orca_decoder_forward_rows_with_1m: NULL row pointer %d", b);
+  RowSrc xs, ds, ys, none;
+  xs.rows = x_rows; ds.rows = distenc_rows; ys.rows = y_rows;
+  if (net->dec_with_1m && net->precision == ORCA_PRECISION_F16X2 && net_1m->precision == ORCA_PRECISION_F16X2 && B > 0) {
+    if (n <= 0 || n > ORCA_LDW || (n & 1)) return fail(ORCA_EINVAL, "map size %d unsupported (even, <=256)", n);
+    HIPCHECK(hipSetDevice(ctx->device));
+    return decoder_with_1m_m16(ctx, net, net_1m, xs, sx_c, sx_l, ds, sd_c, sd_h, sd_w, ys, sy_c, sy_h, sy_w, B, n, out);
+  }
+  ORCA_TRY(decoder_common(ctx, net, xs, sx_c, sx_l, ds, sd_c, sd_h, sd_w, ys, sy_c, sy_h, sy_w, B, n, out, 0));
+  return decoder_common(ctx, net_1m, xs, sx_c, sx_l, none, 0, 0, 0, none, 0, 0, 0, B, n, out, 1);
+}
+
 extern "C" int orca_decoder_forward(orca_ctx* ctx, orca_net* net, const float* x, int64_t sx_b, int64_t sx_c, int64_t sx_l,
                                     const float* distenc, int64_t sd_b, int64_t sd_h, int64_t sd_w, const float* y,
                                     int64_t sy_b, int64_t sy_h, int64_t sy_w, int B, int n, float* out, int accumulate) {
diff --git a/orca_amd/csrc/orca_internal.h b/orca_amd/csrc/orca_internal.h
--- a/orca_amd/csrc/orca_internal.h
+++ b/orca_amd/csrc/orca_internal.h
@@ -85,6 +85,7 @@
   int kind = 0;
   int precision = ORCA_PRECISION_F32;
   int dec_block_runs = 1;
+  int dec_with_1m = 1;
   int enc_two_strands = 1;
   int enc_form = ORCA_ENCODER_FORM_DEFAULT;
   float* d_first_w = nullptr;
@@ -158,6 +159,7 @@
 int launch_pool(orca_ctx* ctx, const float* x, long ldx, float* y, long ldy, long rows, long n_out, int k);
 int launch_conv2d(orca_ctx* ctx, const ConvLayer& L, const float* x, long x_bs, float* y, long y_bs, const float* r, long r_bs, int B, int n, int relu);
 int launch_conv2d_m16(orca_ctx* ctx, const ConvLayer& L, const f32x4* x, long x_bs, int x_oct, f32x4* y, long y_bs, int y_oct, const f32x4* r, long r_bs, int B,
-                      int n, int relu, int mode, int chunk0 = 0, int nchunks_ = 0, const float* tab = nullptr, long tab_bs = 0);
+                      int n, int relu, int mode, int chunk0 = 0, int nchunks_ = 0, const float* tab = nullptr, long tab_bs = 0, const ConvLayer* L2 = nullptr,
+                      int split = 0);
 template <int NS, int DT>
-int launch_dblocks(orca_ctx* ctx, f32x4* cur, long bs, int B, int n, const ConvLayer* p, int nblk);
+int launch_dblocks(orca_ctx* ctx, f32x4* cur, long bs, int B, int n, const ConvLayer* p, int nblk, const ConvLayer* p2 = nullptr, int split = 0);
diff --git a/orca_amd/engine.py b/orca_amd/engine.py
--- a/orca_amd/engine.py
+++ b/orca_amd/engine.py
@@ -53,6 +53,10 @@
 
     def release_workspace(self):
         check(_lib.load().orca_ctx_release_workspace(self.handle))
+
+    def fill_workspace(self, nbytes, value=0xFF):
+        self.sync_stream()
+        check(_lib.load().orca_ctx_fill_workspace(self.handle, nbytes, value), "orca_ctx_fill_workspace")
 
 
 def get_context(device):
@@ -282,6 +286,9 @@
 
     def set_decoder_block_runs(self, on):
         check(_lib.load().orca_net_set_decoder_block_runs(self.handle, 1 if on else 0), "orca_net_set_decoder_block_runs")
+
+    def set_decoder_with_1m(self, on):
+        check(_lib.load().orca_net_set_decoder_with_1m(self.handle, 1 if on else 0), "orca_net_set_decoder_with_1m")
 
     def set_encoder_two_strands(self, on):
         check(_lib.load().orca_net_set_encoder_two_strands(self.handle, 1 if on else 0), "orca_net_set_encoder_two_strands")
@@ -933,6 +940,32 @@
     return out
 
 
+def decoder_forward_rows_with_1m(net, net_1m, xs, des, ys=None, out=None):
+    if net.ctx is not net_1m.ctx:
+        raise ValueError("decoder_forward_rows_with_1m: the two nets belong to different contexts")
+    xs = [_f32_cuda(t, "x") for t in xs]
+    des = [_f32_cuda(t, "distenc") for t in des]
+    B, T = len(xs), net.num_targets()
+    C, n = xs[0].shape
+    if C != 128 or tuple(des[0].shape) != (T, n, n) or len(des) != B or net_1m.num_targets() != T:
+        raise ValueError(f"decoder rows: x [128,n] and distenc [{T},n,n] per row, got {tuple(xs[0].shape)} / {tuple(des[0].shape)}")
+    sx, sd = _same_strides(xs, "x"), _same_strides(des, "distenc")
+    yp, sy = None, (0, 0, 0)
+    if ys is not None:
+        ys = [_f32_cuda(t, "y") for t in ys]
+        if len(ys) != B or tuple(ys[0].shape) != (T, n // 2, n // 2):
+            raise ValueError(f"coarse prediction rows must be [{T},{n // 2},{n // 2}]")
+        yp, sy = _row_ptrs(ys), _same_strides(ys, "y")
+    if out is None:
+        out = torch.empty((B, T, n, n), dtype=torch.float32, device=xs[0].device)
+    elif tuple(out.shape) != (B, T, n, n) or not out.is_contiguous():
+        raise ValueError(f"out must be a contiguous [{B},{T},{n},{n}] tensor")
+    net.ctx.sync_stream()
+    check(_lib.load().orca_decoder_forward_rows_with_1m(net.ctx.handle, net.handle, net_1m.handle, _row_ptrs(xs), sx[0], sx[1], _row_ptrs(des), sd[0],
+                                                        sd[1], sd[2], yp, sy[0], sy[1], sy[2], B, n, _p(out)), "orca_decoder_forward_rows_with_1m")
+    return out
+
+
 def decoder1m_forward_rows(net, xs, out=None, accumulate=False):
     xs = [_f32_cuda(t, "x") for t in xs]
     B, T = len(xs), net.num_targets()
diff --git a/orca_amd/orca_modules.py b/orca_amd/orca_modules.py
--- a/orca_amd/orca_modules.py
+++ b/orca_amd/orca_modules.py
@@ -355,6 +355,19 @@
         net = self._net(xs[0].device)
         return self._run_guarded(net, lambda: engine.decoder_forward_rows(net, xs, distencs, ys), "f32")
 
+    def forward_rows_with_1m(self, dec_1m, xs, distencs, ys=None):
+        net, net1 = self._net(xs[0].device), dec_1m._net(xs[0].device)
+        if (self.precision == "f16x2" and dec_1m.precision == "f16x2" and self.num_2d == dec_1m.num_2d and net.ctx is net1.ctx
+                and not engine._guard["force_safe"]):
+            self._apply_precision(net, "f16x2")
+            dec_1m._apply_precision(net1, "f16x2")
+            out = engine.decoder_forward_rows_with_1m(net, net1, xs, distencs, ys)
+            if engine._guard["defer"] or not net.ctx.take_overflow():
+                return out
+        out = self.forward_rows(xs, distencs, ys)
+        dec_1m.forward_rows_into(out, xs, accumulate=True)
+        return out
+
 
 class Decoder_1m(_HipModule):
 
diff --git a/orca_amd/orca_predict.py b/orca_amd/orca_predict.py
--- a/orca_amd/orca_predict.py
+++ b/orca_amd/orca_predict.py
@@ -338,9 +338,12 @@
             xs = _rows(encodings[level], B, sl, 250, (2,))
             des = [bgs[k][b if bgs[k].shape[0] > 1 else 0] for k in range(S) for b in range(B)]
             ys = _rows(preds[j - 1], B, zoom_idx, 125, (2, 3)) if j > 0 else None
-            pred = dec.forward_rows(xs, des, ys)
-            if level == add_1m_level:
-                model.denet_1_pt.forward_rows_into(pred, xs, accumulate=True)
+            if level == add_1m_level and hasattr(dec, "forward_rows_with_1m"):
+                pred = dec.forward_rows_with_1m(model.denet_1_pt, xs, des, ys)
+            else:
+                pred = dec.forward_rows(xs, des, ys)
+                if level == add_1m_level:
+                    model.denet_1_pt.forward_rows_into(pred, xs, accumulate=True)
             preds.append(pred)
         else:
             enc = _gather(encodings[level], B, sl, 250, (2,))
```

New measurement: 1016 Mb/s, median of 6. No clear change (+0.1%).
